# rishabhjain16/audio-visual-llm

Measured on AMD Instinct MI355X. Metric: AV-clip train-step samples/sec (clip_whisper -> Llama-2-7B LoRA), whole job, higher is better.
Workload: dtype bf16

## Files before the change

### audio-visual-llm_amd/avllm/lib.py

```python
from __future__ import annotations

import ctypes as C
import os

import torch

_HERE = os.path.dirname(os.path.abspath(__file__))
LIB_PATH = os.environ.get("AVLLM_LIB_PATH") or os.path.join(_HERE, "libavllm.so")

F32, BF16 = 0, 1
ACT_NONE, ACT_GELU, ACT_QUICK_GELU, ACT_SILU = 0, 1, 2, 3
GEMM_KERNELS = ("SMALLM", "SKINNY64", "128", "RING", "H16", "HP16", "W4", "WP4", "DP", "F32")
ATTN_FORMS = ("ref", "short13x7", "short17x9", "mfma64x4", "mfma128x4")
LORA_PAD = 64

i32, i64, f32, vp, sz = C.c_int32, C.c_int64, C.c_float, C.c_void_p, C.c_size_t
fp = C.POINTER(C.c_float)


class GemmDesc(C.Structure):
    _fields_ = [("A", vp), ("B", vp), ("A2", vp), ("B2", vp), ("C", vp), ("bias", vp), ("R", vp),
                ("lda", i64), ("ldb", i64), ("lda2", i64), ("ldb2", i64), ("ldc", i64), ("ldr", i64),
                ("M", i32), ("N", i32), ("K", i32), ("K2", i32), ("dtype", i32), ("out_f32", i32), ("act", i32),
                ("alpha", f32), ("r_mod", i32), ("g_in", i32), ("g_out", i32), ("g_off", i32), ("drop_seed", C.c_uint32), ("drop_p", f32), ("a_drop_seed", C.c_uint32), ("a_drop_p", f32), ("n_valid", i32), ("seed_dev", vp)]


class EncLayer(C.Structure):
    _fields_ = [(n, vp) for n in ("ln1_w", "ln1_b", "wqkv", "bqkv", "wo", "bo", "ln2_w", "ln2_b", "w1", "b1", "w2", "b2",
                                  "wqkv8", "sqkv8", "wo8", "so8", "w18", "s18", "w28", "s28")]


class Whisper(C.Structure):
    _fields_ = [(n, i32) for n in ("dtype", "d", "heads", "layers", "ffn", "n_mels", "n_ctx", "k1pad")] + \
               [(n, vp) for n in ("conv1_w", "conv1_b", "conv2_w", "conv2_b", "pos")] + \
               [("layer", C.POINTER(EncLayer)), ("lnf_w", vp), ("lnf_b", vp), ("fp8", i32)]


class Clip(C.Structure):
    _fields_ = [(n, i32) for n in ("dtype", "d", "heads", "layers", "ffn", "image", "patch", "tokens")] + \
               [("eps", f32)] + [(n, vp) for n in ("patch_w", "class_emb", "pos", "pre_ln_w", "pre_ln_b")] + \
               [("layer", C.POINTER(EncLayer)), ("fp8", i32), ("frames_bf16", i32)]


class LoraMod(C.Structure):
    _fields_ = [("A_pad", vp), ("AT_pad", vp), ("B_pad", vp), ("BT_pad", vp), ("ld_at", i64), ("gA", vp), ("gB", vp)]


class LlamaLayer(C.Structure):
    _fields_ = [(n, vp) for n in ("ln1_w", "ln2_w", "wqkv", "wo", "wgu", "wdown", "wqkv_t", "wo_t", "wgu_t", "wdown_t")] + \
               [("lora", LoraMod * 4)] + [(n, vp) for n in ("wqkv8", "sqkv8", "wo8", "so8", "wgu8", "sgu8", "wdown8", "sdown8")] + \
               [(n, vp) for n in ("eqkv8", "eo8", "egu8", "edown8")] + \
               [(n, vp) for n in ("wqkv4", "wo4", "wgu4", "wdown4", "eqkv4", "eo4", "egu4", "edown4")] + \
               [(n, vp) for n in ("bqkv", "bo")] + [(n, vp) for n in ("q_norm_w", "k_norm_w")] + [("lora_mlp", LoraMod * 3)]


class Llama(C.Structure):
    _fields_ = [(n, i32) for n in ("dtype", "d", "heads", "layers", "ffn", "vocab", "lora_r", "kv_heads")] + \
               [(n, f32) for n in ("eps", "theta", "lora_scale", "lora_dropout")] + [("dropout_seed", C.c_uint32)] + \
               [(n, vp) for n in ("dropout_seed_dev", "embed", "norm_w", "lm_head", "lm_head_t")] + [("layer", C.POINTER(LlamaLayer))] + \
               [("fp8", i32), ("lm_head8", vp), ("slm_head8", vp)] + \
               [(n, f32) for n in ("rope_factor", "rope_low_freq_factor", "rope_high_freq_factor")] + [("rope_orig_ctx", i32)] + \
               [("decode_fp8", i32), ("elm_head8", vp), ("decode_fp4", i32), ("kv_fp8", i32)]


class GemmF8Desc(C.Structure):
    _fields_ = [("A", vp), ("SA", vp), ("B", vp), ("SB", vp), ("C", vp), ("bias", vp), ("R", vp), ("lda", i64), ("ldb", i64), ("ldc", i64),
                ("ldr", i64), ("M", i32), ("N", i32), ("K", i32), ("act", i32), ("Cq", vp), ("SCq", vp), ("ldcq", i64)]


class DecProjDesc(C.Structure):
    _fields_ = [("A", vp), ("lda", i64), ("W", vp), ("ldw", i64), ("norm_w", vp), ("eps", f32), ("M", i32), ("K", i32), ("N", i32), ("mode", i32),
                ("C", vp), ("ldc", i64), ("out_f32", i32), ("R", vp), ("ldr", i64), ("dq", i32), ("dkv", i32), ("hd", i32), ("rope", vp),
                ("kc", vp), ("vc", vp), ("Tmax", i32), ("pos", i32), ("pos_dev", vp),
                ("lora_t", vp), ("ld_lora_t", i64), ("lora_b", vp * 3), ("lora_r", i32), ("lora_scale", f32), ("W8", vp), ("E8", vp), ("W4", vp),
                ("bias", vp), ("raw_qkv", i32)]


class LogitsProcDesc(C.Structure):
    _fields_ = [("scores", vp), ("ld", i64), ("rows", i64), ("V", i32), ("dtype", i32),
                ("history", vp), ("ldh", i64), ("append", vp), ("cur", i32), ("cur_dev", vp),
                ("repetition_penalty", f32), ("no_repeat_ngram_size", i32), ("min_new_tokens", i32), ("eos", i64), ("log_softmax", i32),
                ("bias_tokens", vp), ("bias_lengths", vp), ("bias_values", vp), ("n_bias", i32), ("bias_max_len", i32),
                ("bad_tokens", vp), ("bad_lengths", vp), ("n_bad", i32), ("bad_max_len", i32),
                ("suppress", vp), ("n_suppress", i32), ("begin_suppress", vp), ("n_begin_suppress", i32)]


class StepState(C.Structure):
    _fields_ = [("step", C.c_uint32), ("dropout_seed", C.c_uint32), ("lr", f32), ("bc1", f32), ("bc2_sqrt", f32), ("skipped", f32),
                ("reserved", C.c_uint32 * 2)]


class AdamwSeg(C.Structure):
    _fields_ = [("p", vp), ("m", vp), ("v", vp), ("g", vp), ("n", i64), ("weight_decay", f32), ("reserved", i32)]


class Schedule(C.Structure):
    _fields_ = [("base_lr", f32), ("beta1", f32), ("beta2", f32), ("warmup_steps", i32), ("total_steps", i32), ("rank", C.c_uint32)]


LAYER_CB = C.CFUNCTYPE(None, i32, vp)

_SIGS = {
    "avllm_version": ([], i32),
    "avllm_gemm": ([C.POINTER(GemmDesc), vp], i32),
    "avllm_gemm_plan": ([C.POINTER(GemmDesc), C.POINTER(i32)], i32),
    "avllm_set_gemm_variant": ([i32], i32),
    "avllm_set_knob": ([C.c_char_p, i32], i32),
    "avllm_get_knob": ([C.c_char_p, C.POINTER(i32)], i32),
    "avllm_attention_fwd_mxq": ([vp, vp, vp, vp, i64, vp, i32, i32, i32, i32, i64, i64, i64, f32, vp], i32),
    "avllm_im2col_k3": ([vp, vp, i32, i32, i32, i32, i32, vp], i32),
    "avllm_groupnorm_tokens": ([vp, vp, vp, vp, i32, i32, i32, i32, f32, i32, i32, vp], i32),
    "avllm_gemm_tn": ([vp, i64, i32, vp, i64, i32, i32, vp, i64, f32, i32, vp], i32),
    "avllm_gemm_tn_drop": ([vp, i64, i32, vp, i64, i32, i32, vp, i64, f32, C.c_uint32, f32, i32, vp], i32),
    "avllm_logmel_table_bytes": ([], C.c_size_t),
    "avllm_logmel_table_init": ([vp, i32], i32),
    "avllm_logmel_workspace_bytes": ([i32, i32], C.c_size_t),
    "avllm_logmel": ([vp, vp, i32, i32, i64, i32, i32, vp, vp, C.c_size_t, vp], i32),
    "avllm_clip_preproc_plan_bytes": ([i32, i32, i32], C.c_size_t),
    "avllm_clip_preproc_plan_init": ([vp, i32, i32, i32, vp, vp], i32),
    "avllm_clip_preproc_workspace_bytes": ([i32, i32, i32, i32], C.c_size_t),
    "avllm_clip_preproc": ([vp, vp, i32, i32, i32, i32, vp, i32, vp, C.c_size_t, vp], i32),
    "avllm_wave_add_noise_chunk": ([], i32),
    "avllm_wave_add_noise_workspace_bytes": ([i32, i32], C.c_size_t),
    "avllm_wave_add_noise": ([vp, i64, vp, i32, i32, vp, i64, vp, i32, vp, f32, f32, f32, C.c_uint32, vp, vp, i64, vp, vp, C.c_size_t, vp], i32),
    "avllm_spec_augment": ([vp, i32, i32, i32, vp, i32, i32, f32, i32, i32, f32, C.c_uint32, vp, vp, vp], i32),
    "avllm_lora_pack_batch": ([vp, i32, i32, i32, i32, vp], i32),
    "avllm_lora_merge": ([vp, i64, i32, i32, vp, vp, i32, f32, i32, vp], i32),
    "avllm_layernorm": ([vp, vp, vp, vp, i64, i32, f32, i32, vp], i32),
    "avllm_rmsnorm_fwd": ([vp, vp, vp, vp, i64, i32, f32, i32, vp], i32),
    "avllm_rmsnorm_bwd": ([vp, vp, vp, vp, vp, vp, i64, i32, i32, vp], i32),
    "avllm_rope": ([vp, i64, i64, i32, i32, i32, i32, f32, i32, i32, vp], i32),
    "avllm_rope_table": ([vp, i32, i32, i32, f32, vp, f32, f32, f32, i32, vp], i32),
    "avllm_rope_tab": ([vp, i64, i64, i32, i32, i32, vp, i32, i32, vp], i32),
    "avllm_kv_append": ([vp, vp, i64, vp, vp, i32, i32, i32, i32, i32, i32, vp], i32),
    "avllm_swiglu_fwd": ([vp, vp, i64, i32, i32, vp], i32),
    "avllm_swiglu_bwd": ([vp, vp, vp, i64, i32, i32, vp], i32),
    "avllm_swiglu_bwd_h": ([vp, vp, vp, vp, i64, i32, i32, vp], i32),
    "avllm_attention_fwd": ([vp, vp, vp, vp, vp, i32, i32, i32, i32, i32, i64, i64, i64, i64, f32, i32, i32, i32, i32, vp], i32),
    "avllm_attention_bwd": ([vp] * 10 + [i32] * 4 + [i64] * 7 + [f32, i32, i32, i32, i32, vp], i32),
    "avllm_attention_bwd_rope": ([vp] * 10 + [i32] * 4 + [i64] * 7 + [f32, i32, i32, i32, i32, vp, vp], i32),
    "avllm_attention_plan": ([i32] * 9 + [C.POINTER(i32), C.POINTER(i32)], i32),
    "avllm_attention_fwd_mxq_ok": ([i32] * 6, i32),
    "avllm_attention_bwd_fuses_rope": ([i32] * 3, i32),
    "avllm_ce_fwd": ([vp, i64, vp, i32, i32, i32, vp, vp, vp, i32, vp], i32),
    "avllm_ce_bwd": ([vp, i64, vp, vp, vp, f32, vp, i32, i32, i32, i32, vp], i32),
    "avllm_argmax_rows": ([vp, i64, i64, i32, vp, i32, vp], i32),
    "avllm_sample_rows": ([vp, i64, i64, i32, f32, i32, f32, C.c_uint32, vp, i32, vp, vp, i64, i64, vp, i32, vp], i32),
    "avllm_sample_rows_scored": ([vp, i64, i64, i32, f32, i32, f32, C.c_uint32, vp, i32, vp, vp, i64, i64, vp, vp, i32, vp], i32),
    "avllm_row_scores": ([vp, i64, i64, i32, vp, f32, vp, vp, i32, vp], i32),
    "avllm_row_scores_logprobs": ([vp, i64, i64, i32, vp, vp, vp, i32, vp], i32),
    "avllm_beam_topk_workspace_bytes": ([i64, i32, i32], sz),
    "avllm_beam_topk": ([vp, i64, i32, i32, i32, vp, i32, vp, vp, vp, vp, sz, vp], i32),
    "avllm_beam_topk_logprobs": ([vp, i64, i32, i32, i32, vp, i32, vp, vp, vp, vp, sz, vp], i32),
    "avllm_logits_process": ([vp, i64, i64, i32, vp, i64, vp, i32, vp, f32, i32, i32, i64, i32, i32, vp], i32),
    "avllm_logits_process_ex": ([C.POINTER(LogitsProcDesc), vp], i32),
    "avllm_kv_gather_rows": ([vp, vp, i32, i64, vp, vp, i32, i64, i32, i32, vp, i32, i32, i32, vp], i32),
    "avllm_embedding": ([vp, vp, vp, i64, i32, i32, vp], i32),
    "avllm_cast": ([vp, i32, vp, i32, i64, vp], i32),
    "avllm_act_residual": ([vp, vp, vp, i64, i32, i32, vp], i32),
    "avllm_dropout": ([vp, vp, i64, i32, C.c_uint32, f32, i32, vp], i32),
    "avllm_whisper_im2col1": ([vp, vp, i32, i32, i32, i32, i32, vp], i32),
    "avllm_whisper_im2col2": ([vp, vp, i32, i32, i32, i32, vp], i32),
    "avllm_clip_patchify": ([vp, vp, i32, i32, i32, i32, i32, vp], i32),
    "avllm_clip_cls_rows": ([vp, vp, vp, i32, i32, i32, i32, vp], i32),
    "avllm_fuse_pool": ([vp, i32, vp, i32, vp, i32, vp, i32, i32, i32, i32, f32, i32, vp], i32),
    "avllm_fuse_pool_bwd": ([vp, vp, i32, vp, i32, i32, i32, i32, i32, i32, f32, i32, vp], i32),
    "avllm_fuse_pool_rows": ([vp, i32, vp, i32, vp, i32, vp, vp, i32, i32, i32, i32, f32, i32, vp], i32),
    "avllm_fuse_pool_rows_bwd": ([vp, vp, i32, vp, i32, i32, vp, i32, i32, i32, i32, f32, i32, vp], i32),
    "avllm_modality_draw": ([vp, vp, i32, f32, f32, C.c_uint32, vp, vp], i32),
    "avllm_gemm_wgrad": ([vp, i64, vp, i64, i32, i32, i32, vp, i64, vp, f32, i32, vp], i32),
    "avllm_grad_sumsq_det_multi": ([C.POINTER(vp), C.POINTER(i64), i32, vp, i32, vp, vp], i32),
    "avllm_adamw_step_multi": ([C.POINTER(AdamwSeg), i32, f32, f32, f32, f32, i32, vp, f32, f32, vp, vp, vp, vp], i32),
    "avllm_grad_sumsq": ([vp, i64, vp, vp], i32),
    "avllm_grad_sumsq_det": ([vp, i64, vp, i32, vp, vp], i32),
    "avllm_adamw_step": ([vp, vp, vp, vp, i64, f32, f32, f32, f32, f32, i32, vp, f32, f32, vp, vp, vp, vp], i32),
    "avllm_step_advance": ([vp, C.POINTER(Schedule), vp], i32),
    "avllm_mx_scale_bytes": ([i32, i32], sz),
    "avllm_mx_quantize": ([vp, i64, i32, i32, vp, i64, vp, i32, i32, vp], i32),
    "avllm_mx4_quantize": ([vp, i64, i32, i32, vp, i64, vp, i32, vp], i32),
    "avllm_gemm_f8": ([C.POINTER(GemmF8Desc), vp], i32),
    "avllm_lora_dx_masked": ([C.POINTER(vp), C.POINTER(i64), C.POINTER(vp), C.POINTER(i64), C.POINTER(C.c_uint32), i32, i32, vp, i64, vp, i64, i32,
                              i32, f32, vp, i32, vp], i32),
    "avllm_llama_lora_bwd_layers": ([C.POINTER(Llama), vp, i32, i32, vp, f32, vp, sz, i32, i32, LAYER_CB, vp, vp], i32),
    "avllm_llama_lora_bwd_layers_dx": ([C.POINTER(Llama), vp, i32, i32, vp, f32, vp, sz, i32, i32, LAYER_CB, vp, vp, vp], i32),
    "avllm_lora_pack": ([vp, vp, i32, i32, i32, vp, vp, i64, vp, vp, i32, vp], i32),
    "avllm_profile_begin": ([i32], i32),
    "avllm_profile_enable": ([i32], i32),
    "avllm_profile_end": ([C.POINTER(C.c_double)], i32),
    "avllm_whisper_workspace_bytes": ([C.POINTER(Whisper), i32], sz),
    "avllm_whisper_encoder_fwd": ([C.POINTER(Whisper), vp, i32, vp, vp, sz, vp], i32),
    "avllm_clip_workspace_bytes": ([C.POINTER(Clip), i32], sz),
    "avllm_clip_vision_cls_fwd": ([C.POINTER(Clip), vp, i32, vp, vp, sz, vp], i32),
    "avllm_llama_train_workspace_bytes": ([C.POINTER(Llama), i32, i32], sz),
    "avllm_llama_lora_fwd_loss": ([C.POINTER(Llama), vp, vp, i32, i32, vp, vp, vp, vp, sz, vp], i32),
    "avllm_llama_lora_bwd": ([C.POINTER(Llama), vp, i32, i32, vp, f32, vp, sz, LAYER_CB, vp, vp], i32),
    "avllm_llama_infer_workspace_bytes": ([C.POINTER(Llama), i32, i32], sz),
    "avllm_llama_prefill": ([C.POINTER(Llama), vp, i32, i32, vp, vp, i32, vp, vp, vp, sz, vp], i32),
    "avllm_llama_decode_step": ([C.POINTER(Llama), vp, i32, i32, vp, vp, i32, vp, vp, sz, vp], i32),
    "avllm_llama_decode_step_at": ([C.POINTER(Llama), vp, i32, i32, vp, vp, vp, i32, vp, vp, sz, vp], i32),
    "avllm_llama_decode_is_fused": ([C.POINTER(Llama), i32], i32),
    "avllm_llama_decode_streams_fp8": ([C.POINTER(Llama), i32], i32),
    "avllm_llama_decode_streams_fp4": ([C.POINTER(Llama), i32], i32),
    "avllm_llama_decode_caches_fp8": ([C.POINTER(Llama), i32], i32),
    "avllm_llama_decode_shared_workspace_bytes": ([C.POINTER(Llama), i32], sz),
    "avllm_llama_decode_step_shared": ([C.POINTER(Llama), vp, i32, i32, i32, vp, vp, vp, i32, vp, vp, i32, vp, vp, sz, vp], i32),
    "avllm_llama_decode_shares_prefix": ([C.POINTER(Llama), i32], i32),
    "avllm_attention_decode_shared_workspace_bytes": ([i32, i32, i32], sz),
    "avllm_attention_decode_shared": ([vp, i64, vp, vp, i32, i32, vp, vp, i32, vp, i32, vp, i64, i32, i32, i32, i32, f32, i32, vp, sz, vp], i32),
    "avllm_attention_decode_shared_kv8": ([vp, i64, vp, vp, vp, vp, i32, i32, vp, vp, vp, vp, i32, vp, i32, vp, i64, i32, i32, i32, i32, f32, i32, vp, sz,
                                           vp], i32),
    "avllm_llama_kv_cache_bytes": ([C.POINTER(Llama), i32, i32], sz),
    "avllm_kv8_append": ([vp, vp, i64, vp, vp, vp, vp, i32, i32, i32, i32, i32, vp], i32),
    "avllm_kv8_rope_append": ([vp, i64, i32, i32, i32, i32, vp, i32, vp, vp, vp, vp, i32, i32, vp, vp], i32),
    "avllm_attention_decode_kv8": ([vp, i64, vp, vp, vp, vp, vp, i64, i32, i32, i32, i32, vp, i32, f32, i32, vp], i32),
    "avllm_kv8_gather_rows": ([vp, vp, i32, i64, vp, vp, i32, i64, i32, i32, vp, i32, i32, vp], i32),
    "avllm_pos_advance": ([vp, i32, vp], i32),
    "avllm_dec_proj": ([C.POINTER(DecProjDesc), vp], i32),
    "avllm_gemm_f8_takes_quantised_output": ([C.POINTER(GemmF8Desc)], i32),
    "avllm_gemm_f8_takes_fast": ([C.POINTER(GemmF8Desc)], i32),
    "avllm_norm_mxq": ([vp, vp, vp, vp, vp, vp, i64, vp, i64, i32, f32, vp], i32),
    "avllm_lora_rank3": ([vp, vp, vp, vp, vp, vp, vp, vp, i32, i32, i32, f32, f32, vp, i32, i32, vp], i32),
    "avllm_gemm_tn_multi": ([vp, i64, i32, vp, vp, vp, vp, vp, vp, vp, i32, i32, i32, f32, f32, vp, i32, i32, vp], i32),
    "avllm_qk_norm_rope": ([vp, i64, i64, i32, i32, i32, i32, vp, vp, f32, vp, vp, vp, vp, vp, i32, i32, vp, i32, vp], i32),
    "avllm_qk_norm_bwd": ([vp, i64, i64, i32, i32, i32, vp, vp, vp, vp, i32, vp], i32),
    "avllm_attention_decode": ([vp, i64, vp, vp, vp, i64, i32, i32, i32, i32, vp, i32, f32, i32, i32, vp], i32),
}

EXPORTS = sorted(list(_SIGS) + ["avllm_last_error"])

_lib = None


def load():
    global _lib
    if _lib is not None:
        return _lib
    if not os.path.exists(LIB_PATH):
        raise RuntimeError(f"libavllm.so not found at {LIB_PATH}: run `python build.py` (hipcc, gfx950). "
                           "There is no CPU or PyTorch fallback for the hot path.")
    lib = C.CDLL(LIB_PATH)
    lib.avllm_last_error.restype = C.c_char_p
    lib.avllm_last_error.argtypes = []
    for name, (args, res) in _SIGS.items():
        fn = getattr(lib, name)
        fn.argtypes = args
        fn.restype = res
    _lib = lib
    return lib


class AvllmError(RuntimeError):
    pass


class knob:

    def __init__(self, name, value):
        self.name, self.value = name.encode(), int(value)

    def __enter__(self):
        prev = i32()
        check(load().avllm_get_knob(self.name, C.byref(prev)))
        self.prev = prev.value
        check(load().avllm_set_knob(self.name, self.value))
        return self

    def __exit__(self, *a):
        check(load().avllm_set_knob(self.name, self.prev))


def check(rc: int):
    if rc != 0:
        msg = load().avllm_last_error().decode(errors="replace")
        if rc == 1:
            raise ValueError(msg)
        raise AvllmError(f"libavllm error {rc}: {msg}")


def dt_of(t: torch.Tensor) -> int:
    if t.dtype == torch.float32:
        return F32
    if t.dtype == torch.bfloat16:
        return BF16
    raise TypeError(f"unsupported dtype {t.dtype}")


def torch_dtype(dt: int):
    return torch.float32 if dt == F32 else torch.bfloat16


def ptr(t):
    if t is None:
        return None
    assert t.is_cuda, "device tensor required"
    return t.data_ptr()


def stream_ptr():
    return torch.cuda.current_stream().cuda_stream
```

### audio-visual-llm_amd/avllm/ops.py

```python
from __future__ import annotations

import collections
import ctypes as C
import math
import numbers

import numpy as np
import torch

from . import lib as L


def _ld(t):
    assert t.stride(-1) == 1, "innermost dimension must be contiguous"
    return t.stride(-2) if t.dim() >= 2 else t.shape[-1]


def gemm(A, B, out=None, bias=None, R=None, A2=None, B2=None, act=L.ACT_NONE, alpha=1.0, out_f32=False,
         r_mod=0, remap=None, M=None, a_drop=None, n_valid=0, drop=None, plan=False):
    lib = L.load()
    M = A.shape[0] if M is None else M
    N, K = B.shape[0], B.shape[1]
    dt = L.dt_of(A)
    if out is None:
        rows = M if remap is None else (M // remap[0]) * remap[1]
        out = torch.empty(rows, N, device=A.device, dtype=torch.float32 if (out_f32 or dt == L.F32) else A.dtype)
    d = L.GemmDesc()
    d.A, d.B, d.C = L.ptr(A), L.ptr(B), L.ptr(out)
    d.lda, d.ldb, d.ldc = _ld(A), _ld(B), _ld(out)
    d.M, d.N, d.K = M, N, K
    if A2 is not None:
        d.A2, d.B2, d.lda2, d.ldb2, d.K2 = L.ptr(A2), L.ptr(B2), _ld(A2), _ld(B2), B2.shape[1]
    d.bias = L.ptr(bias)
    if R is not None:
        d.R, d.ldr = L.ptr(R), _ld(R)
    d.dtype, d.out_f32, d.act, d.alpha, d.r_mod = dt, int(out_f32), act, alpha, r_mod
    if remap is not None:
        d.g_in, d.g_out, d.g_off = remap
    if a_drop is not None:
        d.a_drop_seed, d.a_drop_p = a_drop[0] & 0xFFFFFFFF, a_drop[1]
    if drop is not None:
        d.drop_seed, d.drop_p = drop[0] & 0xFFFFFFFF, drop[1]
    d.n_valid = n_valid
    if plan:
        k = L.i32()
        L.check(lib.avllm_gemm_plan(C.byref(d), C.byref(k)))
        return L.GEMM_KERNELS[k.value]
    L.check(lib.avllm_gemm(C.byref(d), L.stream_ptr()))
    return out


def gemm_tn(P, Q, out, I=None, J=None, alpha=1.0, drop=None):
    lib = L.load()
    I = P.shape[1] if I is None else I
    J = Q.shape[1] if J is None else J
    if drop is not None:
        L.check(lib.avllm_gemm_tn_drop(L.ptr(P), _ld(P), I, L.ptr(Q), _ld(Q), J, P.shape[0], L.ptr(out), _ld(out), alpha,
                                       drop[0] & 0xFFFFFFFF, drop[1], L.dt_of(P), L.stream_ptr()))
        return out
    L.check(lib.avllm_gemm_tn(L.ptr(P), _ld(P), I, L.ptr(Q), _ld(Q), J, P.shape[0], L.ptr(out), _ld(out), alpha,
                              L.dt_of(P), L.stream_ptr()))
    return out


def layernorm(x, w, b, eps=1e-5):
    y = torch.empty_like(x)
    L.check(L.load().avllm_layernorm(L.ptr(x), L.ptr(w), L.ptr(b), L.ptr(y), x.numel() // x.shape[-1], x.shape[-1], eps,
                                     L.dt_of(x), L.stream_ptr()))
    return y


def rmsnorm_fwd(x, w, eps):
    y = torch.empty_like(x)
    rows = x.numel() // x.shape[-1]
    rstd = torch.empty(rows, device=x.device, dtype=torch.float32)
    L.check(L.load().avllm_rmsnorm_fwd(L.ptr(x), L.ptr(w), L.ptr(y), L.ptr(rstd), rows, x.shape[-1], eps, L.dt_of(x), L.stream_ptr()))
    return y, rstd


def rmsnorm_bwd(dy, x, w, rstd, dres=None):
    dx = torch.empty_like(x)
    L.check(L.load().avllm_rmsnorm_bwd(L.ptr(dy), L.ptr(x), L.ptr(w), L.ptr(rstd), L.ptr(dres), L.ptr(dx),
                                       x.numel() // x.shape[-1], x.shape[-1], L.dt_of(x), L.stream_ptr()))
    return dx


def rope_(x2d, T, heads, hd, pos0=0, theta=10000.0, inverse=False):
    L.check(L.load().avllm_rope(L.ptr(x2d), _ld(x2d), x2d.shape[0], T, heads, hd, pos0, theta, int(inverse), L.dt_of(x2d), L.stream_ptr()))
    return x2d


def rope_table(T, hd, pos0=0, theta=10000.0, pos_dev=None, scaling=None, device="cuda"):
    tab = torch.empty(T, hd // 2, 2, device=device, dtype=torch.float32)
    if pos_dev is not None:
        assert pos_dev.dtype == torch.int32 and pos_dev.numel() == 1 and pos_dev.is_cuda
    f, lo, hi, octx = scaling if scaling else (1.0, 1.0, 4.0, 0)
    L.check(L.load().avllm_rope_table(L.ptr(tab), T, hd, pos0, theta, L.ptr(pos_dev), f, lo, hi, int(octx), L.stream_ptr()))
    return tab


def rope_tab_(x2d, T, heads, hd, tab, inverse=False):
    assert tab.dtype == torch.float32 and tab.is_contiguous() and tab.numel() == T * hd
    L.check(L.load().avllm_rope_tab(L.ptr(x2d), _ld(x2d), x2d.shape[0], T, heads, hd, L.ptr(tab), int(inverse), L.dt_of(x2d), L.stream_ptr()))
    return x2d


def qk_norm_rope_(x2d, T, heads, kv_heads, hd, q_w, k_w, eps, tab, save=False, kc=None, vc=None, pos=0, pos_dev=None):
    rows, nqk = x2d.shape[0], heads + kv_heads
    assert tab.dtype == torch.float32 and tab.is_contiguous() and tab.numel() == T * hd and q_w.dtype == x2d.dtype and k_w.dtype == x2d.dtype
    pre = torch.empty(rows, nqk * hd, device=x2d.device, dtype=x2d.dtype) if save else None
    rstd = torch.empty(rows, nqk, device=x2d.device, dtype=torch.float32) if save else None
    if kc is not None:
        assert kc.shape == vc.shape == (rows, kc.shape[1], kv_heads * hd) and kc.is_contiguous() and vc.is_contiguous() and kc.dtype == x2d.dtype
    L.check(L.load().avllm_qk_norm_rope(L.ptr(x2d), _ld(x2d), rows, T, heads, kv_heads, hd, L.ptr(q_w), L.ptr(k_w), eps, L.ptr(tab), L.ptr(pre),
                                        L.ptr(rstd), L.ptr(kc), L.ptr(vc), kc.shape[1] if kc is not None else 0, pos, L.ptr(pos_dev), L.dt_of(x2d),
                                        L.stream_ptr()))
    return pre, rstd


def qk_norm_bwd_(dy2d, heads, kv_heads, hd, q_w, k_w, pre, rstd):
    assert pre.is_contiguous() and rstd.is_contiguous() and rstd.dtype == torch.float32 and pre.dtype == dy2d.dtype
    L.check(L.load().avllm_qk_norm_bwd(L.ptr(dy2d), _ld(dy2d), dy2d.shape[0], heads, kv_heads, hd, L.ptr(q_w), L.ptr(k_w), L.ptr(pre), L.ptr(rstd),
                                       L.dt_of(dy2d), L.stream_ptr()))
    return dy2d


def kv_append(k, v, kc, vc, T, pos0):
    B, Tmax, d = kc.shape
    assert k.shape == (B * T, d) and v.shape == k.shape and _ld(k) == _ld(v) and kc.is_contiguous() and vc.is_contiguous() and vc.shape == kc.shape
    L.check(L.load().avllm_kv_append(L.ptr(k), L.ptr(v), _ld(k), L.ptr(kc), L.ptr(vc), B, T, pos0, Tmax, d, L.dt_of(kc), L.stream_ptr()))


def swiglu_fwd(gu):
    M, F2 = gu.shape
    h = torch.empty(M, F2 // 2, device=gu.device, dtype=gu.dtype)
    L.check(L.load().avllm_swiglu_fwd(L.ptr(gu), L.ptr(h), M, F2 // 2, L.dt_of(gu), L.stream_ptr()))
    return h


def swiglu_bwd(dh, gu):
    dgu = torch.empty_like(gu)
    L.check(L.load().avllm_swiglu_bwd(L.ptr(dh), L.ptr(gu), L.ptr(dgu), gu.shape[0], gu.shape[1] // 2, L.dt_of(gu), L.stream_ptr()))
    return dgu


def swiglu_bwd_h(dh, gu):
    if gu.dim() != 2 or gu.shape[1] % 8 or dh.shape != (gu.shape[0], gu.shape[1] // 2) or dh.dtype != gu.dtype:
        raise ValueError(f"swiglu_bwd_h: gu [M, 2F] with F % 4 == 0 and dh [M, F] of one dtype, got {tuple(gu.shape)} and {tuple(dh.shape)}")
    if not (gu.is_contiguous() and dh.is_contiguous()):
        raise ValueError("swiglu_bwd_h: contiguous tensors")
    dgu = torch.empty_like(gu)
    h = torch.empty_like(dh)
    L.check(L.load().avllm_swiglu_bwd_h(L.ptr(dh), L.ptr(gu), L.ptr(dgu), L.ptr(h), gu.shape[0], gu.shape[1] // 2, L.dt_of(gu), L.stream_ptr()))
    return dgu, h


def attention_plan(B, Tq, Tk, H, hd, causal, dtype, impl=0, kv_heads=None):
    f, b = L.i32(-1), L.i32(-1)
    L.check(L.load().avllm_attention_plan(B, Tq, Tk, H, hd, int(causal), dtype, impl, kv_heads or 0, C.byref(f), C.byref(b)))
    return L.ATTN_FORMS[f.value], (L.ATTN_FORMS[b.value] if b.value >= 0 else None)


def attention_fwd(qkv, B, T, H, hd, causal, scale=None, impl=0, want_lse=True, kv_heads=None, Tk=None, k=None, v=None, out=None, plan=False):
    d = H * hd
    dkv = (kv_heads or H) * hd
    Tk = T if Tk is None else Tk
    assert (k is None) == (v is None) and (k is not None or Tk == T)
    if plan:
        return attention_plan(B, T, Tk, H, hd, causal, L.dt_of(qkv), impl, kv_heads)[0]
    o = torch.empty(B * T, d, device=qkv.device, dtype=qkv.dtype) if out is None else out
    assert o.shape == (B * T, d) and o.dtype == qkv.dtype
    lse = torch.empty(B, H, T, device=qkv.device, dtype=torch.float32) if want_lse else None
    es = qkv.element_size()
    scale = hd ** -0.5 if scale is None else scale
    p = L.ptr(qkv)
    if k is None:
        pk, pv, ldk, ldv = p + d * es, p + (d + dkv) * es, _ld(qkv), _ld(qkv)
    else:
        assert qkv.shape == (B * T, d) and k.shape == (B * Tk, dkv) and v.shape == k.shape and k.dtype == qkv.dtype and v.dtype == qkv.dtype
        pk, pv, ldk, ldv = L.ptr(k), L.ptr(v), _ld(k), _ld(v)
    L.check(L.load().avllm_attention_fwd(p, pk, pv, L.ptr(o), L.ptr(lse), B, T, Tk, H, hd, _ld(qkv), ldk, ldv, _ld(o), scale, int(causal),
                                         L.dt_of(qkv), impl, kv_heads or 0, L.stream_ptr()))
    return o, lse


def attention_fwd_mxq(qkv, B, T, H, hd, scale=None):
    lib = L.load()
    d = H * hd
    q = torch.empty(B * T, d, device=qkv.device, dtype=torch.uint8)
    s = torch.zeros(lib.avllm_mx_scale_bytes(B * T, d), device=qkv.device, dtype=torch.uint8)
    es = qkv.element_size()
    p = L.ptr(qkv)
    L.check(lib.avllm_attention_fwd_mxq(p, p + d * es, p + 2 * d * es, L.ptr(q), d, L.ptr(s), B, T, H, hd, _ld(qkv), _ld(qkv), _ld(qkv),
                                        float(hd ** -0.5 if scale is None else scale), L.stream_ptr()))
    return q, s


def attention_bwd(qkv, o, dout, lse, B, T, H, hd, causal, scale=None, impl=0, kv_heads=None, rope_tab=None, out=None, plan=False):
    if plan:
        return attention_plan(B, T, T, H, hd, causal, L.dt_of(qkv), impl, kv_heads)[1]
    d = H * hd
    dkv = (kv_heads or H) * hd
    dqkv = torch.empty_like(qkv) if out is None else out
    assert dqkv.shape == qkv.shape and dqkv.dtype == qkv.dtype
    delta = torch.empty(B, H, T, device=qkv.device, dtype=torch.float32)
    es = qkv.element_size()
    scale = hd ** -0.5 if scale is None else scale
    p, g = L.ptr(qkv), L.ptr(dqkv)
    args = (p, p + d * es, p + (d + dkv) * es, L.ptr(o), L.ptr(dout), L.ptr(lse), g, g + d * es, g + (d + dkv) * es,
            L.ptr(delta), B, T, H, hd, _ld(qkv), _ld(qkv), _ld(qkv), d, _ld(dqkv), _ld(dqkv), _ld(dqkv),
            scale, int(causal), L.dt_of(qkv), impl, kv_heads or 0)
    if rope_tab is None:
        L.check(L.load().avllm_attention_bwd(*args, L.stream_ptr()))
    else:
        assert rope_tab.dtype == torch.float32 and rope_tab.is_contiguous() and rope_tab.numel() == T * hd
        L.check(L.load().avllm_attention_bwd_rope(*args, L.ptr(rope_tab), L.stream_ptr()))
    return dqkv


def _ce_ld(logits):
    B, T, V = logits.shape
    ld = logits.stride(1) if T > 1 else (logits.stride(0) if B > 1 else (V + 7) // 8 * 8)
    if logits.stride(2) != 1 or (B > 1 and logits.stride(0) != T * ld) or ld < V or ld % 8:
        raise ValueError(f"cross entropy: logits {tuple(logits.shape)} with strides {tuple(logits.stride())} are not [B*T] rows of one stride "
                         "(a multiple of 8, >= V)")
    return ld


def ce_fwd(logits, labels):
    B, T, V = logits.shape
    row_lse = torch.empty(B * T, device=logits.device, dtype=torch.float32)
    acc = torch.zeros(2, device=logits.device, dtype=torch.float32)
    L.check(L.load().avllm_ce_fwd(L.ptr(logits), _ce_ld(logits), L.ptr(labels), B, T, V, L.ptr(row_lse), L.ptr(acc), L.ptr(acc) + 4,
                                  L.dt_of(logits), L.stream_ptr()))
    return row_lse, acc


def ce_bwd(logits, labels, row_lse, acc, grad_scale=1.0, out=None):
    B, T, V = logits.shape
    ld = _ce_ld(logits)
    if out is None:
        out = torch.empty_strided(logits.shape, logits.stride(), device=logits.device, dtype=logits.dtype)
    elif out.shape != logits.shape or out.stride() != logits.stride() or out.dtype != logits.dtype or out.device != logits.device:
        raise ValueError("ce_bwd: out must have the shape, strides, dtype and device of logits")
    L.check(L.load().avllm_ce_bwd(L.ptr(logits), ld, L.ptr(labels), L.ptr(row_lse), L.ptr(acc) + 4, grad_scale, L.ptr(out),
                                  B, T, V, L.dt_of(logits), L.stream_ptr()))
    return out


def argmax_rows(logits2d):
    out = torch.empty(logits2d.shape[0], device=logits2d.device, dtype=torch.int64)
    L.check(L.load().avllm_argmax_rows(L.ptr(logits2d), _ld(logits2d), logits2d.shape[0], logits2d.shape[1], L.ptr(out),
                                       L.dt_of(logits2d), L.stream_ptr()))
    return out


def check_sampling(temperature, top_k, top_p):
    if not (float(temperature) > 0.0 and float(temperature) < float("inf")):
        raise ValueError(f"temperature must be a strictly positive float, got {temperature}")
    if not (0.0 < float(top_p) <= 1.0):
        raise ValueError(f"top_p must be a float in (0, 1], got {top_p}")
    if int(top_k) != top_k or int(top_k) < 0:
        raise ValueError(f"top_k must be a non-negative integer, got {top_k}")


def row_scores(logits, tokens, temperature=1.0, entropy=False, logprobs=False):
    if not (torch.is_tensor(logits) and logits.dim() == 2 and logits.is_cuda and logits.stride(1) == 1
            and logits.dtype in (torch.float32, torch.bfloat16)):
        raise ValueError("row_scores: logits must be a 2-d float32 device tensor with unit column stride")
    rows, V = logits.shape
    if tokens is not None and not (torch.is_tensor(tokens) and tokens.dtype == torch.int64 and tokens.shape == (rows,) and tokens.is_cuda
                                   and tokens.is_contiguous()):
        raise ValueError(f"row_scores: tokens must be int64 [{rows}] on the device")
    if not logprobs and not (float(temperature) > 0.0 and float(temperature) < float("inf")):
        raise ValueError(f"temperature must be a strictly positive float, got {temperature}")
    lp = torch.empty(rows, device=logits.device, dtype=torch.float32)
    ent = torch.empty(rows, device=logits.device, dtype=torch.float32) if entropy else None
    lib = L.load()
    if logprobs:
        L.check(lib.avllm_row_scores_logprobs(L.ptr(logits), _ld(logits), rows, V, L.ptr(tokens), L.ptr(lp), L.ptr(ent), L.dt_of(logits),
                                              L.stream_ptr()))
    else:
        L.check(lib.avllm_row_scores(L.ptr(logits), _ld(logits), rows, V, L.ptr(tokens), float(temperature), L.ptr(lp), L.ptr(ent),
                                     L.dt_of(logits), L.stream_ptr()))
    return (lp, ent) if entropy else lp


def sample_rows(logits, temperature, top_k, top_p, seed, step, unfinished=None, eos=None, pad=None, row_seeds=None, return_logprob=False):
    check_sampling(temperature, top_k, top_p)
    rows, V = logits.shape
    out = torch.empty(rows, device=logits.device, dtype=torch.int64)
    step_dev = None
    if torch.is_tensor(step):
        assert step.dtype == torch.int32 and step.numel() == 1 and step.is_cuda
        step_dev, step = step, 0
    if unfinished is not None:
        assert unfinished.dtype == torch.bool and unfinished.shape == (rows,) and unfinished.is_contiguous()
    if row_seeds is not None:
        assert row_seeds.dtype == torch.int32 and row_seeds.shape == (rows,) and row_seeds.is_contiguous()
    eos = -1 if eos is None else int(eos)
    pad = (eos if eos >= 0 else 0) if pad is None else int(pad)
    lp = torch.empty(rows, device=logits.device, dtype=torch.float32) if return_logprob else None
    L.check(L.load().avllm_sample_rows_scored(L.ptr(logits), _ld(logits), rows, V, float(temperature), int(top_k), float(top_p),
                                              int(seed) & 0xFFFFFFFF, L.ptr(row_seeds), int(step), L.ptr(step_dev), L.ptr(unfinished),
                                              eos, pad, L.ptr(out), L.ptr(lp), L.dt_of(logits), L.stream_ptr()))
    return (out, lp) if return_logprob else out


LOGITS_PROCESS_MAX_HISTORY = 1024


def check_logits_processors(repetition_penalty, no_repeat_ngram_size, min_new_tokens):
    p = repetition_penalty
    if isinstance(p, bool) or not isinstance(p, numbers.Real) or not (0.0 < float(p) < float("inf")):
        raise ValueError(f"repetition_penalty must be a strictly positive float, got {p!r}")
    for name, v in (("no_repeat_ngram_size", no_repeat_ngram_size), ("min_new_tokens", min_new_tokens)):
        if isinstance(v, bool) or not isinstance(v, numbers.Integral) or v < 0:
            raise ValueError(f"{name} must be a non-negative integer, got {v!r}")
    return float(p) != 1.0 or no_repeat_ngram_size > 0 or min_new_tokens > 0


LOGITS_BIAS_MAX_SEQUENCES, LOGITS_BIAS_MAX_SEQUENCE_LENGTH = 4096, 16

SequenceTable = collections.namedtuple("SequenceTable", "tokens lengths values n max_len vocab")
TokenTable = collections.namedtuple("TokenTable", "ids n vocab")
_TABLE_FIELDS = {
    "sequence_bias": (SequenceTable, dict(bias_tokens="tokens", bias_lengths="lengths", bias_values="values", n_bias="n", bias_max_len="max_len")),
    "bad_words_ids": (SequenceTable, dict(bad_tokens="tokens", bad_lengths="lengths", n_bad="n", bad_max_len="max_len")),
    "suppress_tokens": (TokenTable, dict(suppress="ids", n_suppress="n")),
    "begin_suppress_tokens": (TokenTable, dict(begin_suppress="ids", n_begin_suppress="n")),
}


def _token_ids(name, ids, vocab):
    if hasattr(ids, "tolist"):
        ids = ids.tolist()
    if isinstance(ids, (str, bytes, dict)) or not hasattr(ids, "__iter__"):
        raise ValueError(f"{name} must be a list of token ids, got {ids!r}")
    ids = list(ids)
    for t in ids:
        if isinstance(t, bool) or not isinstance(t, numbers.Integral) or t < 0:
            raise ValueError(f"{name} must hold non-negative integers, got {t!r}")
        if vocab is not None and t >= vocab:
            raise ValueError(f"{name}: token id {t} is outside the vocabulary of {vocab} entries")
    return [int(t) for t in ids]


def _sequences(name, seqs):
    if len(seqs) > LOGITS_BIAS_MAX_SEQUENCES:
        raise ValueError(f"{name} has {len(seqs)} sequences: at most LOGITS_BIAS_MAX_SEQUENCES = {LOGITS_BIAS_MAX_SEQUENCES} are supported")
    for q in seqs:
        if len(q) == 0:
            raise ValueError(f"{name} has an empty sequence")
        if len(q) > LOGITS_BIAS_MAX_SEQUENCE_LENGTH:
            raise ValueError(f"{name} has a sequence of {len(q)} tokens: at most LOGITS_BIAS_MAX_SEQUENCE_LENGTH = "
                             f"{LOGITS_BIAS_MAX_SEQUENCE_LENGTH} are supported")
    return seqs


def _normalise_logits_bias(sequence_bias, bad_words_ids, suppress_tokens, begin_suppress_tokens, vocab, eos):
    sb = bw = None
    if sequence_bias is not None:
        if isinstance(sequence_bias, dict):
            if any(not isinstance(k, tuple) for k in sequence_bias):
                raise ValueError(f"sequence_bias has to be a dict with tuples of token ids as keys, got {sequence_bias!r}")
            items = list(sequence_bias.items())
        elif isinstance(sequence_bias, (list, tuple)):
            if any(not isinstance(e, (list, tuple)) or len(e) != 2 or not isinstance(e[0], (list, tuple)) for e in sequence_bias):
                raise ValueError(f"sequence_bias has to be a list of [token ids, bias] pairs, got {sequence_bias!r}")
            items = [(tuple(e[0]), e[1]) for e in sequence_bias]
        else:
            raise ValueError(f"sequence_bias has to be a non-empty dict or list of [token ids, bias] pairs, got {sequence_bias!r}")
        if not items:
            raise ValueError("sequence_bias has to be non-empty")
        sb = {}
        for k, b in items:
            if isinstance(b, bool) or not isinstance(b, (float, np.floating)) or not math.isfinite(b):
                raise ValueError(f"sequence_bias: the bias of {k!r} must be a finite float, got {b!r}")
            sb[tuple(_token_ids("sequence_bias", k, vocab))] = float(b)
        _sequences("sequence_bias", list(sb))
    if bad_words_ids is not None:
        if not isinstance(bad_words_ids, (list, tuple)) or len(bad_words_ids) == 0:
            raise ValueError(f"bad_words_ids has to be a non-empty list, got {bad_words_ids!r}")
        if any(not isinstance(w, (list, tuple)) for w in bad_words_ids):
            raise ValueError(f"bad_words_ids has to be a list of lists of token ids, got {bad_words_ids!r}")
        bw = [tuple(_token_ids("bad_words_ids", w, vocab)) for w in bad_words_ids]
        bw = list(dict.fromkeys(w for w in bw if eos is None or w != (int(eos),)))
        if not bw:
            raise ValueError("bad_words_ids holds nothing but [eos], which HF drops: no sequence is left to ban")
        _sequences("bad_words_ids", bw)
    st = None if suppress_tokens is None else sorted(set(_token_ids("suppress_tokens", suppress_tokens, vocab)))
    bs = None if begin_suppress_tokens is None else sorted(set(_token_ids("begin_suppress_tokens", begin_suppress_tokens, vocab)))
    return sb, bw, st or None, bs or None


def check_logits_bias(sequence_bias=None, bad_words_ids=None, suppress_tokens=None, begin_suppress_tokens=None, vocab=None, eos=None):
    return any(t is not None for t in _normalise_logits_bias(sequence_bias, bad_words_ids, suppress_tokens, begin_suppress_tokens, vocab, eos))


def logits_bias_tables(sequence_bias=None, bad_words_ids=None, suppress_tokens=None, begin_suppress_tokens=None, *, vocab, eos=None,
                       device="cuda"):
    sb, bw, st, bs = _normalise_logits_bias(sequence_bias, bad_words_ids, suppress_tokens, begin_suppress_tokens, int(vocab), eos)

    def seq_table(seqs, values):
        tok = np.full((len(seqs), LOGITS_BIAS_MAX_SEQUENCE_LENGTH), -1, dtype=np.int32)
        for i, q in enumerate(seqs):
            tok[i, :len(q)] = q
        ln = np.array([len(q) for q in seqs], dtype=np.int32)
        dev = lambda a: torch.from_numpy(a).to(device)
        return SequenceTable(dev(tok), dev(ln), None if values is None else dev(np.array(values, dtype=np.float32)), len(seqs), int(ln.max()),
                             int(vocab))

    out = {}
    if sb is not None:
        keys = sorted(sb, key=lambda q: (q[-1], len(q) != 1))
        out["sequence_bias"] = seq_table(keys, [sb[q] for q in keys])
    if bw is not None:
        out["bad_words_ids"] = seq_table(bw, None)
    for name, ids in (("suppress_tokens", st), ("begin_suppress_tokens", bs)):
        if ids is not None:
            out[name] = TokenTable(torch.tensor(ids, dtype=torch.int32).to(device), len(ids), int(vocab))
    return out


def logits_process(scores, history, cur, repetition_penalty=1.0, no_repeat_ngram_size=0, min_new_tokens=0, eos=None, log_softmax=False,
                   append=None, *, sequence_bias=None, bad_words_ids=None, suppress_tokens=None, begin_suppress_tokens=None):
    check_logits_processors(repetition_penalty, no_repeat_ngram_size, min_new_tokens)
    if scores.dim() != 2 or not scores.is_cuda or scores.stride(1) != 1:
        raise ValueError("logits_process: scores must be a 2-d device tensor with unit column stride")
    rows, V = scores.shape
    cur_dev = None
    if torch.is_tensor(cur):
        assert cur.dtype == torch.int32 and cur.numel() == 1 and cur.is_cuda
        cur_dev, cur = cur, 0
    hptr, ldh = None, 0
    if history is not None:
        if history.dtype != torch.int64 or history.dim() != 2 or history.shape[0] != rows or not history.is_cuda or \
                (history.shape[1] > 1 and history.stride(1) != 1):
            raise ValueError(f"logits_process: history must be an int64 device tensor [{rows}, ld] with unit column stride")
        ldh = history.stride(0) if rows > 1 and history.shape[1] > 0 else history.shape[1]
        if cur_dev is None and int(cur) > history.shape[1]:
            raise ValueError(f"logits_process: history length {cur} > the {history.shape[1]} columns of history")
        hptr = L.ptr(history) if history.numel() else None
    if append is not None:
        assert append.dtype == torch.int64 and append.shape == (rows,) and append.is_contiguous() and append.is_cuda
    d = L.LogitsProcDesc(scores=L.ptr(scores), ld=_ld(scores), rows=rows, V=V, dtype=L.dt_of(scores), history=hptr, ldh=ldh, append=L.ptr(append),
                         cur=int(cur), cur_dev=L.ptr(cur_dev), repetition_penalty=float(repetition_penalty),
                         no_repeat_ngram_size=int(no_repeat_ngram_size), min_new_tokens=int(min_new_tokens), eos=-1 if eos is None else int(eos),
                         log_softmax=int(bool(log_softmax)))
    for (name, (kind, fields)), t in zip(_TABLE_FIELDS.items(), (sequence_bias, bad_words_ids, suppress_tokens, begin_suppress_tokens)):
        if t is None:
            continue
        if not isinstance(t, kind):
            raise ValueError(f"logits_process: {name} must be a prepared {kind.__name__} (ops.logits_bias_tables), got {type(t).__name__}")
        if t.vocab != V:
            raise ValueError(f"logits_process: the {name} table was built for a vocabulary of {t.vocab}, the scores have {V} columns")
        for field, attr in fields.items():
            v = getattr(t, attr)
            setattr(d, field, L.ptr(v) if torch.is_tensor(v) else v)
    L.check(L.load().avllm_logits_process_ex(C.byref(d), L.stream_ptr()))
    return scores


BEAM_MAX_BEAMS, BEAM_MAX_K = 16, 32


def beam_topk(logits, beam_scores, num_beams, k, logprobs=False):
    nb, k = int(num_beams), int(k)
    if not 1 <= nb <= BEAM_MAX_BEAMS:
        raise ValueError(f"num_beams must be in [1, {BEAM_MAX_BEAMS}], got {num_beams}")
    if not 1 <= k <= BEAM_MAX_K:
        raise ValueError(f"k must be in [1, {BEAM_MAX_K}], got {k}")
    if logits.dtype != torch.float32 or logits.dim() != 2 or not logits.is_cuda:
        raise ValueError("beam_topk: logits must be a 2-d float32 device tensor")
    rows, V = logits.shape
    if rows % nb:
        raise ValueError(f"beam_topk: {rows} logits rows are not a multiple of num_beams = {nb}")
    if k > nb * V:
        raise ValueError(f"beam_topk: k = {k} > num_beams * V = {nb * V}")
    if beam_scores.dtype != torch.float32 or beam_scores.numel() != rows or not beam_scores.is_cuda:
        raise ValueError(f"beam_topk: beam_scores must be float32 [{rows}] on the device")
    beam_scores = beam_scores.contiguous()
    B = rows // nb
# ... 521 lines not shown
```

### audio-visual-llm_amd/csrc/api.hip

```cpp
#include "common.h"
#include "avllm_internal.h"
#include <stdarg.h>

static thread_local char g_err[512] = "";

int av_set_error(int code, const char* fmt, ...) {
    va_list ap;
    va_start(ap, fmt);
    vsnprintf(g_err, sizeof(g_err), fmt, ap);
    va_end(ap);
    return code;
}

#include <mutex>
#include <string.h>
static const struct { const char* name; int dflt; } g_knob_def[AV_KNOB_COUNT] = {
    {"DECODE_FUSED", 1}, {"DEC_AL", 0}, {"LORA_UNBATCHED", 0}, {"F8_UNFUSED_QUANT", 0}, {"F8_FAST", 1}, {"ATTN_SHORT", 1},
    {"NARROW_EPILOGUE", 0}, {"TN_CHUNK", 0}, {"GEMM_DBG", 0}, {"GEMM_GW", 0}, {"GEMM_VARIANT", 0}, {"SHARED_SPLIT", 0}};
static int g_knob[AV_KNOB_COUNT];
static std::once_flag g_knob_once;
static void knob_init() {
    for (int i = 0; i < AV_KNOB_COUNT; ++i) {
        char env[64];
        snprintf(env, sizeof(env), "AVLLM_%s", g_knob_def[i].name);
        const char* e = getenv(env);
        g_knob[i] = e ? atoi(e) : g_knob_def[i].dflt;
    }
}
int av_knob(int id) {
    std::call_once(g_knob_once, knob_init);
    return g_knob[id];
}
static int* knob_slot(const char* name) {
    std::call_once(g_knob_once, knob_init);
    for (int i = 0; name && i < AV_KNOB_COUNT; ++i)
        if (!strcmp(name, g_knob_def[i].name)) return &g_knob[i];
    return nullptr;
}

int av_device(int* ncu) {
    static int g_ncu[AV_MAX_DEVICES];
    int dev = 0;
    if (hipGetDevice(&dev) != hipSuccess) dev = 0;
    const int slot = dev & (AV_MAX_DEVICES - 1);
    if (!g_ncu[slot] && hipDeviceGetAttribute(&g_ncu[slot], hipDeviceAttributeMultiprocessorCount, dev) != hipSuccess) g_ncu[slot] = 256;
    *ncu = g_ncu[slot];
    return slot;
}

#define ST ((hipStream_t)stream)
extern "C" {
int avllm_set_knob(const char* name, int32_t value) {
    int* k = knob_slot(name);
    AV_CHECK_ARG(k, "set_knob: unknown knob '%s'", name ? name : "(null)");
    *k = value;
    return AV_OK;
}
int avllm_get_knob(const char* name, int32_t* value) {
    const int* k = knob_slot(name);
    AV_CHECK_ARG(k && value, "get_knob: unknown knob '%s'", name ? name : "(null)");
    *value = *k;
    return AV_OK;
}
int avllm_set_gemm_variant(int v) { return avllm_set_knob("GEMM_VARIANT", v); }
const char* avllm_last_error(void) { return g_err; }
int avllm_version(void) { return 100; }

int avllm_gemm(const avllm_gemm_desc* d, void* stream) { return av_gemm(d, ST); }
int avllm_gemm_plan(const avllm_gemm_desc* d, int32_t* kernel) { AV_CHECK_ARG(kernel, "gemm_plan: null kernel"); return av_gemm_plan(d, kernel); }
int avllm_gemm_tn(const void* P, int64_t ldp, int32_t I, const void* Q, int64_t ldq, int32_t J, int32_t M, float* out,
                  int64_t ldo, float alpha, int32_t dtype, void* stream) { return av_gemm_tn(P, ldp, I, Q, ldq, J, M, out, ldo, alpha, dtype, ST); }
int avllm_gemm_tn_drop(const void* P, int64_t ldp, int32_t I, const void* Q, int64_t ldq, int32_t J, int32_t M, float* out,
                       int64_t ldo, float alpha, uint32_t seed, float p, int32_t dtype, void* stream) { return av_gemm_tn(P, ldp, I, Q, ldq, J, M, out, ldo, alpha, dtype, ST, seed, p); }
int avllm_layernorm(const void* x, const void* w, const void* b, void* y, int64_t rows, int32_t d, float eps, int32_t dtype,
                    void* stream) { return av_layernorm(x, w, b, y, rows, d, eps, dtype, ST); }
int avllm_rmsnorm_fwd(const void* x, const void* w, void* y, float* rstd, int64_t rows, int32_t d, float eps, int32_t dtype,
                      void* stream) { return av_rmsnorm_fwd(x, w, y, rstd, rows, d, eps, dtype, ST); }
int avllm_rmsnorm_bwd(const void* dy, const void* x, const void* w, const float* rstd, const void* dres_in, void* dx_out,
                      int64_t rows, int32_t d, int32_t dtype, void* stream) { return av_rmsnorm_bwd(dy, x, w, rstd, dres_in, dx_out, rows, d, dtype, ST); }
int avllm_rope(void* x, int64_t ld, int64_t rows, int32_t T, int32_t heads, int32_t hd, int32_t pos0, float theta,
               int32_t inverse, int32_t dtype, void* stream) { return av_rope(x, ld, rows, T, heads, hd, pos0, theta, inverse, dtype, ST); }
int avllm_rope_table(float* tab, int32_t T, int32_t hd, int32_t pos0, float theta, const int32_t* pos_dev, float factor,
                     float low_freq_factor, float high_freq_factor, int32_t orig_ctx, void* stream) {
    AvRopeScale sc;
    sc.factor = factor; sc.low_freq_factor = low_freq_factor; sc.high_freq_factor = high_freq_factor; sc.orig_ctx = orig_ctx;
    AV_CHECK_ARG(orig_ctx <= 0 || (factor > 0.f && low_freq_factor > 0.f && high_freq_factor > low_freq_factor), "rope_table: bad llama3 scaling");
    return av_rope_table(tab, T, hd, pos0, theta, ST, pos_dev, sc);
}
int avllm_rope_tab(void* x, int64_t ld, int64_t rows, int32_t T, int32_t heads, int32_t hd, const float* tab, int32_t inverse,
                   int32_t dtype, void* stream) { return av_rope_tab(x, ld, rows, T, heads, hd, tab, inverse, dtype, ST); }
int avllm_kv_append(const void* k, const void* v, int64_t ld, void* kc, void* vc, int32_t B, int32_t T, int32_t pos0, int32_t Tmax,
                    int32_t d, int32_t dtype, void* stream) { return av_kv_append(k, v, ld, kc, vc, B, T, pos0, Tmax, d, dtype, ST); }
int avllm_swiglu_fwd(const void* gu, void* h, int64_t M, int32_t F, int32_t dtype, void* stream) { return av_swiglu_fwd(gu, h, M, F, dtype, ST); }
int avllm_swiglu_bwd(const void* dh, const void* gu, void* dgu, int64_t M, int32_t F, int32_t dtype, void* stream) { return av_swiglu_bwd(dh, gu, dgu, M, F, dtype, ST); }
int avllm_swiglu_bwd_h(const void* dh, const void* gu, void* dgu, void* h, int64_t M, int32_t F, int32_t dtype, void* stream) { return av_swiglu_bwd_h(dh, gu, dgu, h, M, F, dtype, ST); }
int avllm_attention_fwd(const void* q, const void* k, const void* v, void* o, float* lse, int32_t B, int32_t Tq, int32_t Tk,
                        int32_t H, int32_t hd, int64_t ldq, int64_t ldk, int64_t ldv, int64_t ldo, float scale, int32_t causal,
                        int32_t dtype, int32_t impl, int32_t kv_heads, void* stream) {
    return av_attention_fwd(q, k, v, o, lse, B, Tq, Tk, H, hd, ldq, ldk, ldv, ldo, scale, causal, dtype, impl, ST, kv_heads);
}
int avllm_attention_bwd(const void* q, const void* k, const void* v, const void* o, const void* dout, const float* lse, void* dq,
                        void* dk, void* dv, float* delta_ws, int32_t B, int32_t T, int32_t H, int32_t hd, int64_t ldq, int64_t ldk,
                        int64_t ldv, int64_t ldo, int64_t lddq, int64_t lddk, int64_t lddv, float scale, int32_t causal,
                        int32_t dtype, int32_t impl, int32_t kv_heads, void* stream) {
    return av_attention_bwd(q, k, v, o, dout, lse, dq, dk, dv, delta_ws, B, T, H, hd, ldq, ldk, ldv, ldo, lddq, lddk, lddv, scale, causal, dtype, impl, ST, kv_heads);
}
int avllm_attention_bwd_rope(const void* q, const void* k, const void* v, const void* o, const void* dout, const float* lse, void* dq,
                             void* dk, void* dv, float* delta_ws, int32_t B, int32_t T, int32_t H, int32_t hd, int64_t ldq, int64_t ldk,
                             int64_t ldv, int64_t ldo, int64_t lddq, int64_t lddk, int64_t lddv, float scale, int32_t causal,
                             int32_t dtype, int32_t impl, int32_t kv_heads, const float* rope_tab, void* stream) {
    return av_attention_bwd(q, k, v, o, dout, lse, dq, dk, dv, delta_ws, B, T, H, hd, ldq, ldk, ldv, ldo, lddq, lddk, lddv, scale, causal, dtype, impl, ST, kv_heads, rope_tab);
}
int avllm_ce_fwd(const void* logits, int64_t ld, const int64_t* labels, int32_t B, int32_t T, int32_t V, float* row_lse,
                 float* loss_sum, float* count, int32_t dtype, void* stream) { return av_ce_fwd(logits, ld, labels, B, T, V, row_lse, loss_sum, count, dtype, ST); }
int avllm_ce_bwd(const void* logits, int64_t ld, const int64_t* labels, const float* row_lse, const float* count, float grad_scale,
                 void* dlogits, int32_t B, int32_t T, int32_t V, int32_t dtype, void* stream) { return av_ce_bwd(logits, ld, labels, row_lse, count, grad_scale, dlogits, B, T, V, dtype, ST); }
int avllm_argmax_rows(const void* logits, int64_t ld, int64_t rows, int32_t V, int64_t* out, int32_t dtype, void* stream) { return av_argmax_rows(logits, ld, rows, V, out, dtype, ST); }
int avllm_sample_rows(const void* logits, int64_t ld, int64_t rows, int32_t V, float temperature, int32_t top_k, float top_p, uint32_t seed,
                      const uint32_t* row_seeds, int32_t step, const int32_t* step_dev, uint8_t* unfinished, int64_t eos, int64_t pad,
                      int64_t* out, int32_t dtype, void* stream) {
    return av_sample_rows(logits, ld, rows, V, temperature, top_k, top_p, seed, row_seeds, step, step_dev, unfinished, eos, pad, out, nullptr, dtype, ST);
}
int avllm_sample_rows_scored(const void* logits, int64_t ld, int64_t rows, int32_t V, float temperature, int32_t top_k, float top_p, uint32_t seed,
                             const uint32_t* row_seeds, int32_t step, const int32_t* step_dev, uint8_t* unfinished, int64_t eos, int64_t pad,
                             int64_t* out, float* out_logprob, int32_t dtype, void* stream) {
    return av_sample_rows(logits, ld, rows, V, temperature, top_k, top_p, seed, row_seeds, step, step_dev, unfinished, eos, pad, out, out_logprob, dtype,
                          ST);
}
int avllm_row_scores(const void* logits, int64_t ld, int64_t rows, int32_t V, const int64_t* tokens, float temperature, float* out_logprob,
                     float* out_entropy, int32_t dtype, void* stream) {
    return av_row_scores(logits, ld, rows, V, tokens, temperature, out_logprob, out_entropy, 0, dtype, ST);
}
int avllm_row_scores_logprobs(const void* logprobs, int64_t ld, int64_t rows, int32_t V, const int64_t* tokens, float* out_logprob,
                              float* out_entropy, int32_t dtype, void* stream) {
    return av_row_scores(logprobs, ld, rows, V, tokens, 1.0f, out_logprob, out_entropy, 1, dtype, ST);
}
size_t avllm_beam_topk_workspace_bytes(int64_t rows, int32_t V, int32_t k) { return av_beam_topk_workspace_bytes(rows, V, k); }
int avllm_beam_topk(const float* logits, int64_t ld, int32_t B, int32_t num_beams, int32_t V, const float* beam_scores, int32_t k,
                    float* out_scores, int32_t* out_beams, int64_t* out_tokens, void* ws, size_t ws_bytes, void* stream) {
    return av_beam_topk(logits, ld, B, num_beams, V, beam_scores, k, out_scores, out_beams, out_tokens, ws, ws_bytes, 0, ST);
}
int avllm_beam_topk_logprobs(const float* logprobs, int64_t ld, int32_t B, int32_t num_beams, int32_t V, const float* beam_scores, int32_t k,
                             float* out_scores, int32_t* out_beams, int64_t* out_tokens, void* ws, size_t ws_bytes, void* stream) {
    return av_beam_topk(logprobs, ld, B, num_beams, V, beam_scores, k, out_scores, out_beams, out_tokens, ws, ws_bytes, 1, ST);
}
int avllm_logits_process(void* scores, int64_t ld, int64_t rows, int32_t V, int64_t* history, int64_t ldh, const int64_t* append, int32_t cur,
                         const int32_t* cur_dev, float repetition_penalty, int32_t no_repeat_ngram_size, int32_t min_new_tokens, int64_t eos,
                         int32_t log_softmax, int32_t dtype, void* stream) {
    avllm_logits_proc_desc d = {};
    d.scores = scores; d.ld = ld; d.rows = rows; d.V = V; d.dtype = dtype;
    d.history = history; d.ldh = ldh; d.append = append; d.cur = cur; d.cur_dev = cur_dev;
    d.repetition_penalty = repetition_penalty; d.no_repeat_ngram_size = no_repeat_ngram_size; d.min_new_tokens = min_new_tokens;
    d.eos = eos; d.log_softmax = log_softmax;
    return av_logits_process(&d, ST);
}
int avllm_logits_process_ex(const avllm_logits_proc_desc* d, void* stream) { return av_logits_process(d, ST); }
int avllm_kv_gather_rows(const void* k_src, const void* v_src, int32_t src_rows, int64_t src_T, void* k_dst, void* v_dst, int32_t dst_rows,
                         int64_t dst_T, int32_t layers, int32_t dkv, const int32_t* parent, int32_t t0, int32_t t1, int32_t dtype, void* stream) {
    return av_kv_gather_rows(k_src, v_src, src_rows, src_T, k_dst, v_dst, dst_rows, dst_T, layers, dkv, parent, t0, t1, dtype, ST);
}
int avllm_embedding(const void* table, const int64_t* ids, void* out, int64_t n, int32_t d, int32_t dtype, void* stream) { return av_embedding(table, ids, out, n, d, dtype, ST); }
int avllm_cast(const void* src, int32_t sdt, void* dst, int32_t ddt, int64_t n, void* stream) { return av_cast(src, sdt, dst, ddt, n, ST); }
int avllm_dropout(const void* x, void* y, int64_t rows, int32_t d, uint32_t seed, float p, int32_t dtype, void* stream) { return av_dropout(x, y, rows, d, seed, p, dtype, ST); }
int avllm_whisper_im2col1(const float* mel, void* cols, int32_t B, int32_t n_mels, int32_t T, int32_t Kpad, int32_t dtype, void* stream) { return av_whisper_im2col1(mel, cols, B, n_mels, T, Kpad, dtype, ST); }
int avllm_whisper_im2col2(const void* h, void* cols, int32_t B, int32_t T, int32_t d, int32_t dtype, void* stream) { return av_whisper_im2col2(h, cols, B, T, d, dtype, ST); }
int avllm_clip_patchify(const float* frames, void* cols, int32_t N, int32_t S, int32_t p, int32_t Kpad, int32_t dtype, void* stream) { return av_clip_patchify(frames, cols, N, S, p, Kpad, dtype, ST); }
int avllm_clip_cls_rows(const void* ce, const void* pos, void* x, int32_t N, int32_t tokens, int32_t d, int32_t dtype, void* stream) { return av_clip_cls_rows(ce, pos, x, N, tokens, d, dtype, ST); }
int avllm_fuse_pool(const void* a, int32_t Ta, const void* v, int32_t Tv, const void* pe, int32_t P, void* out, int32_t B, int32_t L,
                    int32_t S_out, int32_t D, float fs, int32_t dtype, void* stream) { return av_fuse_pool(a, Ta, v, Tv, pe, P, out, B, L, S_out, D, fs, dtype, ST); }
int avllm_fuse_pool_bwd(const void* dx, void* da, int32_t Ta, void* dv, int32_t Tv, int32_t P, int32_t B, int32_t L, int32_t S_out, int32_t D,
                        float fs, int32_t dtype, void* stream) { return av_fuse_pool_bwd(dx, da, Ta, dv, Tv, P, B, L, S_out, D, fs, dtype, ST); }
int avllm_fuse_pool_rows(const void* a, int32_t Ta, const void* v, int32_t Tv, const void* pe, int32_t P, const int32_t* mode, void* out, int32_t B,
                         int32_t L, int32_t S_out, int32_t D, float fs, int32_t dtype, void* stream) {
    return av_fuse_pool_rows(a, Ta, v, Tv, pe, P, mode, out, B, L, S_out, D, fs, dtype, ST);
}
int avllm_fuse_pool_rows_bwd(const void* dx, void* da, int32_t Ta, void* dv, int32_t Tv, int32_t P, const int32_t* mode, int32_t B, int32_t L,
                             int32_t S_out, int32_t D, float fs, int32_t dtype, void* stream) {
    return av_fuse_pool_rows_bwd(dx, da, Ta, dv, Tv, P, mode, B, L, S_out, D, fs, dtype, ST);
}
int avllm_modality_draw(const int32_t* mode_in, int32_t* mode_out, int32_t B, float p_drop_audio, float p_drop_video, uint32_t seed,
                        const uint32_t* seed_dev, void* stream) { return av_modality_draw(mode_in, mode_out, B, p_drop_audio, p_drop_video, seed, seed_dev, ST); }
int avllm_gemm_wgrad(const void* dY, int64_t ldy, const void* X, int64_t ldx, int32_t M, int32_t N, int32_t K, float* dW, int64_t ldw, float* db,
                     float alpha, int32_t dtype, void* stream) { return av_gemm_wgrad(dY, ldy, X, ldx, M, N, K, dW, ldw, db, alpha, dtype, ST); }
int avllm_grad_sumsq_det_multi(const float* const* g, const int64_t* n, int32_t nbuf, float* partials, int32_t nparts, float* sumsq, void* stream) {
    return av_grad_sumsq_det_multi(g, n, nbuf, partials, nparts, sumsq, ST);
}
int avllm_adamw_step_multi(const avllm_adamw_seg* segs, int32_t nseg, float lr, float b1, float b2, float eps, int32_t step, const float* sumsq,
                           float max_norm, float prescale, const float* guard, float* skipped, const avllm_step_state* state, void* stream) {
    return av_adamw_step_multi(segs, nseg, lr, b1, b2, eps, step, sumsq, max_norm, prescale, guard, skipped, state, ST);
}
int avllm_grad_sumsq(const float* g, int64_t n, float* sumsq, void* stream) { return av_grad_sumsq(g, n, sumsq, ST); }
int avllm_grad_sumsq_det(const float* g, int64_t n, float* partials, int32_t nparts, float* sumsq, void* stream) { return av_grad_sumsq_det(g, n, partials, nparts, sumsq, ST); }
int avllm_adamw_step(float* p, const float* g, float* m, float* v, int64_t n, float lr, float b1, float b2, float eps, float wd,
                     int32_t step, const float* sumsq, float max_norm, float prescale, const float* guard, float* skipped,
                     const avllm_step_state* state, void* stream) {
    return av_adamw_step(p, g, m, v, n, lr, b1, b2, eps, wd, step, sumsq, max_norm, prescale, guard, skipped, state, ST);
}
int avllm_act_residual(const void* x, const void* r, void* y, int64_t n, int32_t act, int32_t dtype, void* stream) { return av_act_residual(x, r, y, n, act, dtype, ST); }
int avllm_step_advance(avllm_step_state* state, const avllm_schedule* sched, void* stream) { return av_step_advance(state, sched, ST); }
int avllm_lora_pack(const float* A, const float* Bm, int32_t r, int32_t din, int32_t dout, void* A_pad, void* AT_pad, int64_t ld_at,
                    void* B_pad, void* BT_pad, int32_t dtype, void* stream) { return av_lora_pack(A, Bm, r, din, dout, A_pad, AT_pad, ld_at, B_pad, BT_pad, dtype, ST); }
int avllm_lora_merge(void* W, int64_t ldw, int32_t N, int32_t K, const float* A, const float* B, int32_t r, float scale, int32_t dtype,
                     void* stream) { return av_lora_merge(W, ldw, N, K, A, B, r, scale, dtype, ST); }
}
```

### audio-visual-llm_amd/csrc/attention.hip

```cpp
#include "common.h"
#include "avllm_internal.h"
#include "attention_tile.h"
#include "mx.h"
#include <type_traits>
#include <cstdlib>

namespace {

using namespace avt;

__device__ __forceinline__ float max3f(float a, float x, float y) { return __builtin_elementwise_maximum(__builtin_elementwise_maximum(a, x), y); }

enum class Stage { Single, Double };

template <int HD, int NW, Stage ST, bool CAUSAL>
__global__ __launch_bounds__(NW * 64, 2) void attn_fwd_mfma(const bf16* __restrict__ q, const bf16* __restrict__ k,
                                                         const bf16* __restrict__ v, bf16* __restrict__ o, float* __restrict__ lse,
                                                         int Tq, int Tk, int H, long ldq, long ldk, long ldv, long ldo,
                                                         float scale_log2e, int G) {
    constexpr int KS = HD * 2 + 16;
    constexpr int VS = HD * 2 + 64;
    constexpr int NT = NW * 64;
    constexpr int NBUF = ST == Stage::Double ? 2 : 1;
    __shared__ __attribute__((aligned(16))) char k_lds_[NBUF * 64 * KS];
    __shared__ __attribute__((aligned(16))) char v_lds_[NBUF * 64 * VS];
    char* k_lds = k_lds_;
    char* v_lds = v_lds_;

    const int tid = threadIdx.x, lane = tid & 63, w = tid >> 6;
    const int r = lane & 31, half = lane >> 5;
    const int hh = blockIdx.y, b = blockIdx.z, hk = hh / G;
    const int q0 = (blockIdx.x * NW + w) * 32;
    const int off = Tk - Tq;
    const int qpos = q0 + r;
    const int qrow = qpos < Tq ? qpos : Tq - 1;

    bf16x8 qf[HD / 16];
    {
        const bf16* qp = q + ((long)b * Tq + qrow) * ldq + (long)hh * HD + 8 * half;
#pragma unroll
        for (int ks = 0; ks < HD / 16; ++ks) qf[ks] = *(const bf16x8*)(qp + 16 * ks);
    }
    f32x16 oacc[HD / 32];
#pragma unroll
    for (int d = 0; d < HD / 32; ++d)
#pragma unroll
        for (int i = 0; i < 16; ++i) oacc[d][i] = 0.f;
    float m_run = -INFINITY, l_run = 0.f;

    const int blk_qmax = min(Tq - 1, (int)(blockIdx.x * NW + NW) * 32 - 1);
    const int k_end = CAUSAL ? min(Tk, blk_qmax + off + 1) : Tk;
    const bool wave_active = q0 < Tq;
    const int wave_kmax = CAUSAL ? min(Tk - 1, min(Tq - 1, q0 + 31) + off) : Tk - 1;

    constexpr int CPR = HD / 8, NCH = (64 * CPR + NT - 1) / NT;
    u32x4 kreg[NCH], vreg[NCH];
    auto prefetch = [&](int kb0) {
#pragma unroll
        for (int i = 0; i < NCH; ++i) {
            const int c = tid + i * NT;
            const int row = c / CPR, ch = c % CPR;
            const int key = kb0 + row;
            kreg[i] = (u32x4){0u, 0u, 0u, 0u}; vreg[i] = (u32x4){0u, 0u, 0u, 0u};
            if (c < 64 * CPR && key < Tk) {
                kreg[i] = *(const u32x4*)(k + ((long)b * Tk + key) * ldk + (long)hk * HD + ch * 8);
                vreg[i] = *(const u32x4*)(v + ((long)b * Tk + key) * ldv + (long)hk * HD + ch * 8);
            }
        }
    };
    auto park = [&](int buf) {
#pragma unroll
        for (int i = 0; i < NCH; ++i) {
            const int c = tid + i * NT;
            if (c < 64 * CPR) {
                const int row = c / CPR, ch = c % CPR;
                *(u32x4*)(k_lds_ + buf * 64 * KS + row * KS + ch * 16) = kreg[i];
                *(u32x4*)(v_lds_ + buf * 64 * VS + row * VS + ch * 16) = vreg[i];
            }
        }
    };
    if (ST == Stage::Double) { prefetch(0); park(0); if (64 < k_end) prefetch(64); }
    for (int kb = 0; kb < k_end; kb += 64) {
        if (ST == Stage::Double) {
            const int buf = (kb >> 6) & 1;
            __syncthreads();
            if (kb + 64 < k_end) { park(buf ^ 1); if (kb + 128 < k_end) prefetch(kb + 128); }
            k_lds = k_lds_ + buf * 64 * KS; v_lds = v_lds_ + buf * 64 * VS;
        } else {
            prefetch(kb);
            __syncthreads();
            park(0);
            __syncthreads();
        }
        if (!wave_active || kb > wave_kmax) continue;

        const bool two = (kb + 32 <= wave_kmax) && (kb + 32 < Tk);
        f32x16 s0, s1;
#pragma unroll
        for (int i = 0; i < 16; ++i) { s0[i] = 0.f; s1[i] = 0.f; }
#pragma unroll
        for (int ks = 0; ks < HD / 16; ++ks) {
            const bf16x8 kf0 = *(const bf16x8*)(k_lds + r * KS + (2 * ks + half) * 16);
            s0 = __builtin_amdgcn_mfma_f32_32x32x16_bf16(kf0, qf[ks], s0, 0, 0, 0);
        }
        if (two) {
#pragma unroll
            for (int ks = 0; ks < HD / 16; ++ks) {
                const bf16x8 kf1 = *(const bf16x8*)(k_lds + (32 + r) * KS + (2 * ks + half) * 16);
                s1 = __builtin_amdgcn_mfma_f32_32x32x16_bf16(kf1, qf[ks], s1, 0, 0, 0);
            }
        }
        const int klim = CAUSAL ? min(Tk - 1, qpos + off) : Tk - 1;
        const bool need_mask = (kb + 64 > Tk) || !two || (CAUSAL && kb + 63 > q0 + off);
        float mloc = -INFINITY;
        if (need_mask) {
#pragma unroll
            for (int i = 0; i < 16; ++i) {
                const int key0 = kb + acc_row(i, half);
                s0[i] = key0 <= klim ? s0[i] : -INFINITY;
                s1[i] = (two && key0 + 32 <= klim) ? s1[i] : -INFINITY;
            }
        }
#pragma unroll
        for (int i = 0; i < 16; ++i) mloc = max3f(mloc, s0[i], s1[i]);
        mloc = __builtin_elementwise_maximum(mloc, __shfl_xor(mloc, 32));
        mloc *= scale_log2e;
        const float m_new = __builtin_elementwise_maximum(m_run, mloc);
        const float m_use = m_new == -INFINITY ? 0.f : m_new;
        const float alpha = __builtin_amdgcn_exp2f(m_run - m_use);
        float psum = 0.f;
#pragma unroll
        for (int i = 0; i < 16; ++i) {
            s0[i] = __builtin_amdgcn_exp2f(fmaf(s0[i], scale_log2e, -m_use));
            s1[i] = __builtin_amdgcn_exp2f(fmaf(s1[i], scale_log2e, -m_use));
            psum += s0[i] + s1[i];
        }
        l_run = l_run * alpha + psum;
        m_run = m_new;
#pragma unroll
        for (int d = 0; d < HD / 32; ++d)
#pragma unroll
            for (int i = 0; i < 16; ++i) oacc[d][i] *= alpha;

#pragma unroll
        for (int sb = 0; sb < 2; ++sb) {
            if (sb == 1 && !two) break;
#pragma unroll
            for (int s = 0; s < 2; ++s) {
                bf16x8 pb;
#pragma unroll
                for (int j = 0; j < 8; ++j) pb[j] = (bf16)(sb == 0 ? s0[8 * s + j] : s1[8 * s + j]);
#pragma unroll
                for (int d = 0; d < HD / 32; ++d) {
                    const bf16x8 vt = tr_frag(v_lds, VS, 32 * sb + 16 * s, 32 * d, lane);
                    oacc[d] = __builtin_amdgcn_mfma_f32_32x32x16_bf16(vt, pb, oacc[d], 0, 0, 0);
                }
            }
        }
    }
    if (!wave_active) return;
    const float l_tot = l_run + __shfl_xor(l_run, 32);
    const float inv = 1.0f / l_tot;
    if (qpos < Tq) {
        store_acc_rows<HD>(o + ((long)b * Tq + qpos) * ldo + (long)hh * HD, oacc, half, inv);
        if (lse && half == 0) lse[((long)b * H + hh) * Tq + qpos] = (m_run + log2f(l_tot)) * 0.69314718055994531f;
    }
}

template <int NKB, int NW, bool QOUT, bool FULLK, bool WLSE>
__global__ __launch_bounds__(NW * 64) void attn_fwd_short(const bf16* __restrict__ q, const bf16* __restrict__ k, const bf16* __restrict__ v,
                                                          bf16* __restrict__ o, float* __restrict__ lse, int T, int H, long ldq, long ldk,
                                                          long ldv, long ldo, float scale_log2e, int G, uint8_t* __restrict__ oq, long ldoq,
                                                          uint8_t* __restrict__ osc, int RBo) {
    constexpr int HD = 64, KS = 160, VS = 160, OS = 80;
    constexpr int NPV = (NKB + 1) / 2, KROWS = NKB * 16, VROWS = NPV * 32, NT = NW * 64;
    constexpr int NQ = (NKB + NW - 1) / NW;
    extern __shared__ __attribute__((aligned(16))) char smem[];
    char* k_lds = smem;
    char* v_lds = smem + KROWS * KS;
    const int tid = threadIdx.x, lane = tid & 63, w = tid >> 6;
    char* o_lds = smem + KROWS * KS + VROWS * VS + w * 16 * OS;
    const int fr = lane & 15, fq = lane >> 4;
    const int hh = blockIdx.x, b = blockIdx.y, hk = hh / G;
    const int nkb = (T + 15) >> 4;

    constexpr int NCH = (VROWS * 8 + NT - 1) / NT;
    u32x4 kreg[NCH], vreg[NCH];
#pragma unroll
    for (int i = 0; i < NCH; ++i) {
        const int c = tid + i * NT, row = c >> 3, ch = c & 7;
        kreg[i] = (u32x4){0u, 0u, 0u, 0u}; vreg[i] = (u32x4){0u, 0u, 0u, 0u};
        if (row < T) {
            kreg[i] = *(const u32x4*)(k + ((long)b * T + row) * ldk + (long)hk * HD + ch * 8);
            vreg[i] = *(const u32x4*)(v + ((long)b * T + row) * ldv + (long)hk * HD + ch * 8);
        }
    }
    bf16x8 qf[NQ][2];
#pragma unroll
    for (int i = 0; i < NQ; ++i) {
        int qrow = (w + NW * i) * 16 + fr;
        qrow = qrow < T ? qrow : T - 1;
        const bf16* qp = q + ((long)b * T + qrow) * ldq + (long)hh * HD + 8 * fq;
        qf[i][0] = *(const bf16x8*)qp;
        qf[i][1] = *(const bf16x8*)(qp + 32);
    }
#pragma unroll
    for (int i = 0; i < NCH; ++i) {
        const int c = tid + i * NT, row = c >> 3, ch = c & 7;
        if (row < KROWS) *(u32x4*)(k_lds + row * KS + ch * 16) = kreg[i];
        if (row < VROWS) *(u32x4*)(v_lds + row * VS + ch * 16) = vreg[i];
    }
    __syncthreads();

    bf16x8 ones;
#pragma unroll
    for (int j = 0; j < 8; ++j) ones[j] = (bf16)1.0f;
    asm volatile("" : "+v"(ones));
    const f32x4 zero4 = {0.f, 0.f, 0.f, 0.f};
    const int i16 = lane & 15, g = lane >> 4;
    auto max3 = [](float a, float x, float y) __attribute__((always_inline)) { return max3f(a, x, y); };
    auto qblock = [&](int qi, auto fullc) __attribute__((always_inline)) {
        constexpr bool FULL = decltype(fullc)::value;
        const int qb = w + NW * qi;
        const int q0 = qb * 16;
        f32x4 sc[NKB];
#pragma unroll
        for (int kb = 0; kb < NKB; ++kb) {
            sc[kb] = (f32x4){-INFINITY, -INFINITY, -INFINITY, -INFINITY};
            if (FULL || kb < nkb) {
                const char* kr = k_lds + (kb * 16 + fr) * KS + fq * 16;
                const bf16x8 k0 = *(const bf16x8*)kr, k1 = *(const bf16x8*)(kr + 64);
                f32x4 a = __builtin_amdgcn_mfma_f32_16x16x32_bf16(k0, qf[qi][0], zero4, 0, 0, 0);
                sc[kb] = __builtin_amdgcn_mfma_f32_16x16x32_bf16(k1, qf[qi][1], a, 0, 0, 0);
            }
        }
        if (T & 15) {
            if constexpr (FULL) {
#pragma unroll
                for (int i = 0; i < 4; ++i) sc[NKB - 1][i] = ((NKB - 1) * 16 + 4 * fq + i < T) ? sc[NKB - 1][i] : -INFINITY;
            } else {
                const int kb = nkb - 1;
#pragma unroll
                for (int x = 0; x < NKB; ++x)
                    if (x == kb) {
#pragma unroll
                        for (int i = 0; i < 4; ++i) sc[x][i] = (x * 16 + 4 * fq + i < T) ? sc[x][i] : -INFINITY;
                    }
            }
        }
        float m = -INFINITY;
#pragma unroll
        for (int kb = 0; kb < NKB; ++kb) { m = max3(m, sc[kb][0], sc[kb][1]); m = max3(m, sc[kb][2], sc[kb][3]); }
        m = max3(m, __shfl_xor(m, 16), m);
        m = max3(m, __shfl_xor(m, 32), m);
        const float msc = m * scale_log2e;
        f32x4 lacc = zero4, oacc[4] = {zero4, zero4, zero4, zero4};
        float lsum = 0.f;
#pragma unroll
        for (int st = 0; st < NPV; ++st) {
            if (FULL || 2 * st < nkb) {
                bf16x8 pb;
                const bool second = 2 * st + 1 < NKB;
                const f32x4 s1 = sc[second ? 2 * st + 1 : 2 * st];
#pragma unroll
                for (int i = 0; i < 4; ++i) {
                    const float p0 = __builtin_amdgcn_exp2f(fmaf(sc[2 * st][i], scale_log2e, -msc));
                    const float p1 = second ? __builtin_amdgcn_exp2f(fmaf(s1[i], scale_log2e, -msc)) : 0.f;
                    if constexpr (WLSE) lsum += p0 + p1;
                    pb[i] = (bf16)p0;
                    pb[4 + i] = (bf16)p1;
                }
                lacc = __builtin_amdgcn_mfma_f32_16x16x32_bf16(ones, pb, lacc, 0, 0, 0);
                const char* vr = v_lds + (32 * st + 4 * g + (i16 >> 2)) * VS + (4 * (i16 & 3)) * 2;
#pragma unroll
                for (int t = 0; t < 4; ++t) {
                    const short4v lo = __builtin_amdgcn_ds_read_tr16_b64_v4i16((lds_s4_ptr)(vr + t * 32));
                    const short4v hi = __builtin_amdgcn_ds_read_tr16_b64_v4i16((lds_s4_ptr)(vr + t * 32 + 16 * VS));
                    const short8v both = {lo[0], lo[1], lo[2], lo[3], hi[0], hi[1], hi[2], hi[3]};
                    oacc[t] = __builtin_amdgcn_mfma_f32_16x16x32_bf16(__builtin_bit_cast(bf16x8, both), pb, oacc[t], 0, 0, 0);
                }
            }
        }
        const float l = lacc[0], inv = 1.0f / l;
        if constexpr (WLSE) {
            lsum += __shfl_xor(lsum, 16);
            lsum += __shfl_xor(lsum, 32);
            if (fq == 0 && q0 + fr < T) lse[((long)b * H + hh) * T + q0 + fr] = (msc + log2f(lsum)) * 0.69314718055994531f;
        }
#pragma unroll
        for (int hf = 0; hf < 2; ++hf) {
#pragma unroll
            for (int tt = 0; tt < 2; ++tt) {
                const f32x4 a = oacc[2 * hf + tt];
                float vals[4] = {a[0] * inv, a[1] * inv, a[2] * inv, a[3] * inv};
                store_f<4>((bf16*)(o_lds + fr * OS) + 16 * tt + 4 * fq, vals);
            }
            asm volatile("s_waitcnt lgkmcnt(0)" ::: "memory");
            const int row = lane >> 2, ch = lane & 3;
            const u32x4 val = *(const u32x4*)(o_lds + row * OS + ch * 16);
            if constexpr (QOUT) {
                const bf16x8 vb = __builtin_bit_cast(bf16x8, val);
                float f[8], amax = 0.f;
#pragma unroll
                for (int c = 0; c < 8; ++c) { f[c] = (float)vb[c]; amax = fmaxf(amax, fabsf(f[c])); }
                amax = fmaxf(amax, __shfl_xor(amax, 1));
                amax = fmaxf(amax, __shfl_xor(amax, 2));
                const int e = mx_block_exp<MX_EMAX_E4M3>(amax);
                uint32_t pk[2];
                mx_pack_e4m3<8>(f, mx_inv_scale(e), pk);
                if (q0 + row < T) {
                    const long m = (long)b * T + q0 + row;
                    typedef __attribute__((ext_vector_type(2))) unsigned int u32x2;
                    *(u32x2*)(oq + m * ldoq + (long)hh * HD + hf * 32 + ch * 8) = (u32x2){pk[0], pk[1]};
                    if (ch == 0) {
                        const int cb = hh * (HD / 32) + hf;
                        osc[((((long)(cb >> 2) * RBo + (m >> 6)) * 4 + (cb & 3)) * 16 + (m & 15)) * 4 + ((m >> 4) & 3)] = (uint8_t)mx_exp_byte(e);
                    }
                }
            } else {
                if (q0 + row < T) *(u32x4*)(o + ((long)b * T + q0 + row) * ldo + (long)hh * HD + hf * 32 + ch * 8) = val;
            }
            asm volatile("s_waitcnt lgkmcnt(0)" ::: "memory");
        }
    };
    if constexpr (FULLK) {
#pragma unroll
        for (int qi = 0; qi < NQ; ++qi)
            if (w + NW * qi < NKB) qblock(qi, std::true_type{});
    } else {
#pragma unroll
        for (int qi = 0; qi < NQ; ++qi)
            if (w + NW * qi < nkb) qblock(qi, std::false_type{});
    }
}

template <int NKB, int NW, bool QOUT, bool FULLK, bool WLSE, class... Args>
int launch_short_form(int B, int H, hipStream_t st, Args... args) {
    constexpr int LDS = NKB * 16 * 160 + ((NKB + 1) / 2) * 32 * 160 + NW * 16 * 80;
    static bool attr[AV_MAX_DEVICES] = {};
    int dev = 0;
    AV_HIP(hipGetDevice(&dev));
    if (!attr[dev & (AV_MAX_DEVICES - 1)]) {
        AV_HIP(hipFuncSetAttribute((const void*)attn_fwd_short<NKB, NW, QOUT, FULLK, WLSE>, hipFuncAttributeMaxDynamicSharedMemorySize, LDS));
        attr[dev & (AV_MAX_DEVICES - 1)] = true;
    }
    hipLaunchKernelGGL((attn_fwd_short<NKB, NW, QOUT, FULLK, WLSE>), dim3(H, B), dim3(NW * 64), LDS, st, args...);
    AV_LAUNCH_CHECK();
    return AV_OK;
}

template <int NKB, int NW>
int launch_fwd_short(const void* q, const void* k, const void* v, void* o, float* lse, int B, int T, int H, long ldq, long ldk, long ldv,
                     long ldo, float scale, hipStream_t st, int G, void* oq = nullptr, long ldoq = 0, void* osc = nullptr) {
    AV_CHECK_ARG(!(oq && lse), "attention_fwd_short: the quantised-output form writes no LSE");
    const int RBo = oq ? (int)(((long)B * T + 255) / 256 * 4) : 0;
    const bool fullk = ((T + 15) >> 4) == NKB;
    auto go = [&](auto qout, auto wlse, auto full) {
        return launch_short_form<NKB, NW, decltype(qout)::value, decltype(full)::value, decltype(wlse)::value>(
            B, H, st, (const bf16*)q, (const bf16*)k, (const bf16*)v, (bf16*)o, lse, T, H, ldq, ldk, ldv, ldo, scale * 1.4426950408889634f, G, (uint8_t*)oq, ldoq,
            (uint8_t*)osc, RBo);
    };
    const std::true_type yes;
    const std::false_type no;
    if (oq) return fullk ? go(yes, no, yes) : go(yes, no, no);
    if (lse) return fullk ? go(no, yes, yes) : go(no, yes, no);
    return fullk ? go(no, no, yes) : go(no, no, no);
}

template <int HD>
int launch_fwd(const void* q, const void* k, const void* v, void* o, float* lse, int B, int Tq, int Tk, int H, long ldq,
               long ldk, long ldv, long ldo, float scale, int causal, hipStream_t st, int G) {
    constexpr int NW = 4;
    constexpr Stage ST = HD == 64 ? Stage::Double : Stage::Single;
    const dim3 grid(av_cdiv(Tq, 32 * NW), H, B), block(NW * 64);
    const float sl = scale * 1.4426950408889634f;
    auto go = [&](auto c) {
        hipLaunchKernelGGL((attn_fwd_mfma<HD, NW, ST, decltype(c)::value>), grid, block, 0, st, (const bf16*)q, (const bf16*)k, (const bf16*)v, (bf16*)o, lse, Tq, Tk, H,
                           ldq, ldk, ldv, ldo, sl, G);
    };
    if (causal) go(std::true_type{}); else go(std::false_type{});
    AV_LAUNCH_CHECK();
    return AV_OK;
}

bool mfma_takes(int hd, int dtype, int impl) { return impl == 0 && dtype == AV_BF16 && (hd == 64 || hd == 128); }
bool is_short(int form) { return form == AVLLM_ATTN_SHORT13X7 || form == AVLLM_ATTN_SHORT17X9; }

}

int av_attention_fwd_form(int B, int Tq, int Tk, int hd, int causal, int dtype, int impl) {
    if (!mfma_takes(hd, dtype, impl)) return AVLLM_ATTN_REF;
    if (hd == 128) return AVLLM_ATTN_MFMA128X4;
    if (!causal && Tq == Tk && B <= 65535 && av_knob(AV_KNOB_ATTN_SHORT) != 0) {
        if (Tq <= 208) return AVLLM_ATTN_SHORT13X7;
        if (Tq <= 272) return AVLLM_ATTN_SHORT17X9;
    }
    return AVLLM_ATTN_MFMA64X4;
}
int av_attention_bwd_form(int hd, int dtype, int impl) {
    return !mfma_takes(hd, dtype, impl) ? AVLLM_ATTN_REF : hd == 64 ? AVLLM_ATTN_MFMA64X4 : AVLLM_ATTN_MFMA128X4;
}
extern "C" int avllm_attention_plan(int32_t B, int32_t Tq, int32_t Tk, int32_t H, int32_t hd, int32_t causal, int32_t dtype, int32_t impl, int32_t kv_heads,
                                    int32_t* fwd_form, int32_t* bwd_form) {
    AV_CHECK_ARG(fwd_form && bwd_form && B > 0 && Tq > 0 && Tk > 0 && H > 0, "attention_plan: bad args");
    AV_CHECK_ARG(H % (kv_heads <= 0 ? H : kv_heads) == 0, "attention_plan: %d query heads are not a multiple of %d key/value heads", H, kv_heads);
    *fwd_form = av_attention_fwd_form(B, Tq, Tk, hd, causal, dtype, impl);
    *bwd_form = Tq == Tk ? av_attention_bwd_form(hd, dtype, impl) : -1;
    return AV_OK;
}

int av_attention_fwd(const void* q, const void* k, const void* v, void* o, float* lse, int B, int Tq, int Tk, int H,
                     int hd, long ldq, long ldk, long ldv, long ldo, float scale, int causal, int dtype, int impl,
                     hipStream_t st, int kv_heads) {
    AV_CHECK_ARG(q && k && v && o && B > 0 && Tq > 0 && Tk > 0 && H > 0, "attention_fwd: bad args");
    if (kv_heads <= 0) kv_heads = H;
    AV_CHECK_ARG(H % kv_heads == 0, "attention_fwd: %d query heads are not a multiple of %d key/value heads", H, kv_heads);
    const int G = H / kv_heads;
    AV_CHECK_ARG(ldq % 8 == 0 && ldk % 8 == 0 && ldv % 8 == 0 && ldo % 8 == 0, "attention_fwd: row strides must be multiples of 8");
    AV_CHECK_ARG(!causal || Tk >= Tq, "attention_fwd: causal needs Tk >= Tq");
    switch (av_attention_fwd_form(B, Tq, Tk, hd, causal, dtype, impl)) {
    case AVLLM_ATTN_SHORT13X7: return launch_fwd_short<13, 7>(q, k, v, o, lse, B, Tq, H, ldq, ldk, ldv, ldo, scale, st, G);
    case AVLLM_ATTN_SHORT17X9: return launch_fwd_short<17, 9>(q, k, v, o, lse, B, Tq, H, ldq, ldk, ldv, ldo, scale, st, G);
    case AVLLM_ATTN_MFMA64X4: return launch_fwd<64>(q, k, v, o, lse, B, Tq, Tk, H, ldq, ldk, ldv, ldo, scale, causal, st, G);
    case AVLLM_ATTN_MFMA128X4: return launch_fwd<128>(q, k, v, o, lse, B, Tq, Tk, H, ldq, ldk, ldv, ldo, scale, causal, st, G);
    default: return av_attention_fwd_ref(q, k, v, o, lse, B, Tq, Tk, H, hd, ldq, ldk, ldv, ldo, scale, causal, dtype, st, G);
    }
}

bool av_attention_fwd_mxq_ok(int B, int T, int H, int hd, int dtype, int kv_heads) {
    return is_short(av_attention_fwd_form(B, T, T, hd, 0, dtype, 0)) && (kv_heads <= 0 || kv_heads == H) && (H * hd) % 128 == 0 && !av_knob(AV_KNOB_F8_UNFUSED_QUANT);
}
int av_attention_fwd_mxq(const void* q, const void* k, const void* v, void* oq, long ldoq, void* osc, int B, int T, int H, int hd, long ldq, long ldk,
                         long ldv, float scale, hipStream_t st) {
    AV_CHECK_ARG(q && k && v && oq && osc && av_attention_fwd_mxq_ok(B, T, H, hd, AV_BF16, H) && ldoq % 16 == 0 && ldq % 8 == 0 && ldk % 8 == 0 && ldv % 8 == 0,
                 "attention_fwd_mxq: bad args (bf16, head_dim 64, T <= 272, 16-byte aligned code rows)");
    if (av_attention_fwd_form(B, T, T, hd, 0, AV_BF16, 0) == AVLLM_ATTN_SHORT13X7)
        return launch_fwd_short<13, 7>(q, k, v, nullptr, nullptr, B, T, H, ldq, ldk, ldv, 0, scale, st, 1, oq, ldoq, osc);
    return launch_fwd_short<17, 9>(q, k, v, nullptr, nullptr, B, T, H, ldq, ldk, ldv, 0, scale, st, 1, oq, ldoq, osc);
}
extern "C" int avllm_attention_fwd_mxq(const void* q, const void* k, const void* v, void* oq, int64_t ldoq, void* scales, int32_t B, int32_t T, int32_t H,
                                       int32_t hd, int64_t ldq, int64_t ldk, int64_t ldv, float scale, void* stream) {
    return av_attention_fwd_mxq(q, k, v, oq, ldoq, scales, B, T, H, hd, ldq, ldk, ldv, scale, (hipStream_t)stream);
}
extern "C" int avllm_attention_fwd_mxq_ok(int32_t B, int32_t T, int32_t H, int32_t hd, int32_t dtype, int32_t kv_heads) {
    return av_attention_fwd_mxq_ok(B, T, H, hd, dtype, kv_heads);
}

bool av_attention_bwd_fuses_rope(int dtype, int hd, int impl) { return av_attention_bwd_form(hd, dtype, impl) != AVLLM_ATTN_REF; }
extern "C" int avllm_attention_bwd_fuses_rope(int32_t dtype, int32_t hd, int32_t impl) { return av_attention_bwd_fuses_rope(dtype, hd, impl); }

int av_attention_bwd(const void* q, const void* k, const void* v, const void* o, const void* dout, const float* lse,
                     void* dq, void* dk, void* dv, float* delta_ws, int B, int T, int H, int hd, long ldq, long ldk,
                     long ldv, long ldo, long lddq, long lddk, long lddv, float scale, int causal, int dtype, int impl,
                     hipStream_t st, int kv_heads, const float* rope_tab) {
    AV_CHECK_ARG(q && k && v && o && dout && lse && dq && dk && dv && delta_ws, "attention_bwd: null");
    AV_CHECK_ARG(!rope_tab || av_attention_bwd_fuses_rope(dtype, hd, impl), "attention_bwd: the fused inverse RoPE exists in the bf16 MFMA kernels only");
    if (kv_heads <= 0) kv_heads = H;
    AV_CHECK_ARG(H % kv_heads == 0, "attention_bwd: %d query heads are not a multiple of %d key/value heads", H, kv_heads);
    const int G = H / kv_heads;
    if (av_attention_bwd_form(hd, dtype, impl) != AVLLM_ATTN_REF)
        return av_attention_bwd_mfma(q, k, v, dout, lse, delta_ws, dq, dk, dv, B, T, H, hd, ldq, ldk, ldv, ldo, lddq, lddk, lddv, scale, causal, st, G, o, ldo, rope_tab);
    AV_TRY(av_attention_delta(o, dout, delta_ws, B, T, H, hd, ldo, ldo, dtype, st));
    return av_attention_bwd_ref(q, k, v, dout, lse, delta_ws, dq, dk, dv, B, T, H, hd, ldq, ldk, ldv, ldo, lddq, lddk, lddv, scale, causal, dtype, st, G);
}
```

### audio-visual-llm_amd/csrc/avllm_internal.h

```cpp
#pragma once
#include <hip/hip_runtime.h>
#include "../../include/avllm.h"

#define AV_MAX_DEVICES 64
int av_device(int* ncu);
int av_gemm_plan(const avllm_gemm_desc* d, int* kernel);
int av_gemm(const avllm_gemm_desc* d, hipStream_t st);
bool av_gemm_dp_ok(const avllm_gemm_desc* d);
int av_gemm_dp(const avllm_gemm_desc* d, hipStream_t st, int dbg, int dev, int ncu);
int av_gemm_tn(const void* P, long ldp, int I, const void* Q, long ldq, int J, int M, float* out, long ldo,
               float alpha, int dtype, hipStream_t st, uint32_t drop_seed = 0, float drop_p = 0.f, const uint32_t* seed_dev = nullptr);
int av_layernorm(const void* x, const void* w, const void* b, void* y, long rows, int d, float eps, int dtype, hipStream_t st);
int av_rmsnorm_fwd(const void* x, const void* w, void* y, float* rstd, long rows, int d, float eps, int dtype, hipStream_t st);
int av_rmsnorm_bwd(const void* dy, const void* x, const void* w, const float* rstd, const void* dres_in, void* dx_out,
                   long rows, int d, int dtype, hipStream_t st);
int av_rope(void* x, long ld, long rows, int T, int heads, int hd, int pos0, float theta, int inverse, int dtype, hipStream_t st);
int av_swiglu_fwd(const void* gu, void* h, long M, int F, int dtype, hipStream_t st);
int av_swiglu_bwd(const void* dh, const void* gu, void* dgu, long M, int F, int dtype, hipStream_t st);
int av_swiglu_bwd_h(const void* dh, const void* gu, void* dgu, void* h, long M, int F, int dtype, hipStream_t st);
int av_attention_fwd_form(int B, int Tq, int Tk, int hd, int causal, int dtype, int impl);
int av_attention_bwd_form(int hd, int dtype, int impl);
int av_attention_fwd_ref(const void* q, const void* k, const void* v, void* o, float* lse, int B, int Tq, int Tk, int H,
                         int hd, long ldq, long ldk, long ldv, long ldo, float scale, int causal, int dtype, hipStream_t st, int G);
int av_attention_delta(const void* o, const void* dout, float* delta, int B, int T, int H, int hd, long ldo, long lddo, int dtype, hipStream_t st);
int av_attention_bwd_ref(const void* q, const void* k, const void* v, const void* dout, const float* lse, const float* delta,
                         void* dq, void* dk, void* dv, int B, int T, int H, int hd, long ldq, long ldk, long ldv, long lddo,
                         long lddq, long lddk, long lddv, float scale, int causal, int dtype, hipStream_t st, int G);
int av_attention_bwd_mfma(const void* q, const void* k, const void* v, const void* dout, const float* lse, float* delta,
                          void* dq, void* dk, void* dv, int B, int T, int H, int hd, long ldq, long ldk, long ldv, long lddo,
                          long lddq, long lddk, long lddv, float scale, int causal, hipStream_t st, int G, const void* o, long ldo, const float* rope_tab);
bool av_attention_fwd_mxq_ok(int B, int T, int H, int hd, int dtype, int kv_heads);
int av_attention_fwd_mxq(const void* q, const void* k, const void* v, void* oq, long ldoq, void* osc, int B, int T, int H, int hd, long ldq, long ldk,
                         long ldv, float scale, hipStream_t st);
int av_attention_fwd(const void* q, const void* k, const void* v, void* o, float* lse, int B, int Tq, int Tk, int H,
                     int hd, long ldq, long ldk, long ldv, long ldo, float scale, int causal, int dtype, int impl,
                     hipStream_t st, int kv_heads = 0);
int av_attention_bwd(const void* q, const void* k, const void* v, const void* o, const void* dout, const float* lse,
                     void* dq, void* dk, void* dv, float* delta_ws, int B, int T, int H, int hd, long ldq, long ldk,
                     long ldv, long ldo, long lddq, long lddk, long lddv, float scale, int causal, int dtype, int impl,
                     hipStream_t st, int kv_heads = 0, const float* rope_tab = nullptr);
bool av_attention_bwd_fuses_rope(int dtype, int hd, int impl);
int av_ce_fwd(const void* logits, long ld, const int64_t* labels, int B, int T, int V, float* row_lse, float* loss_sum,
              float* count, int dtype, hipStream_t st);
int av_ce_bwd(const void* logits, long ld, const int64_t* labels, const float* row_lse, const float* count,
              float grad_scale, void* dlogits, int B, int T, int V, int dtype, hipStream_t st);
int av_argmax_rows(const void* logits, long ld, long rows, int V, int64_t* out, int dtype, hipStream_t st);
int av_sample_rows(const void* logits, long ld, long rows, int V, float temperature, int top_k, float top_p, uint32_t seed,
                   const uint32_t* row_seeds, int step, const int* step_dev, uint8_t* unfinished, long long eos, long long pad,
                   int64_t* out, float* out_logprob, int dtype, hipStream_t st);
int av_row_scores(const void* logits, long ld, long rows, int V, const int64_t* tokens, float temperature, float* out_logprob, float* out_entropy,
                  int logprobs, int dtype, hipStream_t st);
size_t av_beam_topk_workspace_bytes(long rows, int V, int k);
int av_beam_topk(const float* logits, long ld, int B, int nb, int V, const float* beam_scores, int k, float* out_scores, int32_t* out_beams,
                 int64_t* out_tokens, void* ws, size_t ws_bytes, int logprobs, hipStream_t st);
int av_logits_process(const avllm_logits_proc_desc* d, hipStream_t st);
int av_kv_gather_rows(const void* k_src, const void* v_src, int src_rows, long src_T, void* k_dst, void* v_dst, int dst_rows, long dst_T,
                      int layers, int dkv, const int32_t* parent, int t0, int t1, int dtype, hipStream_t st);
int av_embedding(const void* table, const int64_t* ids, void* out, long n, int d, int dtype, hipStream_t st);
int av_cast(const void* src, int sdt, void* dst, int ddt, long n, hipStream_t st);
int av_whisper_im2col1(const float* mel, void* cols, int B, int n_mels, int T, int Kpad, int dtype, hipStream_t st);
int av_whisper_im2col2(const void* h, void* cols, int B, int T, int d, int dtype, hipStream_t st);
int av_clip_patchify(const void* frames, void* cols, int N, int S, int p, int Kpad, int dtype, hipStream_t st, int in_dtype = AV_F32);
int av_clip_cls_rows(const void* class_emb, const void* pos, void* x, int N, int tokens, int d, int dtype, hipStream_t st);
int av_fuse_pool(const void* a, int Ta, const void* v, int Tv, const void* prompt_emb, int P, void* out, int B, int L,
                 int S_out, int D, float fs, int dtype, hipStream_t st);
int av_fuse_pool_bwd(const void* dx, void* da, int Ta, void* dv, int Tv, int P, int B, int L, int S_out, int D, float fs, int dtype, hipStream_t st);
int av_fuse_pool_rows(const void* a, int Ta, const void* v, int Tv, const void* prompt_emb, int P, const int* mode, void* out, int B, int L,
                      int S_out, int D, float fs, int dtype, hipStream_t st);
int av_fuse_pool_rows_bwd(const void* dx, void* da, int Ta, void* dv, int Tv, int P, const int* mode, int B, int L, int S_out, int D, float fs,
                          int dtype, hipStream_t st);
int av_modality_draw(const int* mode_in, int* mode_out, int B, float p_drop_audio, float p_drop_video, uint32_t seed, const uint32_t* seed_dev,
                     hipStream_t st);
int av_gemm_wgrad(const void* dY, long ldy, const void* X, long ldx, int M, int N, int K, float* dW, long ldw, float* db, float alpha, int dtype,
                  hipStream_t st);
int av_grad_sumsq_det_multi(const float* const* g, const int64_t* n, int nbuf, float* partials, int nparts, float* sumsq, hipStream_t st);
int av_adamw_step_multi(const avllm_adamw_seg* segs, int nseg, float lr, float b1, float b2, float eps, int step, const float* sumsq, float max_norm,
                        float grad_prescale, const float* guard, float* skipped, const avllm_step_state* state, hipStream_t st);
int av_grad_sumsq(const float* g, long n, float* sumsq, hipStream_t st);
int av_grad_sumsq_det(const float* g, long n, float* partials, int nparts, float* sumsq, hipStream_t st);
int av_adamw_step(float* p, const float* g, float* m, float* v, long n, float lr, float b1, float b2, float eps,
                  float wd, int step, const float* sumsq, float max_norm, float grad_prescale, const float* guard, float* skipped,
                  const avllm_step_state* state, hipStream_t st);
int av_lora_pack(const float* A, const float* Bm, int r, int din, int dout, void* A_pad, void* AT_pad, long ld_at,
                 void* B_pad, void* BT_pad, int dtype, hipStream_t st);
int av_lora_merge(void* W, long ldw, int N, int K, const float* A, const float* B, int r, float scale, int dtype, hipStream_t st);
int av_kv_append(const void* k, const void* v, long ld, void* kc, void* vc, int B, int T, int pos0, int Tmax, int d,
                 int dtype, hipStream_t st);
int av_attention_decode(const void* q, long ldq, const void* kc, const void* vc, void* o, long ldo, int B, int H, int hd,
                        int Tk, int Tmax, float scale, int dtype, hipStream_t st, int G = 1);
int av_attention_decode1(const void* q, long ldq, const void* kc, const void* vc, void* o, long ldo, int B, int H, int hd, int Tk, const int* tk_dev,
                         int Tmax, float scale, int dtype, hipStream_t st, int G);
int av_kv8_append(const void* k, const void* v, long ld, void* kq, void* ke, void* vq, void* ve, int B, int T, int pos0, int Tmax, int dkv, hipStream_t st);
int av_kv8_rope_append(void* qkv, long ld, int B, int H, int Hkv, int hd, const float* rope, int rotate, void* kq, void* ke, void* vq, void* ve, int Tmax,
                       int pos, const int* pos_dev, hipStream_t st);
int av_attention_decode_kv8(const void* q, long ldq, const void* kq, const void* ke, const void* vq, const void* ve, void* o, long ldo, int B, int H, int hd,
                            int Tk, const int* tk_dev, int Tmax, float scale, int G, hipStream_t st);
size_t av_attention_decode_shared_ws(int R, int H, int hd);
int av_attention_decode_shared(const void* q, long ldq, const void* kp, const void* vp, int S, int Tp, const void* ks, const void* vs, int Tk, const int* tk_dev,
                               int N, void* o, long ldo, int R, int group, int H, int hd, float scale, int GQ, void* ws, size_t ws_bytes, hipStream_t st);
int av_attention_decode_shared_kv8(const void* q, long ldq, const void* kpq, const void* kpe, const void* vpq, const void* vpe, int S, int Tp, const void* ksq,
                                   const void* kse, const void* vsq, const void* vse, int Tk, const int* tk_dev, int N, void* o, long ldo, int R, int group, int H,
                                   int hd, float scale, int GQ, void* ws, size_t ws_bytes, hipStream_t st);
int av_kv8_gather_rows(const void* k_src, const void* v_src, int src_rows, long src_T, void* k_dst, void* v_dst, int dst_rows, long dst_T, int layers,
                       int dkv, const int32_t* parent, int t0, int t1, hipStream_t st);
int av_norm_mxq(const void* x, const void* w, const void* b, void* y, float* rstd_out, void* q, long ldq, void* scales, long rows, int d, float eps,
                hipStream_t st);
bool av_lora_batch_supported(int dtype, int R, int nj);
int av_lora_rank3(const void* const* A, const long* lda, const int* K, const void* const* B, const long* ldb, void* const* C, const long* ldc,
                  const uint32_t* seeds, int nj, int M, int R, float alpha, float p, const uint32_t* seed_dev, int shared, int dtype, hipStream_t st);
int av_gemm_tn_multi(const void* Big, long ldb, int NB, const void* const* Small, const long* lds, float* const* out, const long* ldo,
                     const int* col0, const int* ncol, const uint32_t* seeds, int nj, int R, int M, float alpha, float p,
                     const uint32_t* seed_dev, int shared, int dtype, hipStream_t st);
bool av_dec_proj_supported(int dtype, int M, int K, int N, int mode, int hd);
int av_dec_proj(const avllm_dec_proj_desc* d, hipStream_t st);
struct AvRopeScale { float factor = 1.f, low_freq_factor = 1.f, high_freq_factor = 4.f; int orig_ctx = 0; };
int av_rope_table(float* tab, int T, int hd, int pos0, float theta, hipStream_t st, const int* pos_dev = nullptr, AvRopeScale sc = AvRopeScale());
int av_rope_tab(void* x, long ld, long rows, int T, int heads, int hd, const float* tab, int inverse, int dtype, hipStream_t st);
int av_qk_norm_rope(void* x, long ld, long M, int T, int H, int Hkv, int hd, const void* wq, const void* wk, float eps, const float* tab, void* pre,
                    float* rstd, void* kc, void* vc, int Tmax, int pos, const int* pos_dev, int dtype, hipStream_t st);
int av_qk_norm_bwd(void* dy, long ld, long M, int H, int Hkv, int hd, const void* wq, const void* wk, const void* pre, const float* rstd, int dtype,
                   hipStream_t st);
int av_dropout(const void* x, void* y, long rows, int d, uint32_t seed, float p, int dtype, hipStream_t st, const uint32_t* seed_dev = nullptr);
bool av_lora_dx_masked_supported(int dtype, int N, int r, const long* ldt, const long* ldat, int nj, long ldr, long ldo);
int av_lora_dx_masked(const void* const* T, const long* ldt, const void* const* AT, const long* ldat, const uint32_t* seeds, int nj, int r,
                      const void* R, long ldr, void* out, long ldo, int M, int N, float p, const uint32_t* seed_dev, int dtype, hipStream_t st);
int av_mx_quantize(const void* x, long ldx, int R, int K, void* q, long ldq, void* scales, int layout, int dtype, hipStream_t st);
int av_gemm_f8(const avllm_gemm_f8_desc* d, hipStream_t st);
int av_act_residual(const void* x, const void* r, void* y, long n, int act, int dtype, hipStream_t st);
int av_step_advance(avllm_step_state* state, const avllm_schedule* sched, hipStream_t st);
```

### audio-visual-llm_amd/csrc/common.h

```cpp
#pragma once
#include <cstdlib>
#include <hip/hip_runtime.h>
#include <stdint.h>
#include <stdio.h>
#include <math.h>

typedef __bf16 bf16;
typedef __attribute__((ext_vector_type(2))) __bf16 bf16x2;
typedef __attribute__((ext_vector_type(4))) __bf16 bf16x4;
typedef __attribute__((ext_vector_type(8))) __bf16 bf16x8;
typedef __attribute__((ext_vector_type(4))) short short4v;
typedef __attribute__((ext_vector_type(2))) float f32x2;
typedef __attribute__((ext_vector_type(4))) float f32x4;
typedef __attribute__((ext_vector_type(16))) float f32x16;
typedef __attribute__((ext_vector_type(4))) unsigned int u32x4;

#define AV_WAVE 64

enum AvKnob { AV_KNOB_DECODE_FUSED, AV_KNOB_DEC_AL, AV_KNOB_LORA_UNBATCHED, AV_KNOB_F8_UNFUSED_QUANT, AV_KNOB_F8_FAST, AV_KNOB_ATTN_SHORT,
              AV_KNOB_NARROW_EPILOGUE, AV_KNOB_TN_CHUNK, AV_KNOB_GEMM_DBG, AV_KNOB_GEMM_GW, AV_KNOB_GEMM_VARIANT, AV_KNOB_SHARED_SPLIT, AV_KNOB_COUNT };
int av_knob(int id);

#define AV_OK 0
#define AV_ERR_ARG 1
#define AV_ERR_HIP 2
#define AV_ERR_WORKSPACE 3
#define AV_ERR_UNSUPPORTED 4

extern "C" const char* avllm_last_error(void);
int av_set_error(int code, const char* fmt, ...);

#define AV_CHECK_ARG(cond, ...) \
    do { if (!(cond)) return av_set_error(AV_ERR_ARG, __VA_ARGS__); } while (0)
#define AV_HIP(expr) \
    do { hipError_t e_ = (expr); if (e_ != hipSuccess) return av_set_error(AV_ERR_HIP, "%s failed: %s (%s:%d)", #expr, hipGetErrorString(e_), __FILE__, __LINE__); } while (0)
#define AV_LAUNCH_CHECK() AV_HIP(hipGetLastError())
#define AV_TRY(expr) do { int rc_ = (expr); if (rc_ != AV_OK) return rc_; } while (0)

enum { AV_F32 = 0, AV_BF16 = 1 };
enum { AV_ACT_NONE = 0, AV_ACT_GELU = 1, AV_ACT_QUICK_GELU = 2, AV_ACT_SILU = 3 };

static inline size_t av_dtype_size(int dt) { return dt == AV_F32 ? 4 : 2; }

template <typename T> struct Vec;

__device__ __forceinline__ float to_f(float x) { return x; }
__device__ __forceinline__ float to_f(bf16 x) { return (float)x; }
template <typename T> __device__ __forceinline__ T from_f(float x);
template <> __device__ __forceinline__ float from_f<float>(float x) { return x; }
template <> __device__ __forceinline__ bf16 from_f<bf16>(float x) { return (bf16)x; }

template <typename T, int N> struct Pack { T v[N]; };

template <int N> __device__ __forceinline__ void load_f(const float* p, float (&o)[N]) {
    static_assert(N % 4 == 0, "");
#pragma unroll
    for (int i = 0; i < N; i += 4) { f32x4 t = *(const f32x4*)(p + i); o[i] = t[0]; o[i + 1] = t[1]; o[i + 2] = t[2]; o[i + 3] = t[3]; }
}
template <int N> __device__ __forceinline__ void load_f(const bf16* p, float (&o)[N]) {
    static_assert(N % 4 == 0, "");
    if constexpr (N % 8 == 0) {
#pragma unroll
        for (int i = 0; i < N; i += 8) { bf16x8 t = *(const bf16x8*)(p + i);
#pragma unroll
            for (int j = 0; j < 8; ++j) o[i + j] = (float)t[j]; }
    } else {
#pragma unroll
        for (int i = 0; i < N; i += 4) { bf16x4 t = *(const bf16x4*)(p + i);
#pragma unroll
            for (int j = 0; j < 4; ++j) o[i + j] = (float)t[j]; }
    }
}
template <int N> __device__ __forceinline__ void store_f(float* p, const float (&o)[N]) {
#pragma unroll
    for (int i = 0; i < N; i += 4) { f32x4 t = {o[i], o[i + 1], o[i + 2], o[i + 3]}; *(f32x4*)(p + i) = t; }
}
template <int N> __device__ __forceinline__ void store_f(bf16* p, const float (&o)[N]) {
    if constexpr (N % 8 == 0) {
#pragma unroll
        for (int i = 0; i < N; i += 8) { bf16x8 t;
#pragma unroll
            for (int j = 0; j < 8; ++j) t[j] = (bf16)o[i + j];
            *(bf16x8*)(p + i) = t; }
    } else {
#pragma unroll
        for (int i = 0; i < N; i += 4) { bf16x4 t;
#pragma unroll
            for (int j = 0; j < 4; ++j) t[j] = (bf16)o[i + j];
            *(bf16x4*)(p + i) = t; }
    }
}

__device__ __forceinline__ float wave_sum(float v) {
#pragma unroll
    for (int o = 32; o > 0; o >>= 1) v += __shfl_xor(v, o);
    return v;
}
__device__ __forceinline__ float wave_max(float v) {
#pragma unroll
    for (int o = 32; o > 0; o >>= 1) v = fmaxf(v, __shfl_xor(v, o));
    return v;
}
__device__ __forceinline__ float block_sum(float v, float* red) {
    v = wave_sum(v);
    const int w = threadIdx.x >> 6, nw = (blockDim.x + 63) >> 6;
    __syncthreads();
    if ((threadIdx.x & 63) == 0) red[w] = v;
    __syncthreads();
    float t = 0.f;
    for (int i = 0; i < nw; ++i) t += red[i];
    return t;
}
__device__ __forceinline__ float block_max(float v, float* red) {
    v = wave_max(v);
    const int w = threadIdx.x >> 6, nw = (blockDim.x + 63) >> 6;
    __syncthreads();
    if ((threadIdx.x & 63) == 0) red[w] = v;
    __syncthreads();
    float t = -INFINITY;
    for (int i = 0; i < nw; ++i) t = fmaxf(t, red[i]);
    return t;
}

__device__ __forceinline__ float act_apply(float x, int act) {
    switch (act) {
        case AV_ACT_GELU: return 0.5f * x * (1.0f + erff(x * 0.70710678118654752f));
        case AV_ACT_QUICK_GELU: return x / (1.0f + __expf(-1.702f * x));
        case AV_ACT_SILU: return x / (1.0f + __expf(-x));
        default: return x;
    }
}
__device__ __forceinline__ float act_apply_fast(float x, int act) {
    switch (act) {
        case AV_ACT_GELU: {
            const float z = fabsf(x) * 0.70710678118654752f;
            const float t = __builtin_amdgcn_rcpf(1.0f + 0.3275911f * z);
            const float poly = t * (0.254829592f + t * (-0.284496736f + t * (1.421413741f + t * (-1.453152027f + t * 1.061405429f))));
            const float erf_abs = 1.0f - poly * __builtin_amdgcn_exp2f(-z * z * 1.4426950408889634f);
            return 0.5f * x * (1.0f + copysignf(erf_abs, x));
        }
        case AV_ACT_QUICK_GELU: return x * __builtin_amdgcn_rcpf(1.0f + __builtin_amdgcn_exp2f(-1.702f * 1.4426950408889634f * x));
        case AV_ACT_SILU: return x * __builtin_amdgcn_rcpf(1.0f + __builtin_amdgcn_exp2f(-1.4426950408889634f * x));
        default: return x;
    }
}

__host__ __device__ __forceinline__ uint32_t av_hash32(uint32_t x) {
    x ^= x >> 16; x *= 0x7feb352dU; x ^= x >> 15; x *= 0x846ca68bU; x ^= x >> 16;
    return x;
}
__host__ __device__ __forceinline__ uint32_t av_drop_thr(float p) { return (uint32_t)(p * 65536.0f); }
__host__ __device__ __forceinline__ float av_drop_scale(float p) { return 1.0f / (1.0f - (float)av_drop_thr(p) * (1.0f / 65536.0f)); }
__host__ __device__ __forceinline__ uint32_t av_pair_hash(uint32_t seed, unsigned long long pair) {
    const uint32_t hi = (uint32_t)(pair >> 32);
    uint32_t inner = av_hash32(seed);
    if (__builtin_expect(hi != 0u, 0)) inner = av_hash32(seed + hi * 0x9E3779B9U);
    return av_hash32((uint32_t)pair ^ inner);
}
__host__ __device__ __forceinline__ bool av_keep(uint32_t seed, unsigned long long idx, float p) {
    const uint32_t h = av_pair_hash(seed, idx >> 1);
    return ((idx & 1) ? (h >> 16) : (h & 0xffffu)) >= av_drop_thr(p);
}
__device__ __forceinline__ uint32_t av_seed(const uint32_t* seed_dev, uint32_t off) { return (seed_dev ? *seed_dev : 0u) + off; }
__device__ __forceinline__ void av_mask8(float (&v)[8], uint32_t seed, unsigned long long idx0, uint32_t thr, float sc) {
    const unsigned long long p0 = idx0 >> 1;
    if (__builtin_expect(((p0 + 3) >> 32) == 0, 1)) {
        const uint32_t inner = av_hash32(seed);
#pragma unroll
        for (int q = 0; q < 4; ++q) {
            const uint32_t h = av_hash32(((uint32_t)p0 + q) ^ inner);
            v[2 * q] = (h & 0xffffu) >= thr ? v[2 * q] * sc : 0.f;
            v[2 * q + 1] = (h >> 16) >= thr ? v[2 * q + 1] * sc : 0.f;
        }
        return;
    }
#pragma unroll
    for (int q = 0; q < 4; ++q) {
        const uint32_t h = av_pair_hash(seed, p0 + q);
        v[2 * q] = (h & 0xffffu) >= thr ? v[2 * q] * sc : 0.f;
        v[2 * q + 1] = (h >> 16) >= thr ? v[2 * q + 1] * sc : 0.f;
    }
}

static inline int av_cdiv(long a, long b) { return (int)((a + b - 1) / b); }
```

### audio-visual-llm_amd/csrc/engine.hip

```cpp
#include "common.h"
#include "avllm_internal.h"

namespace {

struct Bump {
    char* base; size_t cap; size_t off = 0; bool ok = true;
    Bump(void* p, size_t c) : base((char*)p), cap(c) {}
    void* take(size_t bytes) {
        const size_t a = (off + 255) & ~(size_t)255;
        if (a + bytes > cap) { ok = false; off = a + bytes; return base; }
        off = a + bytes;
        return base + a;
    }
};
inline size_t bump_size(const Bump& b) { return ((b.off + 255) & ~(size_t)255) + 256; }

inline avllm_gemm_desc gemm_desc(int dtype, const void* A, long lda, const void* B, long ldb, void* C, long ldc, int M, int N, int K) {
    avllm_gemm_desc g = {};
    g.A = A; g.B = B; g.C = C; g.lda = lda; g.ldb = ldb; g.ldc = ldc; g.M = M; g.N = N; g.K = K;
    g.dtype = dtype; g.alpha = 1.0f;
    return g;
}

inline AvRopeScale llama_rope_scale(const avllm_llama* m) {
    AvRopeScale sc;
    sc.factor = m->rope_factor; sc.low_freq_factor = m->rope_low_freq_factor; sc.high_freq_factor = m->rope_high_freq_factor; sc.orig_ctx = m->rope_orig_ctx;
    return sc;
}

struct F8Buf { void* q = nullptr; void* s = nullptr; };
void carve_f8(Bump& b, F8Buf& f, long M, int kmax) {
    f.q = b.take((size_t)M * kmax);
    f.s = b.take(avllm_mx_scale_bytes((int)M, kmax));
}
inline int f8_quant(const F8Buf& f, const void* x, long ldx, int M, int K, hipStream_t st) {
    return av_mx_quantize(x, ldx, M, K, f.q, K, f.s, 0, AV_BF16, st);
}
inline int f8_proj(const F8Buf& f, int M, int K, const void* W8, const void* S8, int N, void* C, long ldc, const void* bias, int act, const void* R,
                   long ldr, hipStream_t st) {
    avllm_gemm_f8_desc d = {};
    d.A = f.q; d.SA = f.s; d.B = W8; d.SB = S8; d.C = C; d.bias = bias; d.R = R;
    d.lda = K; d.ldb = K; d.ldc = ldc; d.ldr = ldr; d.M = M; d.N = N; d.K = K; d.act = act;
    return av_gemm_f8(&d, st);
}

struct Frozen { const void *W, *W8, *S8, *bias; };
int linear(int dtype, const F8Buf* f8, bool quantised, const Frozen& w, const void* x, long ldx, int M, int K, int N, void* y, long ldy, int act,
           const void* R, long ldr, hipStream_t st) {
    if (f8) {
        if (!quantised) AV_TRY(f8_quant(*f8, x, ldx, M, K, st));
        return f8_proj(*f8, M, K, w.W8, w.S8, N, y, ldy, w.bias, act, R, ldr, st);
    }
    avllm_gemm_desc g = gemm_desc(dtype, x, ldx, w.W, K, y, ldy, M, N, K);
    g.bias = w.bias; g.act = act; g.R = R; g.ldr = ldr;
    return av_gemm(&g, st);
}

struct EncBuf { void *x, *xn, *qkv, *att, *ff, *xc, *xcn; F8Buf f8; };
void carve_enc(Bump& b, EncBuf& e, long M, long cls_rows, int d, int ffn, size_t es, bool fp8) {
    e.x = b.take((size_t)M * d * es);
    e.xn = b.take((size_t)M * d * es);
    e.qkv = b.take((size_t)M * 3 * d * es);
    e.att = b.take((size_t)M * d * es);
    e.ff = b.take((size_t)M * ffn * es);
    if (cls_rows) {
        e.xc = b.take((size_t)cls_rows * d * es);
        e.xcn = b.take((size_t)cls_rows * d * es);
    }
    if (fp8) carve_f8(b, e.f8, M, ffn > d ? ffn : d);
}

int encoder_layers(int dtype, const avllm_enc_layer* L, int layers, int d, int heads, int ffn, int tokens, long items,
                   float eps, int act, const EncBuf& b, bool cls_only_last, void* cls_out, hipStream_t st, bool fp8 = false) {
    const long M = items * tokens;
    const int hd = d / heads;
    const size_t es = av_dtype_size(dtype);
    for (int l = 0; l < layers; ++l) {
        const avllm_enc_layer& P = L[l];
        AV_CHECK_ARG(!fp8 || (P.wqkv8 && P.sqkv8 && P.wo8 && P.so8 && P.w18 && P.s18 && P.w28 && P.s28), "encoder layer %d: fp8 mode without fp8 weight images", l);
        const F8Buf* fq = fp8 ? &b.f8 : nullptr;
        const bool nq = fp8 && d % 128 == 0 && d <= 8192 && !av_knob(AV_KNOB_F8_UNFUSED_QUANT);
        if (nq) AV_TRY(av_norm_mxq(b.x, P.ln1_w, P.ln1_b, nullptr, nullptr, b.f8.q, d, b.f8.s, M, d, eps, st));
        else AV_TRY(av_layernorm(b.x, P.ln1_w, P.ln1_b, b.xn, M, d, eps, dtype, st));
        AV_TRY(linear(dtype, fq, nq, {P.wqkv, P.wqkv8, P.sqkv8, P.bqkv}, b.xn, d, (int)M, d, 3 * d, b.qkv, 3 * d, AV_ACT_NONE, nullptr, 0, st));
        const char* qkv = (const char*)b.qkv;
        const bool cls = cls_only_last && l == layers - 1;
        const bool att_q = fp8 && !cls && av_attention_fwd_mxq_ok((int)items, tokens, heads, hd, dtype, heads);
        if (att_q) AV_TRY(av_attention_fwd_mxq(qkv, qkv + (size_t)d * es, qkv + (size_t)2 * d * es, b.f8.q, d, b.f8.s, (int)items, tokens, heads, hd,
                                               3 * d, 3 * d, 3 * d, 1.0f / sqrtf((float)hd), st));
        else
        AV_TRY(av_attention_fwd(qkv, qkv + (size_t)d * es, qkv + (size_t)2 * d * es, b.att, nullptr, (int)items, tokens, tokens,
                                heads, hd, 3 * d, 3 * d, 3 * d, d, 1.0f / sqrtf((float)hd), 0, dtype, 0, st));
        if (cls) fq = nullptr;
        const int rows = cls ? (int)items : (int)M;
        const long ldx = cls ? (long)tokens * d : d;
        void* x1 = cls ? b.xc : b.x;
        void* xn = cls ? b.xcn : b.xn;
        void* out = cls ? cls_out : b.x;
        AV_TRY(linear(dtype, fq, att_q, {P.wo, P.wo8, P.so8, P.bo}, b.att, ldx, rows, d, d, x1, d, AV_ACT_NONE, b.x, ldx, st));
        const bool nq2 = nq && !cls;
        if (nq2) AV_TRY(av_norm_mxq(x1, P.ln2_w, P.ln2_b, nullptr, nullptr, b.f8.q, d, b.f8.s, rows, d, eps, st));
        else AV_TRY(av_layernorm(x1, P.ln2_w, P.ln2_b, xn, rows, d, eps, dtype, st));
        if (fq) {
            if (!nq2) AV_TRY(f8_quant(*fq, xn, d, rows, d, st));
            avllm_gemm_f8_desc q1 = {};
            q1.A = b.f8.q; q1.SA = b.f8.s; q1.B = P.w18; q1.SB = P.s18; q1.bias = P.b1; q1.lda = d; q1.ldb = d; q1.M = rows; q1.N = ffn; q1.K = d; q1.act = act;
            F8Buf ffq;
            ffq.q = b.ff; ffq.s = (char*)b.ff + (((size_t)M * ffn + 255) & ~(size_t)255);
            q1.Cq = ffq.q; q1.SCq = ffq.s; q1.ldcq = ffn;
            if (!av_knob(AV_KNOB_F8_UNFUSED_QUANT) && avllm_gemm_f8_takes_quantised_output(&q1) && (size_t)M * ffn + 256 + avllm_mx_scale_bytes((int)M, ffn) <= (size_t)M * ffn * es) {
                AV_TRY(av_gemm_f8(&q1, st));
                AV_TRY(linear(dtype, &ffq, true, {P.w2, P.w28, P.s28, P.b2}, b.ff, ffn, rows, ffn, d, out, d, AV_ACT_NONE, x1, d, st));
                continue;
            }
        }
        AV_TRY(linear(dtype, fq, true, {P.w1, P.w18, P.s18, P.b1}, xn, d, rows, d, ffn, b.ff, ffn, act, nullptr, 0, st));
        AV_TRY(linear(dtype, fq, false, {P.w2, P.w28, P.s28, P.b2}, b.ff, ffn, rows, ffn, d, out, d, AV_ACT_NONE, x1, d, st));
    }
    return AV_OK;
}

struct WhisperWs { void *cols1, *h1, *cols2; EncBuf e; };
void carve_whisper(const avllm_whisper* w, int B, Bump& b, WhisperWs& s) {
    const size_t es = av_dtype_size(w->dtype);
    const long T2 = 2L * w->n_ctx, M = (long)B * w->n_ctx;
    s.cols1 = b.take((size_t)B * T2 * w->k1pad * es);
    s.h1 = b.take((size_t)B * T2 * w->d * es);
    s.cols2 = b.take((size_t)M * 3 * w->d * es);
    carve_enc(b, s.e, M, 0, w->d, w->ffn, es, w->fp8 != 0);
}

struct ClipWs { void* cols; EncBuf e; };
void carve_clip(const avllm_clip* c, int N, Bump& b, ClipWs& s, int& kpad) {
    const size_t es = av_dtype_size(c->dtype);
    const int g = c->image / c->patch;
    kpad = (3 * c->patch * c->patch + 63) / 64 * 64;
    s.cols = b.take((size_t)N * g * g * kpad * es);
    carve_enc(b, s.e, (long)N * c->tokens, N, c->d, c->ffn, es, c->fp8 != 0);
}

inline int llama_kv_heads(const avllm_llama* m) { return m->kv_heads > 0 ? m->kv_heads : m->heads; }
inline int llama_dkv(const avllm_llama* m) { return llama_kv_heads(m) * (m->d / m->heads); }
inline int llama_qw(const avllm_llama* m) { return m->d + 2 * llama_dkv(m); }
inline int llama_off(const avllm_llama* m, int j) { return j == 0 ? 0 : (j == 1 ? m->d : m->d + llama_dkv(m)); }
inline int llama_wid(const avllm_llama* m, int j) { return j == 0 ? m->d : llama_dkv(m); }
inline const void* llama_bias(const avllm_llama* m, const avllm_llama_layer& P, int j) {
    return P.bqkv ? (const char*)P.bqkv + (size_t)llama_off(m, j) * av_dtype_size(m->dtype) : nullptr;
}

inline bool llama_qk_norm(const avllm_llama* m) { return m->layer && m->layer[0].q_norm_w != nullptr; }
inline bool layer_mlp_lora(const avllm_llama_layer& P) { return P.lora_mlp[0].A_pad || P.lora_mlp[1].A_pad || P.lora_mlp[2].A_pad; }
inline bool llama_mlp_lora(const avllm_llama* m, int k0 = 0, int k1 = 3) {
    if (!m->layer) return false;
    for (int l = 0; l < m->layers; ++l)
        for (int k = k0; k < k1; ++k)
            if (m->layer[l].lora_mlp[k].A_pad) return true;
    return false;
}
inline bool lora_mask_fusable(const avllm_llama* m, int K) { return m->dtype == AV_BF16 && K % 256 == 0 && m->lora_r <= 16; }

struct LlamaLayerAct {
    void *xn1, *qkv, *att, *tqkv, *to, *h1, *gu;
    float *rstd1, *rstd2, *lse;
    void* qk_pre; float* qk_rstd;
    void *tgu, *tdown;
};
struct LlamaTrainWs {
    void** resid;
    LlamaLayerAct* act;
    void *xn2, *hmid, *xf, *logits, *xd;
    float *rstd_f, *row_lse, *delta, *rope_tab;
    void *dres, *dxn, *dgu, *dhmid, *dqkv, *datt, *dtqkv, *dto;
    F8Buf f8;
    void *dtgu, *dtdown;
    void* xdf;
};

void carve_llama_train(const avllm_llama* m, int B, int S, Bump& b, LlamaTrainWs& w, void** resid, LlamaLayerAct* act) {
    const size_t es = av_dtype_size(m->dtype);
    const long M = (long)B * S;
    const int d = m->d, f = m->ffn;
    w.resid = resid; w.act = act;
    for (int l = 0; l <= m->layers; ++l) resid[l] = b.take((size_t)M * d * es);
    for (int l = 0; l < m->layers; ++l) {
        LlamaLayerAct& a = act[l];
        a.xn1 = b.take((size_t)M * d * es);
        a.qkv = b.take((size_t)M * llama_qw(m) * es);
        a.att = b.take((size_t)M * d * es);
        a.tqkv = b.take((size_t)M * 3 * AVLLM_LORA_PAD * es);
        a.to = b.take((size_t)M * AVLLM_LORA_PAD * es);
        a.h1 = b.take((size_t)M * d * es);
        a.gu = b.take((size_t)M * 2 * f * es);
        a.rstd1 = (float*)b.take((size_t)M * 4);
        a.rstd2 = (float*)b.take((size_t)M * 4);
        a.lse = (float*)b.take((size_t)B * m->heads * S * 4);
    }
    w.xn2 = b.take((size_t)M * d * es);
    w.hmid = b.take((size_t)M * f * es);
    w.xf = b.take((size_t)M * d * es);
    w.logits = b.take((size_t)M * m->vocab * es);
    w.xd = b.take((size_t)M * d * es);
    w.rstd_f = (float*)b.take((size_t)M * 4);
    w.row_lse = (float*)b.take((size_t)M * 4);
    w.delta = (float*)b.take((size_t)B * m->heads * S * 4);
    w.rope_tab = (float*)b.take((size_t)S * (d / m->heads) * 4);
    w.dres = b.take((size_t)M * d * es);
    w.dxn = b.take((size_t)M * d * es);
    w.dgu = b.take((size_t)M * 2 * f * es);
    w.dhmid = b.take((size_t)M * f * es);
    w.dqkv = b.take((size_t)M * llama_qw(m) * es);
    w.datt = b.take((size_t)M * d * es);
    w.dtqkv = b.take((size_t)M * 3 * AVLLM_LORA_PAD * es);
    w.dto = b.take((size_t)M * AVLLM_LORA_PAD * es);
    if (m->fp8) carve_f8(b, w.f8, M, f > d ? f : d);
    for (int l = 0; l < m->layers; ++l) {
        act[l].qk_pre = nullptr; act[l].qk_rstd = nullptr;
        if (!llama_qk_norm(m)) continue;
        act[l].qk_pre = b.take((size_t)M * (d + llama_dkv(m)) * es);
        act[l].qk_rstd = (float*)b.take((size_t)M * (m->heads + llama_kv_heads(m)) * 4);
    }
    w.dtgu = w.dtdown = w.xdf = nullptr;
    const bool mlp = llama_mlp_lora(m);
    for (int l = 0; l < m->layers; ++l) {
        act[l].tgu = act[l].tdown = nullptr;
        if (!mlp) continue;
        act[l].tgu = b.take((size_t)M * 2 * AVLLM_LORA_PAD * es);
        act[l].tdown = b.take((size_t)M * AVLLM_LORA_PAD * es);
    }
    if (mlp) {
        w.dtgu = b.take((size_t)M * 2 * AVLLM_LORA_PAD * es);
        w.dtdown = b.take((size_t)M * AVLLM_LORA_PAD * es);
        if (llama_mlp_lora(m, 2, 3) && !lora_mask_fusable(m, f)) w.xdf = b.take((size_t)M * f * es);
    }
}
struct LlamaTrainFrame {
    Bump b; LlamaTrainWs w; void* resid[257]; LlamaLayerAct act[256];
    LlamaTrainFrame(const avllm_llama* m, int B, int S, void* ws, size_t ws_bytes) : b(ws, ws_bytes) { carve_llama_train(m, B, S, b, w, resid, act); }
};

int check_llama(const avllm_llama* m) {
    AV_CHECK_ARG(m && m->layer && m->embed && m->norm_w && m->lm_head, "llama: null model fields");
    AV_CHECK_ARG(m->d % m->heads == 0 && m->d % 64 == 0 && m->ffn % 64 == 0, "llama: d=%d ffn=%d must be multiples of 64", m->d, m->ffn);
    AV_CHECK_ARG(m->layers > 0 && m->layers <= 256, "llama: layers=%d", m->layers);
    AV_CHECK_ARG(m->kv_heads >= 0 && (m->kv_heads == 0 || m->heads % m->kv_heads == 0), "llama: heads=%d kv_heads=%d", m->heads, m->kv_heads);
    for (int l = 0; l < m->layers; ++l) {
        const avllm_llama_layer& P = m->layer[l];
        AV_CHECK_ARG((P.q_norm_w != nullptr) == (P.k_norm_w != nullptr) && (P.q_norm_w != nullptr) == llama_qk_norm(m),
                     "llama layer %d: q_norm_w and k_norm_w go together, on every layer or on none", l);
    }
    AV_CHECK_ARG(!llama_qk_norm(m) || m->d / m->heads == 64 || m->d / m->heads == 128, "llama: q/k head norms need a head dim of 64 or 128 (%d)", m->d / m->heads);
    AV_CHECK_ARG(!m->fp8 || !llama_mlp_lora(m), "llama: fp8 mode does not take adapters on gate_proj / up_proj / down_proj (lora_mlp)");
    if (m->fp8)
        for (int l = 0; l < m->layers; ++l) {
            const avllm_llama_layer& P = m->layer[l];
            AV_CHECK_ARG(P.wqkv8 && P.sqkv8 && P.wo8 && P.so8 && P.wgu8 && P.sgu8 && P.wdown8 && P.sdown8, "llama layer %d: fp8 mode without fp8 weight images", l);
        }
    if (m->decode_fp8 || m->decode_fp4) {
        AV_CHECK_ARG(!(m->decode_fp8 && m->decode_fp4), "llama: decode_fp4 and decode_fp8 are two forms of the same token step, set one");
        const bool f4 = m->decode_fp4 != 0;
        const char* mode = f4 ? "decode_fp4" : "decode_fp8";
        AV_CHECK_ARG(m->dtype == AV_BF16 && m->d % 128 == 0 && m->ffn % 128 == 0 && m->vocab % 16 == 0 && m->lm_head8 && m->elm_head8,
                     "llama: %s needs bf16, d and ffn multiples of 128, vocab a multiple of 16 and the e4m3 lm_head codes + exponents", mode);
        for (int l = 0; l < m->layers; ++l) {
            const avllm_llama_layer& P = m->layer[l];
            AV_CHECK_ARG(f4 ? P.wqkv4 && P.eqkv4 && P.wo4 && P.eo4 && P.wgu4 && P.egu4 && P.wdown4 && P.edown4
                            : P.wqkv8 && P.eqkv8 && P.wo8 && P.eo8 && P.wgu8 && P.egu8 && P.wdown8 && P.edown8,
                         "llama layer %d: %s without the %s codes and their exponents", l, mode, f4 ? "MXFP4" : "fp8");
        }
    }
    return AV_OK;
}

struct LoraDrop {
    float p; bool fused;
    float fused_p() const { return fused ? p : 0.f; }
};
inline LoraDrop lora_drop(const avllm_llama* m, int K) {
    const float p = m->lora_dropout > 0.f ? m->lora_dropout : 0.f;
    return {p, p > 0.f && lora_mask_fusable(m, K)};
}
inline LoraDrop lora_drop(const avllm_llama* m) { return lora_drop(m, m->d); }
inline uint32_t lora_seed(const avllm_llama* m, int l, int j) {
    return j < 4 ? m->dropout_seed + 4u * l + j : m->dropout_seed + 4u * m->layers + 3u * l + (j - 4);
}
int lora_input(const avllm_llama* m, const LoraDrop& dr, const void* x, void* xd, int M, int K, uint32_t seed, const void*& xl, hipStream_t st) {
    xl = x;
    if (dr.p > 0.f && !dr.fused) {
        AV_CHECK_ARG(xd, "llama: no dropout buffer for an adapter input of width %d", K);
        AV_TRY(av_dropout(x, xd, M, K, seed, dr.p, m->dtype, st, m->dropout_seed_dev));
        xl = xd;
    }
    return AV_OK;
}

struct LoraView {
    const avllm_lora_mod* mod;
    uint32_t seed;
    void *t, *dt; long ldt;
    int off, wid;
    bool at_slice;
    int K;
};
inline LoraView lora_view(const avllm_llama* m, int l, int j, const LlamaLayerAct& a, const LlamaTrainWs& w) {
    const avllm_lora_mod* lora = m->layer[l].lora;
    const size_t es_ = av_dtype_size(m->dtype);
    if (j >= 4) {
        const avllm_lora_mod* lm = m->layer[l].lora_mlp;
        const int k = j - 4;
        if (k == 2) return {&lm[2], lora_seed(m, l, j), a.tdown, w.dtdown, AVLLM_LORA_PAD, 0, m->d, false, m->ffn};
        const size_t slot = (size_t)k * AVLLM_LORA_PAD * es_;
        LoraView g = {&lm[k], lora_seed(m, l, j), a.tgu ? (char*)a.tgu + slot : nullptr, w.dtgu ? (char*)w.dtgu + slot : nullptr, 2 * AVLLM_LORA_PAD,
                      k * m->ffn, m->ffn, false, m->d};
        g.at_slice = lm[k].ld_at == 2 * AVLLM_LORA_PAD && (const char*)lm[k].AT_pad == (const char*)lm[0].AT_pad + slot;
        return g;
    }
    LoraView v = {&lora[j], lora_seed(m, l, j), a.to, w.dto, AVLLM_LORA_PAD, 0, m->d, false, m->d};
    if (j < 3) {
        const size_t es = av_dtype_size(m->dtype), slot = (size_t)j * AVLLM_LORA_PAD * es;
        v.t = (char*)a.tqkv + slot; v.dt = (char*)w.dtqkv + slot; v.ldt = 3 * AVLLM_LORA_PAD;
        v.off = llama_off(m, j); v.wid = llama_wid(m, j);
        v.at_slice = lora[j].ld_at == 3 * AVLLM_LORA_PAD && (const char*)lora[j].AT_pad == (const char*)lora[0].AT_pad + slot;
    }
    return v;
}

int lora_linear(const avllm_llama* m, const void* x, int K, const void* W, const void* bias, int N, const avllm_lora_mod& lm, const void* xl,
                uint32_t a_seed, float a_p, void* t, long ldt, bool have_t, void* y, long ldy, const void* R, long ldr, int M, hipStream_t st) {
    avllm_gemm_desc g;
    const bool has = lm.A_pad != nullptr;
    if (has && !have_t) {
        g = gemm_desc(m->dtype, xl, K, lm.A_pad, K, t, ldt, M, AVLLM_LORA_PAD, K);
        g.alpha = m->lora_scale;
        g.a_drop_seed = a_seed; g.a_drop_p = a_p; g.seed_dev = m->dropout_seed_dev;
        g.n_valid = m->lora_r;
        AV_TRY(av_gemm(&g, st));
    }
    if (W) {
        g = gemm_desc(m->dtype, x, K, W, K, y, ldy, M, N, K);
        if (has) { g.A2 = t; g.lda2 = ldt; g.B2 = lm.B_pad; g.ldb2 = AVLLM_LORA_PAD; g.K2 = AVLLM_LORA_PAD; }
        g.R = R; g.ldr = ldr; g.bias = bias;
    } else {
        if (!has) return AV_OK;
        g = gemm_desc(m->dtype, t, ldt, lm.B_pad, AVLLM_LORA_PAD, y, ldy, M, N, AVLLM_LORA_PAD);
        g.R = y; g.ldr = ldy;
    }
    return av_gemm(&g, st);
}

int lora_wgrad(const avllm_llama* m, const LoraDrop& dr, const LoraView& v, const void* dy, long ldy, const void* x, void* xd, int M, hipStream_t st) {
    const avllm_lora_mod& lm = *v.mod;
    const int dt = m->dtype, d = v.K, R = m->lora_r;
    AV_TRY(av_gemm_tn(dy, ldy, v.wid, v.t, v.ldt, R, M, lm.gB, R, 1.0f, dt, st));
    avllm_gemm_desc gt = gemm_desc(dt, dy, ldy, lm.BT_pad, v.wid, v.dt, v.ldt, M, AVLLM_LORA_PAD, v.wid);
    gt.alpha = m->lora_scale; gt.n_valid = R;
    AV_TRY(av_gemm(&gt, st));
    const void* xin;
    AV_TRY(lora_input(m, dr, x, xd, M, d, v.seed, xin, st));
    return av_gemm_tn(v.dt, v.ldt, R, xin, d, d, M, lm.gA, d, 1.0f, dt, st, v.seed, dr.fused_p(), m->dropout_seed_dev);
}

int lora_dx_dropped(const avllm_llama* m, const LoraDrop& dr, const LoraView* v, int n, void* dx, int M, hipStream_t st, int d_in = 0) {
    const int dt = m->dtype, d = d_in ? d_in : m->d;
    const void* Tp[3]; const void* Ap[3]; long lt[3], la[3]; uint32_t sd[3]; int nj = 0;
    for (int j = 0; j < n; ++j) {
        if (!v[j].mod->A_pad) continue;
        Tp[nj] = v[j].dt; lt[nj] = v[j].ldt; Ap[nj] = v[j].mod->AT_pad; la[nj] = v[j].mod->ld_at; sd[nj] = v[j].seed; ++nj;
    }
    if (dr.fused && av_lora_dx_masked_supported(dt, d, m->lora_r, lt, la, nj, d, d))
        return av_lora_dx_masked(Tp, lt, Ap, la, sd, nj, m->lora_r, dx, d, dx, d, M, d, dr.p, m->dropout_seed_dev, dt, st);
    for (int k = 0; k < nj; ++k) {
        avllm_gemm_desc gm = gemm_desc(dt, Tp[k], lt[k], Ap[k], la[k], dx, d, M, d, AVLLM_LORA_PAD);
        gm.R = dx; gm.ldr = d; gm.drop_seed = sd[k]; gm.drop_p = dr.p; gm.seed_dev = m->dropout_seed_dev;
        AV_TRY(av_gemm(&gm, st));
    }
    return AV_OK;
}

int llama_mlp_lora_bwd(const avllm_llama* m, int l, LlamaTrainWs& w, avllm_gemm_desc gd, int M, hipStream_t st) {
    const avllm_llama_layer& P = m->layer[l];
    LlamaLayerAct& a = w.act[l];
    const int dt = m->dtype, d = m->d, f = m->ffn, R = m->lora_r;
    const size_t es = av_dtype_size(dt);
    const LoraDrop dr = lora_drop(m), drf = lora_drop(m, f);
    const bool drop = dr.p > 0.f;
    const LoraView vm[3] = {lora_view(m, l, 4, a, w), lora_view(m, l, 5, a, w), lora_view(m, l, 6, a, w)};
    const bool down = vm[2].mod->A_pad != nullptr;
    if (down) {
        const avllm_lora_mod& lm = *vm[2].mod;
        AV_TRY(av_gemm_tn(w.dres, d, d, vm[2].t, vm[2].ldt, R, M, lm.gB, R, 1.0f, dt, st));
        avllm_gemm_desc gt = gemm_desc(dt, w.dres, d, lm.BT_pad, d, vm[2].dt, vm[2].ldt, M, AVLLM_LORA_PAD, d);
        gt.alpha = m->lora_scale; gt.n_valid = R;
        AV_TRY(av_gemm(&gt, st));
        if (!drop) { gd.A2 = vm[2].dt; gd.lda2 = vm[2].ldt; gd.B2 = lm.AT_pad; gd.ldb2 = lm.ld_at; gd.K2 = AVLLM_LORA_PAD; }
    }
    AV_TRY(av_gemm(&gd, st));
// ... 600 lines not shown
```

### include/avllm.h

```cpp
#ifndef AVLLM_H
#define AVLLM_H
#include <stddef.h>
#include <stdint.h>
#ifdef __cplusplus
extern "C" {
#endif

#define AVLLM_F32 0
#define AVLLM_BF16 1
#define AVLLM_ACT_NONE 0
#define AVLLM_ACT_GELU 1
#define AVLLM_ACT_QUICK_GELU 2
#define AVLLM_ACT_SILU 3
#define AVLLM_LORA_PAD 64

const char* avllm_last_error(void);
int avllm_version(void);


typedef struct avllm_gemm_desc {
    const void* A;  const void* B;
    const void* A2; const void* B2;
    void* C;
    const void* bias;
    const void* R;
    int64_t lda, ldb, lda2, ldb2, ldc, ldr;
    int32_t M, N, K, K2;
    int32_t dtype;
    int32_t out_f32;
    int32_t act;
    float alpha;
    int32_t r_mod;
    int32_t g_in, g_out, g_off;
    uint32_t drop_seed;
    float drop_p;
    uint32_t a_drop_seed;
    float a_drop_p;
    int32_t n_valid;
    const uint32_t* seed_dev;
} avllm_gemm_desc;
int avllm_gemm(const avllm_gemm_desc* d, void* stream);
enum { AVLLM_GEMM_SMALLM, AVLLM_GEMM_SKINNY64, AVLLM_GEMM_128, AVLLM_GEMM_RING, AVLLM_GEMM_H16, AVLLM_GEMM_HP16, AVLLM_GEMM_W4, AVLLM_GEMM_WP4,
       AVLLM_GEMM_DP, AVLLM_GEMM_F32, AVLLM_GEMM_KERNELS };
int avllm_gemm_plan(const avllm_gemm_desc* d, int32_t* kernel);
int avllm_set_gemm_variant(int v);
int avllm_set_knob(const char* name, int32_t value);
int avllm_get_knob(const char* name, int32_t* value);

int avllm_gemm_tn(const void* P, int64_t ldp, int32_t I, const void* Q, int64_t ldq, int32_t J, int32_t M,
                  float* out, int64_t ldo, float alpha, int32_t dtype, void* stream);
int avllm_gemm_tn_drop(const void* P, int64_t ldp, int32_t I, const void* Q, int64_t ldq, int32_t J, int32_t M,
                       float* out, int64_t ldo, float alpha, uint32_t drop_seed, float drop_p, int32_t dtype, void* stream);

int avllm_gemm_wgrad(const void* dY, int64_t ldy, const void* X, int64_t ldx, int32_t M, int32_t N, int32_t K, float* dW, int64_t ldw,
                     float* db, float alpha, int32_t dtype, void* stream);

int avllm_lora_rank3(const void* const* A, const int64_t* lda, const int32_t* K, const void* const* B, const int64_t* ldb, void* const* C,
                     const int64_t* ldc, const uint32_t* seeds, int32_t nj, int32_t M, int32_t R, float alpha, float p,
                     const uint32_t* seed_dev, int32_t shared, int32_t dtype, void* stream);
int avllm_gemm_tn_multi(const void* Big, int64_t ldb, int32_t NB, const void* const* Small, const int64_t* lds, float* const* out,
                        const int64_t* ldo, const int32_t* col0, const int32_t* ncol, const uint32_t* seeds, int32_t nj, int32_t R,
                        int32_t M, float alpha, float p, const uint32_t* seed_dev, int32_t shared, int32_t dtype, void* stream);

int avllm_lora_dx_masked(const void* const* T, const int64_t* ldt, const void* const* AT, const int64_t* ldat, const uint32_t* seeds,
                         int32_t nj, int32_t r, const void* R, int64_t ldr, void* out, int64_t ldo, int32_t M, int32_t N, float p,
                         const uint32_t* seed_dev, int32_t dtype, void* stream);

size_t avllm_mx_scale_bytes(int32_t R, int32_t K);
int avllm_mx_quantize(const void* x, int64_t ldx, int32_t R, int32_t K, void* q, int64_t ldq, void* scales, int32_t layout, int32_t dtype,
                      void* stream);
int avllm_mx4_quantize(const void* x, int64_t ldx, int32_t R, int32_t K, void* q, int64_t ldq, void* exps, int32_t dtype, void* stream);
typedef struct avllm_gemm_f8_desc {
    const void* A;  const void* SA;
    const void* B;  const void* SB;
    void* C;
    const void* bias;
    const void* R;
    int64_t lda, ldb, ldc, ldr;
    int32_t M, N, K;
    int32_t act;
    void* Cq; void* SCq;
    int64_t ldcq;
} avllm_gemm_f8_desc;
int avllm_gemm_f8_takes_quantised_output(const avllm_gemm_f8_desc* d);
int avllm_gemm_f8_takes_fast(const avllm_gemm_f8_desc* d);
int avllm_gemm_f8(const avllm_gemm_f8_desc* d, void* stream);
int avllm_norm_mxq(const void* x, const void* w, const void* b, void* y, float* rstd_out, void* q, int64_t ldq, void* scales, int64_t rows,
                   int32_t d, float eps, void* stream);

typedef struct avllm_step_state {
    uint32_t step;
    uint32_t dropout_seed;
    float lr, bc1, bc2_sqrt;
    float skipped;
    uint32_t reserved[2];
} avllm_step_state;
typedef struct avllm_schedule {
    float base_lr, beta1, beta2;
    int32_t warmup_steps, total_steps;
    uint32_t rank;
} avllm_schedule;
int avllm_step_advance(avllm_step_state* state_dev, const avllm_schedule* sched, void* stream);

int avllm_im2col_k3(const void* x, void* cols, int32_t B, int32_t T, int32_t C, int32_t stride, int32_t dtype, void* stream);
int avllm_groupnorm_tokens(const void* x, const void* w, const void* b, void* y, int32_t B, int32_t T, int32_t C, int32_t groups,
                           float eps, int32_t act, int32_t dtype, void* stream);

int avllm_layernorm(const void* x, const void* w, const void* b, void* y, int64_t rows, int32_t d, float eps,
                    int32_t dtype, void* stream);
int avllm_rmsnorm_fwd(const void* x, const void* w, void* y, float* rstd, int64_t rows, int32_t d, float eps,
                      int32_t dtype, void* stream);
int avllm_rmsnorm_bwd(const void* dy, const void* x, const void* w, const float* rstd, const void* dres_in,
                      void* dx_out, int64_t rows, int32_t d, int32_t dtype, void* stream);
int avllm_rope(void* x, int64_t ld, int64_t rows, int32_t T, int32_t heads, int32_t hd, int32_t pos0, float theta,
               int32_t inverse, int32_t dtype, void* stream);
int avllm_rope_table(float* tab, int32_t T, int32_t hd, int32_t pos0, float theta, const int32_t* pos_dev, float factor,
                     float low_freq_factor, float high_freq_factor, int32_t orig_ctx, void* stream);
int avllm_rope_tab(void* x, int64_t ld, int64_t rows, int32_t T, int32_t heads, int32_t hd, const float* tab, int32_t inverse,
                   int32_t dtype, void* stream);
int avllm_swiglu_fwd(const void* gu, void* h, int64_t M, int32_t F, int32_t dtype, void* stream);
int avllm_swiglu_bwd(const void* dh, const void* gu, void* dgu, int64_t M, int32_t F, int32_t dtype, void* stream);
int avllm_swiglu_bwd_h(const void* dh, const void* gu, void* dgu, void* h, int64_t M, int32_t F, int32_t dtype, void* stream);
int avllm_attention_fwd(const void* q, const void* k, const void* v, void* o, float* lse, int32_t B, int32_t Tq,
                        int32_t Tk, int32_t H, int32_t hd, int64_t ldq, int64_t ldk, int64_t ldv, int64_t ldo,
                        float scale, int32_t causal, int32_t dtype, int32_t impl, int32_t kv_heads, void* stream);
int avllm_attention_bwd(const void* q, const void* k, const void* v, const void* o, const void* dout,
                        const float* lse, void* dq, void* dk, void* dv, float* delta_ws, int32_t B, int32_t T,
                        int32_t H, int32_t hd, int64_t ldq, int64_t ldk, int64_t ldv, int64_t ldo, int64_t lddq,
                        int64_t lddk, int64_t lddv, float scale, int32_t causal, int32_t dtype, int32_t impl,
                        int32_t kv_heads, void* stream);
int avllm_attention_bwd_rope(const void* q, const void* k, const void* v, const void* o, const void* dout,
                             const float* lse, void* dq, void* dk, void* dv, float* delta_ws, int32_t B, int32_t T,
                             int32_t H, int32_t hd, int64_t ldq, int64_t ldk, int64_t ldv, int64_t ldo, int64_t lddq,
                             int64_t lddk, int64_t lddv, float scale, int32_t causal, int32_t dtype, int32_t impl,
                             int32_t kv_heads, const float* rope_tab, void* stream);
enum { AVLLM_ATTN_REF, AVLLM_ATTN_SHORT13X7, AVLLM_ATTN_SHORT17X9, AVLLM_ATTN_MFMA64X4, AVLLM_ATTN_MFMA128X4, AVLLM_ATTN_FORMS };
int avllm_attention_plan(int32_t B, int32_t Tq, int32_t Tk, int32_t H, int32_t hd, int32_t causal, int32_t dtype, int32_t impl, int32_t kv_heads,
                         int32_t* fwd_form, int32_t* bwd_form);
int avllm_attention_fwd_mxq_ok(int32_t B, int32_t T, int32_t H, int32_t hd, int32_t dtype, int32_t kv_heads);
int avllm_attention_bwd_fuses_rope(int32_t dtype, int32_t hd, int32_t impl);
int avllm_ce_fwd(const void* logits, int64_t ld, const int64_t* labels, int32_t B, int32_t T, int32_t V,
                 float* row_lse, float* loss_sum, float* count, int32_t dtype, void* stream);
int avllm_attention_fwd_mxq(const void* q, const void* k, const void* v, void* oq, int64_t ldoq, void* scales, int32_t B, int32_t T, int32_t H,
                            int32_t hd, int64_t ldq, int64_t ldk, int64_t ldv, float scale, void* stream);
int avllm_ce_bwd(const void* logits, int64_t ld, const int64_t* labels, const float* row_lse, const float* count,
                 float grad_scale, void* dlogits, int32_t B, int32_t T, int32_t V, int32_t dtype, void* stream);
int avllm_argmax_rows(const void* logits, int64_t ld, int64_t rows, int32_t V, int64_t* out, int32_t dtype, void* stream);
int avllm_sample_rows(const void* logits, int64_t ld, int64_t rows, int32_t V, float temperature, int32_t top_k, float top_p, uint32_t seed,
                      const uint32_t* row_seeds, int32_t step, const int32_t* step_dev, uint8_t* unfinished, int64_t eos, int64_t pad,
                      int64_t* out, int32_t dtype, void* stream);
int avllm_sample_rows_scored(const void* logits, int64_t ld, int64_t rows, int32_t V, float temperature, int32_t top_k, float top_p, uint32_t seed,
                             const uint32_t* row_seeds, int32_t step, const int32_t* step_dev, uint8_t* unfinished, int64_t eos, int64_t pad,
                             int64_t* out, float* out_logprob, int32_t dtype, void* stream);
int avllm_row_scores(const void* logits, int64_t ld, int64_t rows, int32_t V, const int64_t* tokens, float temperature, float* out_logprob,
                     float* out_entropy, int32_t dtype, void* stream);
int avllm_row_scores_logprobs(const void* logprobs, int64_t ld, int64_t rows, int32_t V, const int64_t* tokens, float* out_logprob,
                              float* out_entropy, int32_t dtype, void* stream);
size_t avllm_beam_topk_workspace_bytes(int64_t rows, int32_t V, int32_t k);
int avllm_beam_topk(const float* logits, int64_t ld, int32_t B, int32_t num_beams, int32_t V, const float* beam_scores, int32_t k,
                    float* out_scores, int32_t* out_beams, int64_t* out_tokens, void* ws, size_t ws_bytes, void* stream);
int avllm_beam_topk_logprobs(const float* logprobs, int64_t ld, int32_t B, int32_t num_beams, int32_t V, const float* beam_scores, int32_t k,
                             float* out_scores, int32_t* out_beams, int64_t* out_tokens, void* ws, size_t ws_bytes, void* stream);
int avllm_logits_process(void* scores, int64_t ld, int64_t rows, int32_t V, int64_t* history, int64_t ldh, const int64_t* append, int32_t cur,
                         const int32_t* cur_dev, float repetition_penalty, int32_t no_repeat_ngram_size, int32_t min_new_tokens, int64_t eos,
                         int32_t log_softmax, int32_t dtype, void* stream);
#define AVLLM_LOGITS_MAX_SEQUENCES 4096
#define AVLLM_LOGITS_MAX_SEQUENCE_LEN 16
typedef struct avllm_logits_proc_desc {
    void* scores; int64_t ld; int64_t rows; int32_t V; int32_t dtype;
    int64_t* history; int64_t ldh; const int64_t* append; int32_t cur; const int32_t* cur_dev;
    float repetition_penalty; int32_t no_repeat_ngram_size; int32_t min_new_tokens; int64_t eos; int32_t log_softmax;
    const int32_t* bias_tokens; const int32_t* bias_lengths; const float* bias_values; int32_t n_bias; int32_t bias_max_len;
    const int32_t* bad_tokens; const int32_t* bad_lengths; int32_t n_bad; int32_t bad_max_len;
    const int32_t* suppress; int32_t n_suppress;
    const int32_t* begin_suppress; int32_t n_begin_suppress;
} avllm_logits_proc_desc;
int avllm_logits_process_ex(const avllm_logits_proc_desc* d, void* stream);
int avllm_kv_gather_rows(const void* k_src, const void* v_src, int32_t src_rows, int64_t src_T, void* k_dst, void* v_dst, int32_t dst_rows,
                         int64_t dst_T, int32_t layers, int32_t dkv, const int32_t* parent, int32_t t0, int32_t t1, int32_t dtype, void* stream);
int avllm_kv_append(const void* k, const void* v, int64_t ld, void* kc, void* vc, int32_t B, int32_t T, int32_t pos0, int32_t Tmax,
                    int32_t d, int32_t dtype, void* stream);
int avllm_embedding(const void* table, const int64_t* ids, void* out, int64_t n, int32_t d, int32_t dtype, void* stream);
int avllm_cast(const void* src, int32_t src_dtype, void* dst, int32_t dst_dtype, int64_t n, void* stream);
int avllm_act_residual(const void* x, const void* r, void* y, int64_t n, int32_t act, int32_t dtype, void* stream);
int avllm_dropout(const void* x, void* y, int64_t rows, int32_t d, uint32_t seed, float p, int32_t dtype, void* stream);

int avllm_whisper_im2col1(const float* mel, void* cols, int32_t B, int32_t n_mels, int32_t T, int32_t Kpad,
                          int32_t dtype, void* stream);
int avllm_whisper_im2col2(const void* h, void* cols, int32_t B, int32_t T, int32_t d, int32_t dtype, void* stream);
int avllm_clip_patchify(const float* frames, void* cols, int32_t N, int32_t S, int32_t p, int32_t Kpad, int32_t dtype,
                        void* stream);
int avllm_clip_cls_rows(const void* class_emb, const void* pos, void* x, int32_t N, int32_t tokens, int32_t d,
                        int32_t dtype, void* stream);
int avllm_fuse_pool(const void* a, int32_t Ta, const void* v, int32_t Tv, const void* prompt_emb, int32_t P,
                    void* out, int32_t B, int32_t L, int32_t S_out, int32_t D, float fusion_scale, int32_t dtype,
                    void* stream);
int avllm_fuse_pool_bwd(const void* dx, void* da, int32_t Ta, void* dv, int32_t Tv, int32_t P, int32_t B, int32_t L, int32_t S_out,
                        int32_t D, float fusion_scale, int32_t dtype, void* stream);
enum { AVLLM_MODE_BOTH = 0, AVLLM_MODE_AUDIO = 1, AVLLM_MODE_VIDEO = 2 };
int avllm_fuse_pool_rows(const void* a, int32_t Ta, const void* v, int32_t Tv, const void* prompt_emb, int32_t P, const int32_t* mode,
                         void* out, int32_t B, int32_t L, int32_t S_out, int32_t D, float fusion_scale, int32_t dtype, void* stream);
int avllm_fuse_pool_rows_bwd(const void* dx, void* da, int32_t Ta, void* dv, int32_t Tv, int32_t P, const int32_t* mode, int32_t B, int32_t L,
                             int32_t S_out, int32_t D, float fusion_scale, int32_t dtype, void* stream);
int avllm_modality_draw(const int32_t* mode_in, int32_t* mode_out, int32_t B, float p_drop_audio, float p_drop_video, uint32_t seed,
                        const uint32_t* seed_dev, void* stream);
int avllm_grad_sumsq(const float* g, int64_t n, float* sumsq, void* stream);
int avllm_grad_sumsq_det(const float* g, int64_t n, float* partials, int32_t nparts, float* sumsq, void* stream);
int avllm_adamw_step(float* p, const float* g, float* m, float* v, int64_t n, float lr, float beta1, float beta2,
                     float eps, float weight_decay, int32_t step, const float* sumsq, float max_norm,
                     float grad_prescale, const float* guard, float* skipped, const avllm_step_state* state_dev, void* stream);
int avllm_grad_sumsq_det_multi(const float* const* g, const int64_t* n, int32_t nbuf, float* partials, int32_t nparts, float* sumsq,
                               void* stream);
typedef struct avllm_adamw_seg {
    float *p, *m, *v;
    const float* g;
    int64_t n;
    float weight_decay;
    int32_t reserved;
} avllm_adamw_seg;
int avllm_adamw_step_multi(const avllm_adamw_seg* segs, int32_t nseg, float lr, float beta1, float beta2, float eps, int32_t step,
                           const float* sumsq, float max_norm, float grad_prescale, const float* guard, float* skipped,
                           const avllm_step_state* state_dev, void* stream);
int avllm_lora_pack(const float* A, const float* Bm, int32_t r, int32_t din, int32_t dout, void* A_pad, void* AT_pad,
                    int64_t ld_at, void* B_pad, void* BT_pad, int32_t dtype, void* stream);
typedef struct avllm_lora_pack_item {
    const float *A, *B;
    void *A_pad, *AT_pad, *B_pad, *BT_pad;
    int64_t ld_at, dout;
} avllm_lora_pack_item;
int avllm_lora_pack_batch(const avllm_lora_pack_item* items_dev, int32_t n, int32_t r, int32_t din, int32_t dtype, void* stream);
int avllm_lora_merge(void* W, int64_t ldw, int32_t N, int32_t K, const float* A, const float* B, int32_t r, float scale, int32_t dtype,
                     void* stream);


size_t avllm_logmel_table_bytes(void);
int avllm_logmel_table_init(void* table_dev, int32_t n_mels);
size_t avllm_logmel_workspace_bytes(int32_t B, int32_t n_mels);
int avllm_logmel(const void* table, const float* wave, int32_t B, int32_t n, int64_t ld, int32_t normalize, int32_t n_mels, float* out,
                 void* ws, size_t ws_bytes, void* stream);

size_t avllm_clip_preproc_plan_bytes(int32_t H, int32_t W, int32_t image);
int avllm_clip_preproc_plan_init(void* plan_dev, int32_t H, int32_t W, int32_t image, const float* mean3, const float* std3);
size_t avllm_clip_preproc_workspace_bytes(int32_t N, int32_t H, int32_t W, int32_t image);
int avllm_clip_preproc(const void* plan, const uint8_t* frames, int32_t N, int32_t H, int32_t W, int32_t image, void* out,
                       int32_t dtype, void* ws, size_t ws_bytes, void* stream);

typedef struct avllm_noise_info {
    int32_t applied;
    int32_t row, offset;
    float snr_db;
    float gain;
} avllm_noise_info;
int32_t avllm_wave_add_noise_chunk(void);
size_t avllm_wave_add_noise_workspace_bytes(int32_t B, int32_t n);
int avllm_wave_add_noise(const float* wave, int64_t ld, const int32_t* len, int32_t B, int32_t n, const float* noise, int64_t ld_noise,
                         const int32_t* noise_len, int32_t Nn, const float* snr_db, float snr_lo, float snr_hi, float p_apply, uint32_t seed,
                         const uint32_t* seed_dev, float* out, int64_t ld_out, avllm_noise_info* info, void* ws, size_t ws_bytes,
                         void* stream);
int avllm_spec_augment(float* feat, int32_t B, int32_t M, int32_t T, const int32_t* valid, int32_t n_time, int32_t max_time_width,
                       float max_time_ratio, int32_t n_freq, int32_t max_freq_width, float fill, uint32_t seed, const uint32_t* seed_dev,
                       int32_t* spans, void* stream);

int avllm_profile_begin(int32_t max_launches);
int avllm_profile_enable(int32_t on);
int avllm_profile_end(double* out);


typedef struct avllm_enc_layer {
    const void *ln1_w, *ln1_b;
    const void *wqkv, *bqkv;
    const void *wo, *bo;
    const void *ln2_w, *ln2_b;
    const void *w1, *b1, *w2, *b2;
    const void *wqkv8, *sqkv8, *wo8, *so8, *w18, *s18, *w28, *s28;
} avllm_enc_layer;

typedef struct avllm_whisper {
    int32_t dtype, d, heads, layers, ffn, n_mels, n_ctx, k1pad;
    const void *conv1_w, *conv1_b;
    const void *conv2_w, *conv2_b;
    const void* pos;
    const avllm_enc_layer* layer;
    const void *lnf_w, *lnf_b;
    int32_t fp8;
} avllm_whisper;
size_t avllm_whisper_workspace_bytes(const avllm_whisper* w, int32_t B);
int avllm_whisper_encoder_fwd(const avllm_whisper* w, const float* mel, int32_t B, void* out, void* ws,
                              size_t ws_bytes, void* stream);

typedef struct avllm_clip {
    int32_t dtype, d, heads, layers, ffn, image, patch, tokens;
    float eps;
    const void* patch_w;
    const void *class_emb, *pos;
    const void *pre_ln_w, *pre_ln_b;
    const avllm_enc_layer* layer;
    int32_t fp8;
    int32_t frames_bf16;
} avllm_clip;
size_t avllm_clip_workspace_bytes(const avllm_clip* c, int32_t N);
int avllm_clip_vision_cls_fwd(const avllm_clip* c, const void* frames, int32_t N, void* cls, void* ws,
                              size_t ws_bytes, void* stream);

typedef struct avllm_lora_mod {
    const void *A_pad, *AT_pad, *B_pad, *BT_pad;
    int64_t ld_at;
    float *gA, *gB;
} avllm_lora_mod;

typedef struct avllm_llama_layer {
    const void *ln1_w, *ln2_w;
    const void *wqkv;
    const void *wo;
    const void *wgu;
    const void *wdown;
    const void *wqkv_t;
    const void *wo_t;
    const void *wgu_t;
    const void *wdown_t;
    avllm_lora_mod lora[4];
    const void *wqkv8, *sqkv8, *wo8, *so8, *wgu8, *sgu8, *wdown8, *sdown8;
    const void *eqkv8, *eo8, *egu8, *edown8;
    const void *wqkv4, *wo4, *wgu4, *wdown4;
    const void *eqkv4, *eo4, *egu4, *edown4;
    const void *bqkv, *bo;
    const void *q_norm_w, *k_norm_w;
    avllm_lora_mod lora_mlp[3];
} avllm_llama_layer;

typedef struct avllm_llama {
    int32_t dtype, d, heads, layers, ffn, vocab, lora_r;
    int32_t kv_heads;
    float eps, theta, lora_scale;
    float lora_dropout;
    uint32_t dropout_seed;
    const uint32_t* dropout_seed_dev;
    const void* embed;
    const void* norm_w;
    const void* lm_head;
    const void* lm_head_t;
    const avllm_llama_layer* layer;
    int32_t fp8;
    const void *lm_head8, *slm_head8;
    float rope_factor, rope_low_freq_factor, rope_high_freq_factor;
    int32_t rope_orig_ctx;
    int32_t decode_fp8;
    const void* elm_head8;
    int32_t decode_fp4;
    int32_t kv_fp8;
} avllm_llama;

size_t avllm_llama_train_workspace_bytes(const avllm_llama* m, int32_t B, int32_t S);
int avllm_llama_lora_fwd_loss(const avllm_llama* m, const void* x, const int64_t* labels, int32_t B, int32_t S,
                              void* logits, float* loss_sum, float* count, void* ws, size_t ws_bytes, void* stream);
typedef void (*avllm_layer_cb)(int32_t layer, void* user);
int avllm_llama_lora_bwd(const avllm_llama* m, const int64_t* labels, int32_t B, int32_t S, const float* count,
                         float grad_scale, void* ws, size_t ws_bytes, avllm_layer_cb after_layer, void* user,
                         void* stream);
int avllm_llama_lora_bwd_layers(const avllm_llama* m, const int64_t* labels, int32_t B, int32_t S, const float* count,
                                float grad_scale, void* ws, size_t ws_bytes, int32_t layer_hi, int32_t layer_lo,
                                avllm_layer_cb after_layer, void* user, void* stream);
int avllm_llama_lora_bwd_layers_dx(const avllm_llama* m, const int64_t* labels, int32_t B, int32_t S, const float* count,
                                   float grad_scale, void* ws, size_t ws_bytes, int32_t layer_hi, int32_t layer_lo,
                                   avllm_layer_cb after_layer, void* user, void* dx_embeds, void* stream);

size_t avllm_llama_infer_workspace_bytes(const avllm_llama* m, int32_t B, int32_t S);
int avllm_llama_prefill(const avllm_llama* m, const void* x, int32_t B, int32_t S, void* kcache, void* vcache,
                        int32_t Tmax, float* logits_last, void* all_logits, void* ws, size_t ws_bytes, void* stream);
int avllm_llama_decode_step(const avllm_llama* m, const int64_t* ids, int32_t B, int32_t pos, void* kcache,
                            void* vcache, int32_t Tmax, float* logits, void* ws, size_t ws_bytes, void* stream);
int avllm_llama_decode_step_at(const avllm_llama* m, const int64_t* ids, int32_t B, int32_t pos, const int32_t* pos_dev, void* kcache,
                               void* vcache, int32_t Tmax, float* logits, void* ws, size_t ws_bytes, void* stream);
int avllm_llama_decode_is_fused(const avllm_llama* m, int32_t B);
int avllm_llama_decode_streams_fp8(const avllm_llama* m, int32_t B);
int avllm_llama_decode_streams_fp4(const avllm_llama* m, int32_t B);
int avllm_llama_decode_caches_fp8(const avllm_llama* m, int32_t B);
size_t avllm_llama_decode_shared_workspace_bytes(const avllm_llama* m, int32_t R);
int avllm_llama_decode_step_shared(const avllm_llama* m, const int64_t* ids, int32_t R, int32_t group, int32_t pos, const int32_t* pos_dev,
                                   const void* k_prefix, const void* v_prefix, int32_t S, void* k_suffix, void* v_suffix, int32_t N, float* logits,
                                   void* ws, size_t ws_bytes, void* stream);
int avllm_llama_decode_shares_prefix(const avllm_llama* m, int32_t R);
size_t avllm_llama_kv_cache_bytes(const avllm_llama* m, int32_t B, int32_t Tmax);

int avllm_kv8_append(const void* k, const void* v, int64_t ld, void* k_codes, void* k_exps, void* v_codes, void* v_exps, int32_t B, int32_t T,
                     int32_t pos0, int32_t Tmax, int32_t dkv, void* stream);
int avllm_kv8_rope_append(void* qkv, int64_t ld, int32_t B, int32_t heads, int32_t kv_heads, int32_t hd, const float* rope, int32_t rotate,
                          void* k_codes, void* k_exps, void* v_codes, void* v_exps, int32_t Tmax, int32_t pos, const int32_t* pos_dev, void* stream);
int avllm_attention_decode_kv8(const void* q, int64_t ldq, const void* k_codes, const void* k_exps, const void* v_codes, const void* v_exps, void* o,
                               int64_t ldo, int32_t B, int32_t H, int32_t hd, int32_t Tk, const int32_t* tk_dev, int32_t Tmax, float scale,
                               int32_t kv_group, void* stream);
size_t avllm_attention_decode_shared_workspace_bytes(int32_t R, int32_t H, int32_t hd);
int avllm_attention_decode_shared(const void* q, int64_t ldq, const void* k_prefix, const void* v_prefix, int32_t S, int32_t Tprefix,
                                  const void* k_suffix, const void* v_suffix, int32_t Tk, const int32_t* tk_dev, int32_t N, void* o, int64_t ldo,
                                  int32_t R, int32_t group, int32_t H, int32_t hd, float scale, int32_t kv_group, void* ws, size_t ws_bytes,
                                  void* stream);
int avllm_attention_decode_shared_kv8(const void* q, int64_t ldq, const void* kp_codes, const void* kp_exps, const void* vp_codes, const void* vp_exps,
                                      int32_t S, int32_t Tprefix, const void* ks_codes, const void* ks_exps, const void* vs_codes, const void* vs_exps,
                                      int32_t Tk, const int32_t* tk_dev, int32_t N, void* o, int64_t ldo, int32_t R, int32_t group, int32_t H,
                                      int32_t hd, float scale, int32_t kv_group, void* ws, size_t ws_bytes, void* stream);
int avllm_kv8_gather_rows(const void* k_src, const void* v_src, int32_t src_rows, int64_t src_T, void* k_dst, void* v_dst, int32_t dst_rows,
                          int64_t dst_T, int32_t layers, int32_t dkv, const int32_t* parent, int32_t t0, int32_t t1, void* stream);
int avllm_pos_advance(int32_t* pos_dev, int32_t by, void* stream);

typedef struct avllm_dec_proj_desc {
    const void* A; int64_t lda;
    const void* W; int64_t ldw;
    const void* norm_w; float eps;
    int32_t M, K, N, mode;
    void* C; int64_t ldc; int32_t out_f32;
    const void* R; int64_t ldr;
    int32_t dq, dkv, hd;
    const float* rope;
    void *kc, *vc;
    int32_t Tmax, pos;
    const int32_t* pos_dev;
    const float* lora_t; int64_t ld_lora_t;
    const void* lora_b[3];
    int32_t lora_r; float lora_scale;
    const void* W8; const void* E8;
    const void* W4;
    const void* bias;
    int32_t raw_qkv;
} avllm_dec_proj_desc;
int avllm_dec_proj(const avllm_dec_proj_desc* d, void* stream);
int avllm_qk_norm_rope(void* x, int64_t ld, int64_t rows, int32_t T, int32_t heads, int32_t kv_heads, int32_t hd, const void* q_norm_w,
                       const void* k_norm_w, float eps, const float* tab, void* pre, float* rstd, void* kc, void* vc, int32_t Tmax, int32_t pos,
                       const int32_t* pos_dev, int32_t dtype, void* stream);
int avllm_qk_norm_bwd(void* dy, int64_t ld, int64_t rows, int32_t heads, int32_t kv_heads, int32_t hd, const void* q_norm_w, const void* k_norm_w,
                      const void* pre, const float* rstd, int32_t dtype, void* stream);
int avllm_attention_decode(const void* q, int64_t ldq, const void* kc, const void* vc, void* o, int64_t ldo, int32_t B, int32_t H, int32_t hd,
                           int32_t Tk, const int32_t* tk_dev, int32_t Tmax, float scale, int32_t kv_group, int32_t dtype, void* stream);

#ifdef __cplusplus
// ... 4 lines not shown
```

Before: 91.84.

## Compute only CLS query block in last CLIP layer and share K/V LDS

In the final CLIP vision layer, where only the CLS token output is used, the QKV projection is split: K/V are projected for all tokens, Q only for the first token of each item. Attention runs only the first 16-row query block via a new nqb parameter. The short attention kernel is also reworked to reuse a single LDS region for K (sized by VROWS), defer V's LDS store when double occupancy fits, and use masked stores instead of branches. A knob CLIP_LAST_FULL restores the full path; the risk is subtle correctness in the masked/late-V LDS logic.

New measurement: 92.54, median of 6. Within noise of the previous version (+0.8%).

```diff
diff --git a/audio-visual-llm_amd/avllm/lib.py b/audio-visual-llm_amd/avllm/lib.py
--- a/audio-visual-llm_amd/avllm/lib.py
+++ b/audio-visual-llm_amd/avllm/lib.py
@@ -107,6 +107,7 @@
     "avllm_set_gemm_variant": ([i32], i32),
     "avllm_set_knob": ([C.c_char_p, i32], i32),
     "avllm_get_knob": ([C.c_char_p, C.POINTER(i32)], i32),
+    "avllm_attention_fwd_blocks": ([vp, vp, vp, vp, vp, i32, i32, i32, i32, i64, i64, i64, i64, f32, i32, i32, i32, vp], i32),
     "avllm_attention_fwd_mxq": ([vp, vp, vp, vp, i64, vp, i32, i32, i32, i32, i64, i64, i64, f32, vp], i32),
     "avllm_im2col_k3": ([vp, vp, i32, i32, i32, i32, i32, vp], i32),
     "avllm_groupnorm_tokens": ([vp, vp, vp, vp, i32, i32, i32, i32, f32, i32, i32, vp], i32),
diff --git a/audio-visual-llm_amd/avllm/ops.py b/audio-visual-llm_amd/avllm/ops.py
--- a/audio-visual-llm_amd/avllm/ops.py
+++ b/audio-visual-llm_amd/avllm/ops.py
@@ -161,11 +161,12 @@
     return L.ATTN_FORMS[f.value], (L.ATTN_FORMS[b.value] if b.value >= 0 else None)
 
 
-def attention_fwd(qkv, B, T, H, hd, causal, scale=None, impl=0, want_lse=True, kv_heads=None, Tk=None, k=None, v=None, out=None, plan=False):
+def attention_fwd(qkv, B, T, H, hd, causal, scale=None, impl=0, want_lse=True, kv_heads=None, Tk=None, k=None, v=None, out=None, plan=False, nqb=0):
     d = H * hd
     dkv = (kv_heads or H) * hd
     Tk = T if Tk is None else Tk
     assert (k is None) == (v is None) and (k is not None or Tk == T)
+    assert not nqb or (not causal and Tk == T and impl == 0)
     if plan:
         return attention_plan(B, T, Tk, H, hd, causal, L.dt_of(qkv), impl, kv_heads)[0]
     o = torch.empty(B * T, d, device=qkv.device, dtype=qkv.dtype) if out is None else out
@@ -179,6 +180,10 @@
     else:
         assert qkv.shape == (B * T, d) and k.shape == (B * Tk, dkv) and v.shape == k.shape and k.dtype == qkv.dtype and v.dtype == qkv.dtype
         pk, pv, ldk, ldv = L.ptr(k), L.ptr(v), _ld(k), _ld(v)
+    if nqb:
+        L.check(L.load().avllm_attention_fwd_blocks(p, pk, pv, L.ptr(o), L.ptr(lse), B, T, H, hd, _ld(qkv), ldk, ldv, _ld(o), scale, L.dt_of(qkv),
+                                                    kv_heads or 0, nqb, L.stream_ptr()))
+        return o, lse
     L.check(L.load().avllm_attention_fwd(p, pk, pv, L.ptr(o), L.ptr(lse), B, T, Tk, H, hd, _ld(qkv), ldk, ldv, _ld(o), scale, int(causal),
                                          L.dt_of(qkv), impl, kv_heads or 0, L.stream_ptr()))
     return o, lse
diff --git a/audio-visual-llm_amd/csrc/api.hip b/audio-visual-llm_amd/csrc/api.hip
--- a/audio-visual-llm_amd/csrc/api.hip
+++ b/audio-visual-llm_amd/csrc/api.hip
@@ -16,7 +16,7 @@
 #include <string.h>
 static const struct { const char* name; int dflt; } g_knob_def[AV_KNOB_COUNT] = {
     {"DECODE_FUSED", 1}, {"DEC_AL", 0}, {"LORA_UNBATCHED", 0}, {"F8_UNFUSED_QUANT", 0}, {"F8_FAST", 1}, {"ATTN_SHORT", 1},
-    {"NARROW_EPILOGUE", 0}, {"TN_CHUNK", 0}, {"GEMM_DBG", 0}, {"GEMM_GW", 0}, {"GEMM_VARIANT", 0}, {"SHARED_SPLIT", 0}};
+    {"NARROW_EPILOGUE", 0}, {"TN_CHUNK", 0}, {"GEMM_DBG", 0}, {"GEMM_GW", 0}, {"GEMM_VARIANT", 0}, {"SHARED_SPLIT", 0}, {"CLIP_LAST_FULL", 0}};
 static int g_knob[AV_KNOB_COUNT];
 static std::once_flag g_knob_once;
 static void knob_init() {
@@ -99,6 +99,10 @@
                         int32_t dtype, int32_t impl, int32_t kv_heads, void* stream) {
     return av_attention_fwd(q, k, v, o, lse, B, Tq, Tk, H, hd, ldq, ldk, ldv, ldo, scale, causal, dtype, impl, ST, kv_heads);
 }
+int avllm_attention_fwd_blocks(const void* q, const void* k, const void* v, void* o, float* lse, int32_t B, int32_t T, int32_t H, int32_t hd,
+                               int64_t ldq, int64_t ldk, int64_t ldv, int64_t ldo, float scale, int32_t dtype, int32_t kv_heads, int32_t nqb, void* stream) {
+    return av_attention_fwd(q, k, v, o, lse, B, T, T, H, hd, ldq, ldk, ldv, ldo, scale, 0, dtype, 0, ST, kv_heads, nqb);
+}
 int avllm_attention_bwd(const void* q, const void* k, const void* v, const void* o, const void* dout, const float* lse, void* dq,
                         void* dk, void* dv, float* delta_ws, int32_t B, int32_t T, int32_t H, int32_t hd, int64_t ldq, int64_t ldk,
                         int64_t ldv, int64_t ldo, int64_t lddq, int64_t lddk, int64_t lddv, float scale, int32_t causal,
diff --git a/audio-visual-llm_amd/csrc/attention.hip b/audio-visual-llm_amd/csrc/attention.hip
--- a/audio-visual-llm_amd/csrc/attention.hip
+++ b/audio-visual-llm_amd/csrc/attention.hip
@@ -167,49 +167,72 @@
     }
 }
 
+template <int NKB, int NW>
+constexpr int short_lds() { return 2 * ((NKB + 1) / 2) * 32 * 160 + NW * 16 * 80; }
+
 template <int NKB, int NW, bool QOUT, bool FULLK, bool WLSE>
 __global__ __launch_bounds__(NW * 64) void attn_fwd_short(const bf16* __restrict__ q, const bf16* __restrict__ k, const bf16* __restrict__ v,
                                                           bf16* __restrict__ o, float* __restrict__ lse, int T, int H, long ldq, long ldk,
                                                           long ldv, long ldo, float scale_log2e, int G, uint8_t* __restrict__ oq, long ldoq,
-                                                          uint8_t* __restrict__ osc, int RBo) {
+                                                          uint8_t* __restrict__ osc, int RBo, int nqb) {
     constexpr int HD = 64, KS = 160, VS = 160, OS = 80;
-    constexpr int NPV = (NKB + 1) / 2, KROWS = NKB * 16, VROWS = NPV * 32, NT = NW * 64;
+    constexpr int NPV = (NKB + 1) / 2, VROWS = NPV * 32, NT = NW * 64;
     constexpr int NQ = (NKB + NW - 1) / NW;
+    constexpr bool VLATE = 2 * short_lds<NKB, NW>() <= 160 * 1024;
     extern __shared__ __attribute__((aligned(16))) char smem[];
     char* k_lds = smem;
-    char* v_lds = smem + KROWS * KS;
+    char* v_lds = smem + VROWS * KS;
     const int tid = threadIdx.x, lane = tid & 63, w = tid >> 6;
-    char* o_lds = smem + KROWS * KS + VROWS * VS + w * 16 * OS;
+    char* o_lds = smem + VROWS * KS + VROWS * VS + w * 16 * OS;
     const int fr = lane & 15, fq = lane >> 4;
     const int hh = blockIdx.x, b = blockIdx.y, hk = hh / G;
     const int nkb = (T + 15) >> 4;
 
     constexpr int NCH = (VROWS * 8 + NT - 1) / NT;
+    static_assert(NCH * NT == VROWS * 8, "the workgroup's chunks tile the K and V images exactly: a row test on a store would let the compiler sink its load behind the test");
     u32x4 kreg[NCH], vreg[NCH];
+    unsigned keep[NCH];
+#pragma unroll
+    for (int i = 0; i < NCH; ++i) {
+        keep[i] = ((tid + i * NT) >> 3) < T ? 0xffffffffu : 0u;
+        asm volatile("" : "+v"(keep[i]));
+    }
 #pragma unroll
     for (int i = 0; i < NCH; ++i) {
         const int c = tid + i * NT, row = c >> 3, ch = c & 7;
-        kreg[i] = (u32x4){0u, 0u, 0u, 0u}; vreg[i] = (u32x4){0u, 0u, 0u, 0u};
-        if (row < T) {
-            kreg[i] = *(const u32x4*)(k + ((long)b * T + row) * ldk + (long)hk * HD + ch * 8);
-            vreg[i] = *(const u32x4*)(v + ((long)b * T + row) * ldv + (long)hk * HD + ch * 8);
-        }
-    }
+        kreg[i] = *(const u32x4*)(k + ((long)b * T + (row < T ? row : T - 1)) * ldk + (long)hk * HD + ch * 8);
+    }
+    typedef const __attribute__((address_space(1))) bf16* gq_ptr;
+    gq_ptr q_here = (gq_ptr)q;
+    asm volatile("" : "+s"(q_here));
     bf16x8 qf[NQ][2];
 #pragma unroll
     for (int i = 0; i < NQ; ++i) {
         int qrow = (w + NW * i) * 16 + fr;
         qrow = qrow < T ? qrow : T - 1;
-        const bf16* qp = q + ((long)b * T + qrow) * ldq + (long)hh * HD + 8 * fq;
-        qf[i][0] = *(const bf16x8*)qp;
-        qf[i][1] = *(const bf16x8*)(qp + 32);
+        const gq_ptr qp = q_here + ((long)b * T + qrow) * ldq + (long)hh * HD + 8 * fq;
+        qf[i][0] = *(const __attribute__((address_space(1))) bf16x8*)qp;
+        qf[i][1] = *(const __attribute__((address_space(1))) bf16x8*)(qp + 32);
     }
 #pragma unroll
     for (int i = 0; i < NCH; ++i) {
         const int c = tid + i * NT, row = c >> 3, ch = c & 7;
-        if (row < KROWS) *(u32x4*)(k_lds + row * KS + ch * 16) = kreg[i];
-        if (row < VROWS) *(u32x4*)(v_lds + row * VS + ch * 16) = vreg[i];
-    }
+        vreg[i] = *(const u32x4*)(v + ((long)b * T + (row < T ? row : T - 1)) * ldv + (long)hk * HD + ch * 8);
+    }
+    auto park_v = [&](bool sync) __attribute__((always_inline)) {
+#pragma unroll
+        for (int i = 0; i < NCH; ++i) {
+            const int c = tid + i * NT, row = c >> 3, ch = c & 7;
+            *(u32x4*)(v_lds + row * VS + ch * 16) = vreg[i] & (u32x4){keep[i], keep[i], keep[i], keep[i]};
+        }
+        if (sync) __syncthreads();
+    };
+#pragma unroll
+    for (int i = 0; i < NCH; ++i) {
+        const int c = tid + i * NT, row = c >> 3, ch = c & 7;
+        *(u32x4*)(k_lds + row * KS + ch * 16) = kreg[i] & (u32x4){keep[i], keep[i], keep[i], keep[i]};
+    }
+    if constexpr (!VLATE) park_v(false);
     __syncthreads();
 
     bf16x8 ones;
@@ -219,11 +242,8 @@
     const f32x4 zero4 = {0.f, 0.f, 0.f, 0.f};
     const int i16 = lane & 15, g = lane >> 4;
     auto max3 = [](float a, float x, float y) __attribute__((always_inline)) { return max3f(a, x, y); };
-    auto qblock = [&](int qi, auto fullc) __attribute__((always_inline)) {
+    auto scores = [&](int qi, auto fullc, f32x4 (&sc)[NKB]) __attribute__((always_inline)) -> float {
         constexpr bool FULL = decltype(fullc)::value;
-        const int qb = w + NW * qi;
-        const int q0 = qb * 16;
-        f32x4 sc[NKB];
 #pragma unroll
         for (int kb = 0; kb < NKB; ++kb) {
             sc[kb] = (f32x4){-INFINITY, -INFINITY, -INFINITY, -INFINITY};
@@ -253,7 +273,11 @@
         for (int kb = 0; kb < NKB; ++kb) { m = max3(m, sc[kb][0], sc[kb][1]); m = max3(m, sc[kb][2], sc[kb][3]); }
         m = max3(m, __shfl_xor(m, 16), m);
         m = max3(m, __shfl_xor(m, 32), m);
-        const float msc = m * scale_log2e;
+        return m * scale_log2e;
+    };
+    auto finish = [&](int qi, auto fullc, const f32x4 (&sc)[NKB], const float msc) __attribute__((always_inline)) {
+        constexpr bool FULL = decltype(fullc)::value;
+        const int q0 = (w + NW * qi) * 16;
         f32x4 lacc = zero4, oacc[4] = {zero4, zero4, zero4, zero4};
         float lsum = 0.f;
 #pragma unroll
@@ -323,26 +347,31 @@
             asm volatile("s_waitcnt lgkmcnt(0)" ::: "memory");
         }
     };
-    if constexpr (FULLK) {
-#pragma unroll
-        for (int qi = 0; qi < NQ; ++qi)
-            if (w + NW * qi < NKB) qblock(qi, std::true_type{});
-    } else {
-#pragma unroll
-        for (int qi = 0; qi < NQ; ++qi)
-            if (w + NW * qi < nkb) qblock(qi, std::false_type{});
-    }
+    auto run = [&](auto fullc) __attribute__((always_inline)) {
+        f32x4 sc[NKB];
+        float msc = 0.f;
+        const bool first = w < nqb;
+        if (first) msc = scores(0, fullc, sc);
+        if constexpr (VLATE) park_v(true);
+        if (first) finish(0, fullc, sc, msc);
+#pragma unroll
+        for (int qi = 1; qi < NQ; ++qi)
+            if (w + NW * qi < nqb) {
+                msc = scores(qi, fullc, sc);
+                finish(qi, fullc, sc, msc);
+            }
+    };
+    if constexpr (FULLK) run(std::true_type{});
+    else run(std::false_type{});
 }
 
 template <int NKB, int NW, bool QOUT, bool FULLK, bool WLSE, class... Args>
-int launch_short_form(int B, int H, hipStream_t st, Args... args) {
-    constexpr int LDS = NKB * 16 * 160 + ((NKB + 1) / 2) * 32 * 160 + NW * 16 * 80;
+int launch_short_form(int B, int H, int dev, hipStream_t st, Args... args) {
+    constexpr int LDS = short_lds<NKB, NW>();
     static bool attr[AV_MAX_DEVICES] = {};
-    int dev = 0;
-    AV_HIP(hipGetDevice(&dev));
-    if (!attr[dev & (AV_MAX_DEVICES - 1)]) {
+    if (!attr[dev]) {
         AV_HIP(hipFuncSetAttribute((const void*)attn_fwd_short<NKB, NW, QOUT, FULLK, WLSE>, hipFuncAttributeMaxDynamicSharedMemorySize, LDS));
-        attr[dev & (AV_MAX_DEVICES - 1)] = true;
+        attr[dev] = true;
     }
     hipLaunchKernelGGL((attn_fwd_short<NKB, NW, QOUT, FULLK, WLSE>), dim3(H, B), dim3(NW * 64), LDS, st, args...);
     AV_LAUNCH_CHECK();
@@ -351,14 +380,18 @@
 
 template <int NKB, int NW>
 int launch_fwd_short(const void* q, const void* k, const void* v, void* o, float* lse, int B, int T, int H, long ldq, long ldk, long ldv,
-                     long ldo, float scale, hipStream_t st, int G, void* oq = nullptr, long ldoq = 0, void* osc = nullptr) {
+                     long ldo, float scale, hipStream_t st, int G, int nqb = 0, void* oq = nullptr, long ldoq = 0, void* osc = nullptr) {
     AV_CHECK_ARG(!(oq && lse), "attention_fwd_short: the quantised-output form writes no LSE");
     const int RBo = oq ? (int)(((long)B * T + 255) / 256 * 4) : 0;
-    const bool fullk = ((T + 15) >> 4) == NKB;
+    const int nkb = (T + 15) >> 4;
+    const bool fullk = nkb == NKB;
+    if (nqb <= 0 || nqb > nkb) nqb = nkb;
+    int ncu = 0;
+    const int dev = av_device(&ncu);
     auto go = [&](auto qout, auto wlse, auto full) {
         return launch_short_form<NKB, NW, decltype(qout)::value, decltype(full)::value, decltype(wlse)::value>(
-            B, H, st, (const bf16*)q, (const bf16*)k, (const bf16*)v, (bf16*)o, lse, T, H, ldq, ldk, ldv, ldo, scale * 1.4426950408889634f, G, (uint8_t*)oq, ldoq,
-            (uint8_t*)osc, RBo);
+            B, H, dev, st, (const bf16*)q, (const bf16*)k, (const bf16*)v, (bf16*)o, lse, T, H, ldq, ldk, ldv, ldo, scale * 1.4426950408889634f, G, (uint8_t*)oq, ldoq,
+            (uint8_t*)osc, RBo, nqb);
     };
     const std::true_type yes;
     const std::false_type no;
@@ -411,16 +444,16 @@
 
 int av_attention_fwd(const void* q, const void* k, const void* v, void* o, float* lse, int B, int Tq, int Tk, int H,
                      int hd, long ldq, long ldk, long ldv, long ldo, float scale, int causal, int dtype, int impl,
-                     hipStream_t st, int kv_heads) {
-    AV_CHECK_ARG(q && k && v && o && B > 0 && Tq > 0 && Tk > 0 && H > 0, "attention_fwd: bad args");
+                     hipStream_t st, int kv_heads, int nqb) {
+    AV_CHECK_ARG(q && k && v && o && B > 0 && Tq > 0 && Tk > 0 && H > 0 && nqb >= 0, "attention_fwd: bad args");
     if (kv_heads <= 0) kv_heads = H;
     AV_CHECK_ARG(H % kv_heads == 0, "attention_fwd: %d query heads are not a multiple of %d key/value heads", H, kv_heads);
     const int G = H / kv_heads;
     AV_CHECK_ARG(ldq % 8 == 0 && ldk % 8 == 0 && ldv % 8 == 0 && ldo % 8 == 0, "attention_fwd: row strides must be multiples of 8");
     AV_CHECK_ARG(!causal || Tk >= Tq, "attention_fwd: causal needs Tk >= Tq");
     switch (av_attention_fwd_form(B, Tq, Tk, hd, causal, dtype, impl)) {
-    case AVLLM_ATTN_SHORT13X7: return launch_fwd_short<13, 7>(q, k, v, o, lse, B, Tq, H, ldq, ldk, ldv, ldo, scale, st, G);
-    case AVLLM_ATTN_SHORT17X9: return launch_fwd_short<17, 9>(q, k, v, o, lse, B, Tq, H, ldq, ldk, ldv, ldo, scale, st, G);
+    case AVLLM_ATTN_SHORT13X7: return launch_fwd_short<13, 7>(q, k, v, o, lse, B, Tq, H, ldq, ldk, ldv, ldo, scale, st, G, nqb);
+    case AVLLM_ATTN_SHORT17X9: return launch_fwd_short<17, 9>(q, k, v, o, lse, B, Tq, H, ldq, ldk, ldv, ldo, scale, st, G, nqb);
     case AVLLM_ATTN_MFMA64X4: return launch_fwd<64>(q, k, v, o, lse, B, Tq, Tk, H, ldq, ldk, ldv, ldo, scale, causal, st, G);
     case AVLLM_ATTN_MFMA128X4: return launch_fwd<128>(q, k, v, o, lse, B, Tq, Tk, H, ldq, ldk, ldv, ldo, scale, causal, st, G);
     default: return av_attention_fwd_ref(q, k, v, o, lse, B, Tq, Tk, H, hd, ldq, ldk, ldv, ldo, scale, causal, dtype, st, G);
@@ -435,8 +468,8 @@
     AV_CHECK_ARG(q && k && v && oq && osc && av_attention_fwd_mxq_ok(B, T, H, hd, AV_BF16, H) && ldoq % 16 == 0 && ldq % 8 == 0 && ldk % 8 == 0 && ldv % 8 == 0,
                  "attention_fwd_mxq: bad args (bf16, head_dim 64, T <= 272, 16-byte aligned code rows)");
     if (av_attention_fwd_form(B, T, T, hd, 0, AV_BF16, 0) == AVLLM_ATTN_SHORT13X7)
-        return launch_fwd_short<13, 7>(q, k, v, nullptr, nullptr, B, T, H, ldq, ldk, ldv, 0, scale, st, 1, oq, ldoq, osc);
-    return launch_fwd_short<17, 9>(q, k, v, nullptr, nullptr, B, T, H, ldq, ldk, ldv, 0, scale, st, 1, oq, ldoq, osc);
+        return launch_fwd_short<13, 7>(q, k, v, nullptr, nullptr, B, T, H, ldq, ldk, ldv, 0, scale, st, 1, 0, oq, ldoq, osc);
+    return launch_fwd_short<17, 9>(q, k, v, nullptr, nullptr, B, T, H, ldq, ldk, ldv, 0, scale, st, 1, 0, oq, ldoq, osc);
 }
 extern "C" int avllm_attention_fwd_mxq(const void* q, const void* k, const void* v, void* oq, int64_t ldoq, void* scales, int32_t B, int32_t T, int32_t H,
                                        int32_t hd, int64_t ldq, int64_t ldk, int64_t ldv, float scale, void* stream) {
diff --git a/audio-visual-llm_amd/csrc/avllm_internal.h b/audio-visual-llm_amd/csrc/avllm_internal.h
--- a/audio-visual-llm_amd/csrc/avllm_internal.h
+++ b/audio-visual-llm_amd/csrc/avllm_internal.h
@@ -34,7 +34,7 @@
                          long ldv, float scale, hipStream_t st);
 int av_attention_fwd(const void* q, const void* k, const void* v, void* o, float* lse, int B, int Tq, int Tk, int H,
                      int hd, long ldq, long ldk, long ldv, long ldo, float scale, int causal, int dtype, int impl,
-                     hipStream_t st, int kv_heads = 0);
+                     hipStream_t st, int kv_heads = 0, int nqb = 0);
 int av_attention_bwd(const void* q, const void* k, const void* v, const void* o, const void* dout, const float* lse,
                      void* dq, void* dk, void* dv, float* delta_ws, int B, int T, int H, int hd, long ldq, long ldk,
                      long ldv, long ldo, long lddq, long lddk, long lddv, float scale, int causal, int dtype, int impl,
diff --git a/audio-visual-llm_amd/csrc/common.h b/audio-visual-llm_amd/csrc/common.h
--- a/audio-visual-llm_amd/csrc/common.h
+++ b/audio-visual-llm_amd/csrc/common.h
@@ -18,7 +18,8 @@
 #define AV_WAVE 64
 
 enum AvKnob { AV_KNOB_DECODE_FUSED, AV_KNOB_DEC_AL, AV_KNOB_LORA_UNBATCHED, AV_KNOB_F8_UNFUSED_QUANT, AV_KNOB_F8_FAST, AV_KNOB_ATTN_SHORT,
-              AV_KNOB_NARROW_EPILOGUE, AV_KNOB_TN_CHUNK, AV_KNOB_GEMM_DBG, AV_KNOB_GEMM_GW, AV_KNOB_GEMM_VARIANT, AV_KNOB_SHARED_SPLIT, AV_KNOB_COUNT };
+              AV_KNOB_NARROW_EPILOGUE, AV_KNOB_TN_CHUNK, AV_KNOB_GEMM_DBG, AV_KNOB_GEMM_GW, AV_KNOB_GEMM_VARIANT, AV_KNOB_SHARED_SPLIT, AV_KNOB_CLIP_LAST_FULL,
+              AV_KNOB_COUNT };
 int av_knob(int id);
 
 #define AV_OK 0
diff --git a/audio-visual-llm_amd/csrc/engine.hip b/audio-visual-llm_amd/csrc/engine.hip
--- a/audio-visual-llm_amd/csrc/engine.hip
+++ b/audio-visual-llm_amd/csrc/engine.hip
@@ -82,15 +82,23 @@
         const bool nq = fp8 && d % 128 == 0 && d <= 8192 && !av_knob(AV_KNOB_F8_UNFUSED_QUANT);
         if (nq) AV_TRY(av_norm_mxq(b.x, P.ln1_w, P.ln1_b, nullptr, nullptr, b.f8.q, d, b.f8.s, M, d, eps, st));
         else AV_TRY(av_layernorm(b.x, P.ln1_w, P.ln1_b, b.xn, M, d, eps, dtype, st));
-        AV_TRY(linear(dtype, fq, nq, {P.wqkv, P.wqkv8, P.sqkv8, P.bqkv}, b.xn, d, (int)M, d, 3 * d, b.qkv, 3 * d, AV_ACT_NONE, nullptr, 0, st));
         const char* qkv = (const char*)b.qkv;
         const bool cls = cls_only_last && l == layers - 1;
+        const bool cls_front = cls && !fp8 && !av_knob(AV_KNOB_CLIP_LAST_FULL);
+        if (cls_front) {
+            const void* bkv = P.bqkv ? (const char*)P.bqkv + (size_t)d * es : nullptr;
+            AV_TRY(linear(dtype, nullptr, false, {(const char*)P.wqkv + (size_t)d * d * es, nullptr, nullptr, bkv}, b.xn, d, (int)M, d, 2 * d,
+                          (char*)b.qkv + (size_t)d * es, 3 * d, AV_ACT_NONE, nullptr, 0, st));
+            AV_TRY(linear(dtype, nullptr, false, {P.wqkv, nullptr, nullptr, P.bqkv}, b.xn, (long)tokens * d, (int)items, d, d, b.qkv, (long)tokens * 3 * d,
+                          AV_ACT_NONE, nullptr, 0, st));
+        } else
+        AV_TRY(linear(dtype, fq, nq, {P.wqkv, P.wqkv8, P.sqkv8, P.bqkv}, b.xn, d, (int)M, d, 3 * d, b.qkv, 3 * d, AV_ACT_NONE, nullptr, 0, st));
         const bool att_q = fp8 && !cls && av_attention_fwd_mxq_ok((int)items, tokens, heads, hd, dtype, heads);
         if (att_q) AV_TRY(av_attention_fwd_mxq(qkv, qkv + (size_t)d * es, qkv + (size_t)2 * d * es, b.f8.q, d, b.f8.s, (int)items, tokens, heads, hd,
                                                3 * d, 3 * d, 3 * d, 1.0f / sqrtf((float)hd), st));
         else
         AV_TRY(av_attention_fwd(qkv, qkv + (size_t)d * es, qkv + (size_t)2 * d * es, b.att, nullptr, (int)items, tokens, tokens,
-                                heads, hd, 3 * d, 3 * d, 3 * d, d, 1.0f / sqrtf((float)hd), 0, dtype, 0, st));
+                                heads, hd, 3 * d, 3 * d, 3 * d, d, 1.0f / sqrtf((float)hd), 0, dtype, 0, st, 0, cls_front ? 1 : 0));
         if (cls) fq = nullptr;
         const int rows = cls ? (int)items : (int)M;
         const long ldx = cls ? (long)tokens * d : d;
diff --git a/include/avllm.h b/include/avllm.h
--- a/include/avllm.h
+++ b/include/avllm.h
@@ -129,6 +129,9 @@
                         int32_t H, int32_t hd, int64_t ldq, int64_t ldk, int64_t ldv, int64_t ldo, int64_t lddq,
                         int64_t lddk, int64_t lddv, float scale, int32_t causal, int32_t dtype, int32_t impl,
                         int32_t kv_heads, void* stream);
+int avllm_attention_fwd_blocks(const void* q, const void* k, const void* v, void* o, float* lse, int32_t B, int32_t T, int32_t H, int32_t hd,
+                               int64_t ldq, int64_t ldk, int64_t ldv, int64_t ldo, float scale, int32_t dtype, int32_t kv_heads, int32_t nqb,
+                               void* stream);
 int avllm_attention_bwd_rope(const void* q, const void* k, const void* v, const void* o, const void* dout,
                              const float* lse, void* dq, void* dk, void* dv, float* delta_ws, int32_t B, int32_t T,
                              int32_t H, int32_t hd, int64_t ldq, int64_t ldk, int64_t ldv, int64_t ldo, int64_t lddq,
```
